# jizongFox/Self-paced-Contrastive-Learning

Hardware: AMD Instinct MI355X
Metric: pretrain slices/sec/node (UNet+InfoNCE, 224^2, bs=32/GPU) (higher is better)
Workload: dtype bf16; 1 GPU; BASELINE.json configs[1]: self-paced pretrain step, UNet base (max_channel=256) encoder to Conv5 + ProjectionHead(256,256,256) + SelfPacedSupConLoss(soft, partition labels, correct_grad) fwd+bwd + RAdam; slices_per_gpu=32, images_per_gpu_step=64, image=1x224x224, global_batch=32, parallelism=dp1, params=1311056, hipgraph=epocher, capture_steps=3

## Files before the change

include/spcl_hip.h:

```cpp
#ifndef SPCL_HIP_H
#define SPCL_HIP_H
#include <stddef.h>
#include <stdint.h>
#ifdef __cplusplus
extern "C" {
#endif

#define SPCL_F32 0
#define SPCL_BF16 1

#define SPCL_OK 0
#define SPCL_EINVAL (-1)
#define SPCL_ELAUNCH (-2)
#define SPCL_EUNSUPPORTED (-3)

#define SPCL_ABI_VERSION 27
int spcl_abi_version(void);
const char* spcl_last_error(void);

size_t spcl_supcon_workspace_bytes(int n, int d);
int spcl_supcon_forward(const float* z1, const float* z2, const float* labels, const float* mask, int n, int d,
                        float temperature, int sp_mode, float gamma, int correct_grad, float* ws, float* out,
                        void* stream);
int spcl_supcon_backward(const float* labels, const float* mask, int n, int d, float temperature, int sp_mode,
                         float gamma, const float* ws_fwd, float* ws_bwd, const float* out_fwd,
                         const float* grad_out, float* dz1, float* dz2, void* stream);
size_t spcl_supcon_bwd_workspace_bytes(int n, int d);
int spcl_supcon_unit_gradient_block(int n, int d, size_t* offset_floats, int* row_pitch);
int spcl_supcon_forward_heads(int K, const float* z1, const float* z2, size_t z_stride, const float* labels, int n,
                              int d, float temperature, int sp_mode, const float* gammas, int correct_grad, float* ws,
                              size_t ws_stride, float* out, void* stream);
int spcl_supcon_rows_supported(int n, int d);
int spcl_supcon_forward_rows(int K, const float* o1, const float* o2, size_t o_stride, const float* labels, int n, int d,
                             float temperature, int sp_mode, const float* gammas, int correct_grad, float* ws,
                             size_t ws_stride, float* out, void* stream);
int spcl_supcon_backward_heads(int K, const float* labels, int n, int d, float temperature, int sp_mode,
                               const float* gammas, const float* ws_fwd, size_t ws_stride, float* ws_bwd,
                               size_t wsb_stride, const float* out_fwd, const float* grad_out, float* dz1, float* dz2,
                               size_t z_stride, void* stream);
int spcl_supcon_materialize(const float* labels, const float* mask, int n, int d, float temperature, int sp_mode,
                            float gamma, const float* ws_fwd, float* sim_logits, float* sim_exp, float* pos_mask,
                            float* neg_mask, float* sp_mask, void* stream);

size_t spcl_supcon_xpos_workspace_bytes(int n, int d);
int spcl_supcon_xpos_forward(const float* z1, const float* z2, const float* labels, const float* mask, int n, int d,
                             float temperature, float* ws, float* out, void* stream);
int spcl_supcon_xpos_backward(const float* z1, const float* z2, int n, int d, float temperature, const float* ws,
                              const float* grad_out, float* dz1, float* dz2, void* stream);

size_t spcl_supcon_weighted_workspace_bytes(int n, int d);
int spcl_supcon_weighted_forward(const float* z1, const float* z2, const float* labels, const float* w11,
                                 const float* w22, const float* w12, int blocks, int mask_semantics, int in_mode, int n,
                                 int d, float temperature, float* ws, float* out, void* stream);
int spcl_supcon_weighted_backward(const float* z1, const float* z2, int n, int d, float temperature, float* ws,
                                  const float* grad_out, float* dz1, float* dz2, void* stream);
int spcl_supcon_weighted_materialize(const float* z1, const float* z2, const float* labels, const float* w11,
                                     const float* w22, const float* w12, int blocks, int mask_semantics, int n, int d,
                                     float temperature, float* ws, float* sim_logits, float* sim_exp, float* pos_weight,
                                     float* enable_mask, void* stream);

int spcl_proj_forward(const void* feat, int dtype, int N, int HW, int C, int Cs, const float* w1, const float* b1,
                      const float* w2, const float* b2, int hid, int out_dim, int normalize, float* pooled,
                      float* pre, float* o, float* z, void* stream);
int spcl_proj_backward(const float* dz, int dtype, int N, int HW, int C, int Cs, const float* w1, const float* w2,
                       int hid, int out_dim, int normalize, const float* pooled, const float* pre, const float* o,
                       float* dw1, float* db1, float* dw2, float* db2, float* scratch ,
                       void* dfeat, void* stream);

int spcl_proj_heads_forward(int K, const void* feat, int dtype, int N, int HW, int C, int Cs, const float* const* w1 ,
                            const float* const* b1 , const float* const* w2 , const float* const* b2 ,
                            int hid, int out_dim, int normalize, float* pooled, float* const* pre ,
                            float* const* o , float* const* z , void* stream);
int spcl_proj_heads_backward(int K, const float* const* dz , int dtype, int N, int HW, int C, int Cs,
                             const float* const* w1 , const float* const* w2 , int hid, int out_dim,
                             int normalize, const float* pooled, const float* const* pre ,
                             const float* const* o , float* const* dw1 , float* const* db1 ,
                             float* const* dw2 , float* const* db2 , float* scratch, void* dfeat, void* stream);
int spcl_proj_heads_backward_pooled(int K, const float* const* dz, int dtype, int N, int HW, int C, int Cs,
                                    const float* const* w1, const float* const* w2, int hid, int out_dim, int normalize,
                                    const float* pooled, const float* const* pre, const float* const* o, float* const* dw1,
                                    float* const* db1, float* const* dw2, float* const* db2, float* scratch, void* dfeat_nc,
                                    void* stream);


size_t spcl_conv_packed_elems(int Cin, int Cout, int kind, int dtype);
int spcl_conv_pack_weights(const float* w_oihw, int Cin, int Cout, int kind, int dtype, void* packed, void* stream);
int spcl_conv_pack_weights_both(const float* w_oihw, int Cin, int Cout, int dtype, void* packed_fwd,
                                void* packed_dgrad, void* stream);

int spcl_conv_pack_weights_block(const float* wa_oihw, int CinA, int CoutA, void* a_fwd, void* a_dgrad,
                                 const float* wb_oihw, int CinB, int CoutB, void* b_fwd, void* b_dgrad, int dtype,
                                 void* stream);
int spcl_conv_pack_weights_block_at(const float* wa_oihw, int CinA, int CoutA, void* a_fwd, void* a_dgrad,
                                    const float* wb_oihw, int CinB, int CoutB, void* b_fwd, void* b_dgrad, int dtype,
                                    int H, int W, void* stream);

#define SPCL_PACK_MULTI_MAX 24
typedef struct spcl_pack_item {
  const float* w_oihw;
// ... 265 lines not shown
int spcl_stage_bytes(void* dst, const void* host_src, size_t nbytes, void* stream);
int spcl_copy_pair(void* dst_a, const void* src_a, size_t bytes_a, void* dst_b, const void* src_b, size_t bytes_b,
                   void* stream);

int spcl_augment_views(const float* src, int S, int HS, int WS, const int* params, int nviews, float* out, int OH,
                       int OW, void* stream);
int spcl_augment_views_pil(const float* src, int S, int HS, int WS, const int* params, int nviews, float* out, int OH,
                           int OW, void* stream);
int spcl_rows_linear_forward(const void* x, int x_dtype, long ldx, int leaky_in, const float* W, const float* bias, int M,
                             int K, int N, float* y, void* stream);
int spcl_rows_linear_forward_act(const void* x, int x_dtype, long ldx, const float* W, const float* bias, int M, int K, int N,
                                 void* h, int h_dtype, void* stream);
int spcl_adaptive_avgpool2d_backward_act(const float* dout, const void* act, int dtype, int N, int H, int W, int C, int OH,
                                         int OW, void* dx, void* stream);
int spcl_rows_linear_backward_input(const void* g, int g_dtype, const float* W, const float* pre, int M, int N, int K, void* dx,
                                    int dx_dtype, long lddx, void* stream);
size_t spcl_rows_linear_backward_weight_workspace_bytes(int M, int N, int K);
int spcl_rows_linear_backward_weight(const void* g, int g_dtype, const void* x, int x_dtype, long ldx, int leaky_in, int M, int N,
                                     int K, float* ws, size_t ws_bytes, float* dW, float* db, void* stream);
int spcl_augment_views_recipe(const float* src, const unsigned char* labels, int S, int HS, int WS, const int* params,
                              int nviews, float* out, long long* label_out, int OH, int OW, int max_pad, void* stream);
size_t spcl_augment_views_recipe_workspace_bytes(int nviews, int OH, int OW);
int spcl_augment_views_recipe_ws(const float* src, const unsigned char* labels, int S, int HS, int WS, const int* params,
                                 int nviews, float* out, long long* label_out, int OH, int OW, int max_pad, void* workspace,
                                 size_t workspace_bytes, void* stream);
int spcl_resize_bilinear_pil(const float* src, int S, int HS, int WS, const int* bounds_x, const int* kk_x, int ksize_x,
                             const int* bounds_y, const int* kk_y, int ksize_y, float* tmp, float* out, int OH, int OW,
                             void* stream);
int spcl_resize_nearest_pil(const unsigned char* src, int S, int HS, int WS, const int* xtab ,
                            const int* ytab , unsigned char* out, int OH, int OW, void* stream);

int spcl_flip_batch(const void* x, void* out, int elem_size, int N, int C, int H, int W, const uint8_t* flags,
                    void* stream);
int spcl_flip_pair(const void* first, const void* second, void* out, int elem_size, int N, int C, int H, int W,
                   const uint8_t* flags, void* stream);
int spcl_flip_pair_stage(const void* first, const void* second, void* out, int elem_size, int N, int C, int H, int W,
                         void* stage_dst, const void* host_src, size_t nbytes, size_t flag_off, void* stream);

int spcl_profile_enable(int on);
int spcl_profile_count(void);
int spcl_profile_get(int i, char* name, int name_cap, float* usec, double* bytes, double* flops);

typedef struct spcl_bn_acc {
  long long* acc;
  const float* gamma;
  const float* beta;
  float* running_mean;
  float* running_var;
  long long* num_batches_tracked;
  float* st;
  float momentum, eps;
  float count;
  int C, CS;
} spcl_bn_acc;
size_t spcl_bn_acc_elems(int CS);
int spcl_conv_bn_acc_supported(int dtype, int N, int H, int W, int CinK, int CoutS, int in_kind, int with_stats_acc);
int spcl_conv3x3_forward_acc(const void* x, int dtype, int N, int H, int W, int CinK, int CoutS, const void* w_packed,
                             const spcl_bn_acc* in_bn, const float* in_scale, const float* in_shift, void* y,
                             long long* stats_acc, float* stats_rows, void* stream);
int spcl_bnrelu_pool_forward_acc(const void* y, int dtype, int N, int H, int W, int CS, const spcl_bn_acc* bn, void* act_out,
                                 void* pool_out, void* stream);
int spcl_bnrelu_gap_supported(int dtype, int H, int W, int C, int CS);
int spcl_bnrelu_gap_forward(const void* y, int dtype, int N, int H, int W, int C, int CS, const float* scale,
                            const float* shift, const spcl_bn_acc* bn, void* act_out, float* gap_out, void* stream);
int spcl_conv_dgrad_bnstats_acc_supported(int dtype, int N, int H, int W, int CinK, int CoutS);
int spcl_conv3x3_dgrad_bnstats_acc(const void* dy, int dtype, int N, int H, int W, int CinK, int CoutS, const void* w_packed,
                                   void* g, const void* y2, const float* scale2, const float* shift2, const float* mean2,
                                   long long* acc, void* stream);
int spcl_conv_dgrad_poolstats_acc_supported(int dtype, int N, int H, int W, int CinK, int CoutS, int H2, int W2);
int spcl_conv3x3_dgrad_poolstats_acc(const void* dy, int dtype, int N, int H, int W, int CinK, int CoutS, const void* w_packed,
                                     void* g, const void* y2, int H2, int W2, const float* scale2, const float* shift2,
                                     const float* mean2, long long* acc, void* stream);
int spcl_bnrelu_pool_forward_ymax(const void* y, int dtype, int N, int H, int W, int CS, const float* scale,
                                  const float* shift, const spcl_bn_acc* bn, void* act_out, void* pool_out, void* ymax_out,
                                  void* stream);
int spcl_conv_dgrad_poolmax_supported(int dtype, int N, int H, int W, int CinK, int CoutS);
int spcl_conv3x3_dgrad_poolmax(const void* dy, int dtype, int N, int H, int W, int CinK, int CoutS, const void* w_packed,
                               void* g, const void* ymax, const float* scale2, const float* shift2, const float* mean2,
                               float* rows2, void* stream);
int spcl_conv_dgrad_poolmax_acc_supported(int dtype, int N, int H, int W, int CinK, int CoutS);
int spcl_conv3x3_dgrad_poolmax_acc(const void* dy, int dtype, int N, int H, int W, int CinK, int CoutS, const void* w_packed,
                                   void* g, const void* ymax, const float* scale2, const float* shift2, const float* mean2,
                                   long long* acc, void* stream);
int spcl_bnrelu_backward_acc(const void* y, const void* dact, const void* dpool, const void* dact_nc, int dtype, int N, int H,
                             int W, int C, int CS, const float* st4, int training, long long* acc, float* dgamma, float* dbeta,
                             void* dy, void* stream);
int spcl_bnrelu_backward_fill_acc(const void* y, void* dact, int dact_stride, const void* dpool, const void* d_up, int dtype,
                                  int N, int H, int W, int C, int CS, const float* st4, int training, long long* acc,
                                  float* dgamma, float* dbeta, void* dy, void* stream);
int spcl_bnrelu_backward_rows_acc(const void* y, const void* dact, const void* dpool, const float* rows, int nrows, int dtype,
                                  int N, int H, int W, int C, int CS, const float* st4, int training, long long* acc,
                                  float* dgamma, float* dbeta, void* dy, void* stream);

size_t spcl_iic_joint_workspace_bytes(int S, int K, int pad);
int spcl_iic_joint_forward(const float* lx, const float* ly, long ld, int N, int H, int W, int S, int K, int pad,
                           const uint8_t* flags_x, long long* jacc, void* stream);
size_t spcl_iic_loss_workspace_bytes(int S, int T);
int spcl_iic_loss(const long long* jacc, const float* jf32, int S, int K, int T, int dense, float scale, float* j_out,
                  float* loss, float* dj, int* nan_flag, void* ws, size_t ws_bytes, void* stream);
int spcl_iic_joint_backward(const float* lx, const float* ly, long ld, int N, int H, int W, int S, int K, int pad,
                            const uint8_t* flags_x, const float* dj, const float* gscale, float* dlx, float* dly, void* stream);
size_t spcl_consistency_workspace_bytes(int N, int H, int W);
int spcl_consistency_softmax_mse(const float* a, const float* b, int N, int C, int H, int W, const uint8_t* flags_a,
                                 float weight, float* loss, float* db, void* ws, size_t ws_bytes, void* stream);

int spcl_iic_patch_plan(int N, int C, int H, int W, int pad, int patch, int* num_patches, size_t* ws_bytes, size_t* dj_elems);
int spcl_iic_patch_forward(const float* lx, const float* ly, int N, int C, int H, int W, int pad, int patch,
                           const uint8_t* flags_y, float scale, float* loss, float* patch_loss, int* nan_flag, float* dj,
                           void* ws, size_t ws_bytes, void* stream);
int spcl_iic_patch_backward(const float* lx, const float* ly, int N, int C, int H, int W, int pad, int patch,
                            const uint8_t* flags_y, const float* dj, const float* gscale, float* dlx, float* dly, void* stream);

int spcl_iic_patch_heads_plan(int N, int S, int K, long ld, int H, int W, int pad, int patch, int* num_patches,
                              size_t* ws_bytes, size_t* dj_elems);
int spcl_iic_patch_heads_forward(const float* lx, const float* ly, long ld, int N, int H, int W, int S, int K, int pad,
                                 int patch, const uint8_t* flags_y, float scale, float* loss, float* head_patch_loss,
                                 int* nan_flag, float* dj, void* ws, size_t ws_bytes, void* stream);
int spcl_iic_patch_heads_backward(const float* lx, const float* ly, long ld, int N, int H, int W, int S, int K, int pad,
                                  int patch, const uint8_t* flags_y, const float* dj, const float* gscale, float* dlx,
                                  float* dly, void* stream);

int spcl_ema_update(float* teacher, const float* student, size_t n, double alpha, double decay, void* stream);
size_t spcl_mt_softmax_mse_workspace_bytes(int N, int H, int W);
int spcl_mt_softmax_mse(const float* teacher, const float* student_logits, int N, int C, int H, int W,
                        const uint8_t* flags_teacher, int teacher_mode, float weight, float* loss, float* dstudent, void* ws,
                        size_t ws_bytes, void* stream);
size_t spcl_entropy_softmax_workspace_bytes(int N, int H, int W);
int spcl_entropy_softmax(const float* logits, int N, int C, int H, int W, float eps, float weight, float* loss, float* dlogits,
                         void* ws, size_t ws_bytes, void* stream);
size_t spcl_ucmt_workspace_bytes(int N, int H, int W);
int spcl_ucmt_softmax_mse(const float* teacher, const float* const* noisy, int K, const float* student_logits, int N, int C,
                          int H, int W, const uint8_t* flags_teacher, float threshold, float eps, float weight, float* loss,
                          float* dstudent, unsigned long long* kept, uint8_t* mask, void* ws, size_t ws_bytes, void* stream);

int spcl_mixup_images(const float* image, const float* image_tf, const int* index, int N2, size_t per_sample, float lam,
                      float oml, float* out, void* stream);
size_t spcl_mixup_kl_workspace_bytes(int N2, int H, int W);
int spcl_mixup_kl_onehot(const float* logits, const int64_t* target, const int64_t* target_tf, const int* index, int N2, int C,
                         int H, int W, float lam, float oml, float eps, float weight, float* loss, float* dlogits, void* ws,
                         size_t ws_bytes, void* stream);

int spcl_patch4s2_rows_forward(const float* a, int Ca, long a_sn, long a_sc, long a_sh, long a_sw, const float* b, int Cb,
                               long b_sn, long b_sc, long b_sh, long b_sw, int N, int H, int W, int mode, const float* scale,
                               const float* shift, float* rows, void* stream);
int spcl_patch4s2_rows_backward(const float* drows, const float* x, int N, int H, int W, int C, int c_lo, int mode,
                                const float* scale, const float* shift, float* dx, void* stream);
size_t spcl_rows_bn_workspace_bytes(int M, int C);
int spcl_rows_bn_forward(const float* x, int M, int C, const float* gamma, const float* beta, float eps, float momentum,
                         float* running_mean, float* running_var, float* stats, void* ws, size_t ws_bytes, void* stream);
int spcl_rows_bn_eval_affine(const float* gamma, const float* beta, const float* running_mean, const float* running_var,
                             float eps, int C, float* stats, void* stream);
int spcl_rows_bn_backward(const float* du, const float* x, int M, int C, const float* gamma, const float* stats, int training,
                          float* dx, float* dgamma, float* dbeta, void* ws, size_t ws_bytes, void* stream);
size_t spcl_discr_head_workspace_bytes(int N, int H, int W, int C);
int spcl_discr_head_forward(const float* x, int N, int H, int W, int C, const float* scale, const float* shift, const float* w,
                            int y, float* t, float* d, float* loss, float* dt, void* ws, size_t ws_bytes, void* stream);
int spcl_discr_head_backward(const float* x, int N, int H, int W, int C, const float* scale, const float* shift, const float* w,
                             const float* dt, const float* grad, float* du, float* dw, void* ws, size_t ws_bytes, void* stream);

int spcl_mine_pairs_forward(const void* feat, const uint8_t* flags, int dtype, int n, int H, int W, int C, void* joint, void* marg,
                            void* stream);
int spcl_mine_pairs_backward(const void* djoint, const void* dmarg, const uint8_t* flags, int dtype, int n, int H, int W, int C,
                             void* dfeat, void* stream);
size_t spcl_mine_head_workspace_bytes(int n, int H, int W, int C);
int spcl_mine_head_forward(const void* act_joint, const void* act_marg, int dtype, int n, int H, int W, int C, const float* w,
                           const float* b, float* t, float* maxima, int* argmax, float* loss, void* ws, size_t ws_bytes,
// ... 16 lines not shown
```

self-paced-contrastive-learning_amd/csrc/bn_acc.hpp:

```cpp
#pragma once
#include "common.hpp"

namespace spcl {

#ifndef SPCL_ACC_REPLICAS
#define SPCL_ACC_REPLICAS 8
#endif
constexpr int BN_ACC_REPLICAS = SPCL_ACC_REPLICAS;
constexpr int BN_ACC_FLAG_WORDS = 4;
constexpr double BN_ACC_HI = 1024.0, BN_ACC_HI_INV = 1.0 / 1024.0;
constexpr double BN_ACC_LO = 1152921504606846976.0 , BN_ACC_LO_INV = 1.0 / 1152921504606846976.0;
constexpr float BN_ACC_MAX = 1099511627776.0f;
#ifndef SPCL_ACC_FWD_TILES
#define SPCL_ACC_FWD_TILES 4096
#endif
constexpr int BN_ACC_MAX_TILES_FWD = SPCL_ACC_FWD_TILES;
constexpr int BN_ACC_MAX_TILES_BWD = 4096;

__host__ __device__ inline size_t bn_acc_words(int CS) { return (size_t)BN_ACC_REPLICAS * CS * 4 + BN_ACC_FLAG_WORDS; }

struct BnAccFwd {
  const long long* acc;
  const float* gamma;
  const float* beta;
// ... 91 lines not shown
    const int cc = c < f.C ? c : f.C - 1;
    g = f.gamma[cc];
    b = f.beta[cc];
    rm = (f.running_mean != nullptr ? f.running_mean : f.gamma)[cc];
    rv = (f.running_var != nullptr ? f.running_var : f.gamma)[cc];
  }
};
__device__ __forceinline__ void bn_acc_fwd_channel(const BnAccFwd& f, const BnAccSums& sums, const BnAccFwdParams& in, int c,
                                                   float& scale, float& shift, bool write) {
  if (c >= f.C) {
    scale = 0.f;
    shift = 0.f;
    if (write) { f.st[c] = 0.f; f.st[f.CS + c] = 0.f; f.st[2 * f.CS + c] = 0.f; f.st[3 * f.CS + c] = 0.f; }
    return;
  }
  double s1, s2;
  sums.totals(s1, s2);
  const float g = in.g, b = in.b;
  const double n = (double)f.count;
  const double mu = s1 * f.inv_count;
  const double m2 = fmax(s2 - s1 * mu, 0.0);
  const double var = m2 * f.inv_count;
  float is = 1.0f / sqrtf((float)var + f.eps);
  float sc = g * is;
  scale = sc;
  shift = b - (float)mu * sc;
  if (sums.flag != 0) {
    is = sc = scale = shift = __builtin_nanf("");
  }
  if (write) {
    f.st[c] = (float)mu;
    f.st[f.CS + c] = is;
    f.st[2 * f.CS + c] = sc;
    f.st[3 * f.CS + c] = shift;
    if (f.running_mean != nullptr) f.running_mean[c] = (1.f - f.momentum) * in.rm + f.momentum * (float)mu;
    if (f.running_var != nullptr) {
      const double unbiased = n > 1.0 ? m2 / (n - 1.0) : var;
      f.running_var[c] = (1.f - f.momentum) * in.rv + f.momentum * (float)unbiased;
    }
    if (f.nbt != nullptr && c == 0) f.nbt[0] += 1;
  }
}
struct BnAccFwdRaw {
  BnAccRaw raw;
  BnAccFwdParams prm;
  __device__ __forceinline__ void load(const BnAccFwd& f, int c) {
    raw.load(f.acc, f.CS, c < f.C ? c : f.C - 1, 0);
    prm.load(f, c);
  }
};
__device__ __forceinline__ void bn_acc_fwd_channel(const BnAccFwd& f, const BnAccFwdRaw& in, int c, float& scale, float& shift,
                                                   bool write) {
  bn_acc_fwd_channel(f, in.raw.sums(), in.prm, c, scale, shift, write);
}

struct BnAccBwdRaw {
  BnAccRaw raw;
  float mean, invstd, scale;
  __device__ __forceinline__ void load(const BnAccBwd& f, int c) {
    raw.load(f.acc, f.CS, c, 0);
    mean = f.st[c];
    invstd = f.st[f.CS + c];
    scale = f.st[2 * f.CS + c];
  }
};
__device__ __forceinline__ void bn_acc_bwd_channel(const BnAccBwd& f, const BnAccBwdRaw& in, int c, float& A, float& B,
                                                   bool write) {
  double t1, t2;
  in.raw.sums().totals(t1, t2);
  const float mean = in.mean, invstd = in.invstd, scale = in.scale;
  const float s1 = (float)t1;
  const float s2 = (float)t2 * invstd;
  A = 0.f;
  B = 0.f;
  if (f.training) {
    A = -scale * invstd * (s2 / f.count);
    B = -scale * (s1 / f.count) - A * mean;
  }
  if (write && c < f.C) {
    f.dbeta[c] = s1;
    f.dgamma[c] = s2;
  }
}
#endif

}
```

self-paced-contrastive-learning_amd/csrc/conv.hip:

```cpp
#include <stdlib.h>
#include "bn_acc.hpp"
#include "conv_common.hpp"
#include "image_acorr.hpp"

namespace spcl {

#ifndef SPCL_SPLIT_KC_MAX
#define SPCL_SPLIT_KC_MAX 64
#endif
__host__ __device__ inline int split_kc(int CinK, int CoutS) {
  const int cap = CoutS <= 16 ? 16 : (CoutS <= 32 ? 32 : SPCL_SPLIT_KC_MAX);
  return CinK < cap ? CinK : cap;
}
__host__ __device__ inline int split_pstride(int KC) {
  const int b = 3 * KC * 2;
  return (b / 32) % 2 == 1 ? b : b + 32;
}
__device__ __forceinline__ f32x4 mfma_bf16(u32x4 w, u32x4 x, f32x4 acc) {
  return __builtin_amdgcn_mfma_f32_16x16x32_bf16(__builtin_bit_cast(bf16x8, w), __builtin_bit_cast(bf16x8, x), acc, 0, 0, 0);
}

template <typename T, int TH, int TW, int NT, bool SPLIT = false>
__global__ __launch_bounds__(256) void conv3x3_mfma_kernel(ConvArgs a) {
  static_assert(!SPLIT || sizeof(T) == 4, "the split k-loop is the f32 storage path");
// ... 1354 lines not shown
  if (!(CinK <= 64 || CinK % 64 == 0)) return false;
  a.in_scale = a.in_shift = nullptr;
  a.stats = nullptr;
  a.N = N; a.H = H; a.W = W; a.CinS = CinK; a.CinK = CinK; a.CoutS = CoutS; a.in_mode = 0;
  a.tilesX = a.tilesY = 0;
  a.tpw = 1;
  a.dbg = 0;
  return true;
}

extern "C" int spcl_conv_dgrad_bnstats_supported(int dtype, int N, int H, int W, int CinK, int CoutS) {
  static const bool off = lab_flag("SPCL_NO_DGRAD_BNSTATS");
  ConvArgs a;
  if (off || !dgrad_bnstats_args(a, dtype, N, H, W, CinK, CoutS)) return 0;
  if (conv_use_gemm(CinK, CoutS, H, W)) return 1;
  a.x = nullptr; a.y = nullptr; a.wp = nullptr;
  float dummy;
  a.rows2 = &dummy;
  TileCfg t = pick_tile(H, W);
  return (t.tw == 14 && launch_conv_fast(a, t.th, nullptr, true)) ? 1 : 0;
}

static int dgrad_bnstats_impl(const void* dy, int dtype, int N, int H, int W, int CinK, int CoutS, const void* w_packed, void* g,
                              const void* y2, const float* scale2, const float* shift2, const float* mean2, float* rows2,
                              long long* acc, void* stream);

extern "C" int spcl_conv3x3_dgrad_bnstats(const void* dy, int dtype, int N, int H, int W, int CinK, int CoutS,
                                          const void* w_packed, void* g, const void* y2, const float* scale2,
                                          const float* shift2, const float* mean2, float* rows2, void* stream) {
  SPCL_CHECK_ARG(rows2, "conv3x3_dgrad_bnstats: null pointer");
  return dgrad_bnstats_impl(dy, dtype, N, H, W, CinK, CoutS, w_packed, g, y2, scale2, shift2, mean2, rows2, nullptr, stream);
}

extern "C" int spcl_conv_dgrad_bnstats_acc_supported(int dtype, int N, int H, int W, int CinK, int CoutS) {
  ConvArgs a;
  if (!spcl_conv_dgrad_bnstats_supported(dtype, N, H, W, CinK, CoutS) || conv_use_gemm(CinK, CoutS, H, W)) return 0;
  if (!dgrad_bnstats_args(a, dtype, N, H, W, CinK, CoutS)) return 0;
  a.x = nullptr; a.y = nullptr; a.wp = nullptr;
  float dummy;
  long long dummy2;
  a.rows2 = &dummy;
  a.rows2_acc = &dummy2;
  TileCfg t = pick_tile(H, W);
  return (t.tw == 14 && launch_conv_fast(a, t.th, nullptr, true)) ? 1 : 0;
}

extern "C" int spcl_conv3x3_dgrad_bnstats_acc(const void* dy, int dtype, int N, int H, int W, int CinK, int CoutS,
                                              const void* w_packed, void* g, const void* y2, const float* scale2,
                                              const float* shift2, const float* mean2, long long* acc, void* stream) {
  SPCL_CHECK_ARG(acc, "conv3x3_dgrad_bnstats_acc: null pointer");
  return dgrad_bnstats_impl(dy, dtype, N, H, W, CinK, CoutS, w_packed, g, y2, scale2, shift2, mean2, nullptr, acc, stream);
}

static int dgrad_bnstats_impl(const void* dy, int dtype, int N, int H, int W, int CinK, int CoutS, const void* w_packed, void* g,
                              const void* y2, const float* scale2, const float* shift2, const float* mean2, float* rows2,
                              long long* acc, void* stream) {
  SPCL_CHECK_ARG(dy && w_packed && g && y2 && scale2 && shift2 && mean2, "conv3x3_dgrad_bnstats: null pointer");
  ConvArgs a;
  if (!dgrad_bnstats_args(a, dtype, N, H, W, CinK, CoutS) || (acc != nullptr && conv_use_gemm(CinK, CoutS, H, W))) {
    set_error("conv3x3_dgrad_bnstats: unsupported configuration");
    return SPCL_EUNSUPPORTED;
  }
  a.x = dy; a.y = g; a.wp = w_packed;
  a.y2 = y2; a.scale2 = scale2; a.shift2 = shift2; a.mean2 = mean2;
  a.rows2 = acc != nullptr ? (float*)acc : rows2;
  a.rows2_acc = acc;
  hipStream_t st = (hipStream_t)stream;
  const double px = (double)N * H * W;
  prof_cost(px * (CinK + 2.0 * CoutS) * 2.0 + 9.0 * CinK * CoutS * 2.0, 2.0 * px * 9.0 * CinK * CoutS);
  TileCfg t = pick_tile(H, W);
  if (conv_use_gemm(CinK, CoutS, H, W)) {
    if (!launch_conv_gemm(a, st)) {
      set_error("conv3x3_dgrad_bnstats: H=%d W=%d CinK=%d CoutS=%d outside the gemm kernel's range", H, W, CinK, CoutS);
      return SPCL_EUNSUPPORTED;
    }
  } else if (!(t.tw == 14 && launch_conv_fast(a, t.th, st))) {
    set_error("conv3x3_dgrad_bnstats: no specialised kernel for H=%d W=%d CinK=%d CoutS=%d", H, W, CinK, CoutS);
    return SPCL_EUNSUPPORTED;
  }
  SPCL_LAUNCH_CHECK("conv3x3_dgrad_bnstats");
  return SPCL_OK;
}

extern "C" int spcl_conv_dgrad_bnstats_image_supported(int dtype, int N, int H, int W, int CinK, int CoutS) {
  static const bool off = lab_flag("SPCL_NO_IMAGE3");
  ConvArgs a;
  if (off || CinK != 16 || CoutS != 16 || !dgrad_bnstats_args(a, dtype, N, H, W, CinK, CoutS)) return 0;
  if (!spcl_conv_dgrad_bnstats_supported(dtype, N, H, W, CinK, CoutS) || conv_use_gemm(CinK, CoutS, H, W)) return 0;
  a.x = nullptr; a.y = nullptr; a.wp = nullptr;
  float dummy;
  a.rows2 = &dummy;
  a.img2 = &dummy;
  TileCfg t = pick_tile(H, W);
  return (t.tw == 14 && t.th == 14 && launch_conv_fast(a, t.th, nullptr, true)) ? 1 : 0;
}

extern "C" int spcl_conv3x3_dgrad_bnstats_image(const void* dy, int dtype, int N, int H, int W, int CinK, int CoutS,
                                                const void* w_packed, void* g, const void* y2, const float* scale2,
                                                const float* shift2, const float* mean2, const float* image,
                                                float* rows11, void* stream) {
  SPCL_CHECK_ARG(dy && w_packed && y2 && scale2 && shift2 && mean2 && image && rows11,
                 "conv3x3_dgrad_bnstats_image: null pointer");
  ConvArgs a;
  if (!spcl_conv_dgrad_bnstats_image_supported(dtype, N, H, W, CinK, CoutS) ||
      !dgrad_bnstats_args(a, dtype, N, H, W, CinK, CoutS)) {
    set_error("conv3x3_dgrad_bnstats_image: unsupported configuration (bf16, 16 -> 16 channels, 14 x 14 tiles)");
    return SPCL_EUNSUPPORTED;
  }
  a.x = dy; a.y = g; a.wp = w_packed;
  a.y2 = y2; a.scale2 = scale2; a.shift2 = shift2; a.mean2 = mean2; a.rows2 = rows11; a.img2 = image;
  hipStream_t st = (hipStream_t)stream;
  const double px = (double)N * H * W;
  prof_cost(px * (CinK + (g ? 2.0 : 1.0) * CoutS) * 2.0 + px * 4.0 + 9.0 * CinK * CoutS * 2.0,
            2.0 * px * 9.0 * CinK * CoutS + 2.0 * px * 9.0 * CoutS);
  TileCfg t = pick_tile(H, W);
  if (!(t.tw == 14 && launch_conv_fast(a, t.th, st))) {
    set_error("conv3x3_dgrad_bnstats_image: no specialised kernel for H=%d W=%d", H, W);
    return SPCL_EUNSUPPORTED;
  }
  SPCL_LAUNCH_CHECK("conv3x3_dgrad_bnstats_image");
  return SPCL_OK;
}

extern "C" int spcl_conv_dgrad_poolstats_supported(int dtype, int N, int H, int W, int CinK, int CoutS, int H2, int W2) {
  static const bool off = lab_flag("SPCL_NO_DGRAD_POOLSTATS");
  ConvArgs a;
  if (off || H != H2 / 2 || W != W2 / 2 || !dgrad_bnstats_args(a, dtype, N, H, W, CinK, CoutS)) return 0;
  if (conv_use_gemm(CinK, CoutS, H, W)) return 0;
  a.x = nullptr; a.y = nullptr; a.wp = nullptr;
  float dummy;
  a.rows2 = &dummy;
  a.H2 = H2; a.W2 = W2;
  TileCfg t = pick_tile(H, W);
  return (t.tw == 14 && launch_conv_fast(a, t.th, nullptr, true)) ? 1 : 0;
}

static int dgrad_poolstats_impl(const void* dy, int dtype, int N, int H, int W, int CinK, int CoutS, const void* w_packed,
                                void* g, const void* y2, int H2, int W2, const float* scale2, const float* shift2,
                                const float* mean2, float* rows2, long long* acc, void* stream);

extern "C" int spcl_conv3x3_dgrad_poolstats(const void* dy, int dtype, int N, int H, int W, int CinK, int CoutS,
                                            const void* w_packed, void* g, const void* y2, int H2, int W2,
                                            const float* scale2, const float* shift2, const float* mean2, float* rows2,
                                            void* stream) {
  SPCL_CHECK_ARG(rows2, "conv3x3_dgrad_poolstats: null pointer");
  return dgrad_poolstats_impl(dy, dtype, N, H, W, CinK, CoutS, w_packed, g, y2, H2, W2, scale2, shift2, mean2, rows2, nullptr,
                              stream);
}

extern "C" int spcl_conv_dgrad_poolstats_acc_supported(int dtype, int N, int H, int W, int CinK, int CoutS, int H2, int W2) {
  ConvArgs a;
  if (!spcl_conv_dgrad_poolstats_supported(dtype, N, H, W, CinK, CoutS, H2, W2)) return 0;
  if (!dgrad_bnstats_args(a, dtype, N, H, W, CinK, CoutS)) return 0;
  a.x = nullptr; a.y = nullptr; a.wp = nullptr;
  float dummy;
  long long dummy2;
  a.rows2 = &dummy;
  a.rows2_acc = &dummy2;
  a.H2 = H2; a.W2 = W2;
  TileCfg t = pick_tile(H, W);
  return (t.tw == 14 && launch_conv_fast(a, t.th, nullptr, true)) ? 1 : 0;
}

extern "C" int spcl_conv3x3_dgrad_poolstats_acc(const void* dy, int dtype, int N, int H, int W, int CinK, int CoutS,
                                                const void* w_packed, void* g, const void* y2, int H2, int W2,
                                                const float* scale2, const float* shift2, const float* mean2,
// ... 97 lines not shown
```

self-paced-contrastive-learning_amd/csrc/conv_common.hpp:

```cpp
#pragma once
#include "common.hpp"

namespace spcl {

struct BnAccFwd;
template <typename T> struct Chunk;
template <> struct Chunk<float> { static constexpr int EPC = 4; };
template <> struct Chunk<bf16_t> { static constexpr int EPC = 8; };

struct uint4_ { uint32_t x, y, z, w; };
typedef __attribute__((ext_vector_type(4))) uint32_t u32x4;

__host__ __device__ inline int conv_kc(int CinK) { return CinK < 64 ? CinK : 64; }
template <typename T> __host__ __device__ inline int conv_pstride(int KC) {
  int b = KC * (int)sizeof(T);
  return b == 32 ? 32 : b + 32;
}
template <typename T> __host__ __device__ inline int conv_nsteps(int KC) {
  int cp = KC / Chunk<T>::EPC;
  return (9 * cp + 3) / 4;
}

struct ConvArgs {
  const void* x;
  void* y;
  const void* wp;
  float* stats;
  const float* in_scale;
  const float* in_shift;
  int N, H, W;
  int CinS;
  int CinK;
  int CoutS;
  int in_mode;
  int tilesX, tilesY;
  int tpw;
  int dbg;
  const void* y2 = nullptr;
  const float* scale2 = nullptr;
  const float* shift2 = nullptr;
  const float* mean2 = nullptr;
  float* rows2 = nullptr;
  int H2 = 0, W2 = 0;
  bool y2_is_poolmax = false;
  const float* img2 = nullptr;
  const void* x2 = nullptr;
  void* y_hi = nullptr;
  bool x_up2 = false;
  float* acorr_rows = nullptr;
  const float* img1 = nullptr;
  const void* wp1 = nullptr;
  long long* stats_acc = nullptr;
  long long* rows2_acc = nullptr;
  const struct BnAccFwd* in_bn = nullptr;
};

struct split_f32 { float v; };
template <> struct Chunk<split_f32> { static constexpr int EPC = 4; };
bool conv_f32_split();

typedef __attribute__((ext_vector_type(2))) float f32x2_;
typedef __attribute__((ext_vector_type(2))) __bf16 bf16x2v_;
struct Split3 { uint32_t hi, mid, lo; };
__device__ __forceinline__ Split3 split3_pair(float v0, float v1) {
  Split3 o;
  f32x2_ v = {v0, v1};
  o.hi = __builtin_bit_cast(uint32_t, __builtin_convertvector(v, bf16x2v_));
  v[0] -= __uint_as_float(o.hi << 16);
  v[1] -= __uint_as_float(o.hi & 0xffff0000u);
  o.mid = __builtin_bit_cast(uint32_t, __builtin_convertvector(v, bf16x2v_));
  v[0] -= __uint_as_float(o.mid << 16);
  v[1] -= __uint_as_float(o.mid & 0xffff0000u);
  o.lo = __builtin_bit_cast(uint32_t, __builtin_convertvector(v, bf16x2v_));
  return o;
}
__device__ __forceinline__ void split3_chunk(const float* e, u32x4& ph, u32x4& pm, u32x4& pl) {
#pragma unroll
  for (int k = 0; k < 4; ++k) {
    const Split3 o = split3_pair(e[2 * k], e[2 * k + 1]);
    ph[k] = o.hi;
    pm[k] = o.mid;
    pl[k] = o.lo;
  }
}
template <typename T> __device__ __forceinline__ f32x4 mfma_chunk(u32x4 w, u32x4 x, f32x4 acc);
template <> __device__ __forceinline__ f32x4 mfma_chunk<bf16_t>(u32x4 w, u32x4 x, f32x4 acc) {
  return __builtin_amdgcn_mfma_f32_16x16x32_bf16(__builtin_bit_cast(bf16x8, w), __builtin_bit_cast(bf16x8, x), acc, 0,
                                                 0, 0);
}
template <> __device__ __forceinline__ f32x4 mfma_chunk<float>(u32x4 w, u32x4 x, f32x4 acc) {
  f32x4 wf = __builtin_bit_cast(f32x4, w), xf = __builtin_bit_cast(f32x4, x);
  acc = __builtin_amdgcn_mfma_f32_16x16x4f32(wf[0], xf[0], acc, 0, 0, 0);
  acc = __builtin_amdgcn_mfma_f32_16x16x4f32(wf[1], xf[1], acc, 0, 0, 0);
  acc = __builtin_amdgcn_mfma_f32_16x16x4f32(wf[2], xf[2], acc, 0, 0, 0);
  acc = __builtin_amdgcn_mfma_f32_16x16x4f32(wf[3], xf[3], acc, 0, 0, 0);
  return acc;
}

__device__ __forceinline__ float row16_sum(float v) {
  v += __builtin_bit_cast(float, __builtin_amdgcn_update_dpp(0, __builtin_bit_cast(int, v), 0xB1, 0xF, 0xF, true));
  v += __builtin_bit_cast(float, __builtin_amdgcn_update_dpp(0, __builtin_bit_cast(int, v), 0x4E, 0xF, 0xF, true));
  v += __builtin_bit_cast(float, __builtin_amdgcn_update_dpp(0, __builtin_bit_cast(int, v), 0x141, 0xF, 0xF, true));
  v += __builtin_bit_cast(float, __builtin_amdgcn_update_dpp(0, __builtin_bit_cast(int, v), 0x140, 0xF, 0xF, true));
  return v;
}

typedef __attribute__((ext_vector_type(2))) float f32x2;
typedef __attribute__((ext_vector_type(2))) __bf16 bf16x2v;
typedef __attribute__((ext_vector_type(2))) short s16x2v;

__device__ __forceinline__ uint32_t relu_bf16x2(uint32_t packed) {
  const s16x2v z = {0, 0};
  return __builtin_bit_cast(uint32_t, __builtin_elementwise_max(__builtin_bit_cast(s16x2v, packed), z));
}

template <typename T> __device__ __forceinline__ u32x4 bnrelu_regs(u32x4 raw, const float* s, const float* b);
template <> __device__ __forceinline__ u32x4 bnrelu_regs<float>(u32x4 raw, const float* s, const float* b) {
  f32x4 v = __builtin_bit_cast(f32x4, raw);
#pragma unroll
  for (int e = 0; e < 4; ++e) v[e] = fmaxf(fmaf(s[e], v[e], b[e]), 0.f);
  return __builtin_bit_cast(u32x4, v);
}
template <> __device__ __forceinline__ u32x4 bnrelu_regs<bf16_t>(u32x4 raw, const float* s, const float* b) {
  u32x4 out;
#pragma unroll
  for (int e = 0; e < 4; ++e) {
    float lo = __uint_as_float(raw[e] << 16), hi = __uint_as_float(raw[e] & 0xffff0000u);
    lo = fmaf(s[2 * e], lo, b[2 * e]);
    hi = fmaf(s[2 * e + 1], hi, b[2 * e + 1]);
    const f32x2 v = {lo, hi};
    out[e] = relu_bf16x2(__builtin_bit_cast(uint32_t, __builtin_convertvector(v, bf16x2v)));
  }
  return out;
}

template <typename T> __device__ __forceinline__ void store4_fast(unsigned char* p, f32x4 v);
template <> __device__ __forceinline__ void store4_fast<float>(unsigned char* p, f32x4 v) { *(f32x4*)p = v; }
template <> __device__ __forceinline__ void store4_fast<bf16_t>(unsigned char* p, f32x4 v) {
  const f32x2 lo = {v[0], v[1]}, hi = {v[2], v[3]};
  uint2 o;
  o.x = __builtin_bit_cast(uint32_t, __builtin_convertvector(lo, bf16x2v));
  o.y = __builtin_bit_cast(uint32_t, __builtin_convertvector(hi, bf16x2v));
  *(uint2*)p = o;
}

__device__ __forceinline__ void write_tile_stats(float* stats, int tile, int CoutS, int cb, int r16, float cnt,
                                                 f32x4 ssum, f32x4 ssq) {
  const float inv = 1.f / cnt;
  f32x4 o;
#pragma unroll
  for (int r = 0; r < 4; ++r) {
    const float s1 = row16_sum(ssum[r]), s2 = row16_sum(ssq[r]);
    const float mean = s1 * inv;
    float prod = s1 * mean;
    asm volatile("" : "+v"(prod));
    const float m2 = fmaxf(s2 - prod, 0.f);
    o[r] = r16 == 0 ? cnt : (r16 == 1 ? mean : m2);
  }
  if (r16 < 3) *(f32x4*)(stats + ((size_t)tile * 3 + r16) * CoutS + cb) = o;
}

bool launch_conv_fast(const ConvArgs& a, int th, hipStream_t st, bool dry = false);

__host__ __device__ inline bool conv_gemm_channels(int CinK, int CoutS) {
  return CinK % 64 == 0 && CoutS % 64 == 0 && CinK >= 64 && CoutS >= 64 && (CinK >= 128 || CoutS >= 128);
}
bool conv_gemm_fits(int H, int W, int CinK, int CoutS);
bool conv_use_gemm(int CinK, int CoutS, int H, int W);
void conv_set_gemm(int mode);
bool launch_conv_gemm(const ConvArgs& a, hipStream_t st);
int conv_gemm_stat_rows(int N, int H, int W, int CinK, int CoutS);

}
```

self-paced-contrastive-learning_amd/csrc/conv_fast.hip:

```cpp
#include <stdlib.h>
#include <type_traits>
#include <vector>
#include "bn_acc.hpp"
#include "conv_common.hpp"

namespace spcl {

struct FastArgs {
  const unsigned char* x;
  const unsigned char* x2;
  unsigned char* y;
  unsigned char* y_hi;
  int up2;
  const u32x4* wp;
  float* stats;
  const float* in_scale;
  const float* in_shift;
  int N, H, W, CinK, CoutS, tilesX, tilesY, gy;
  unsigned long long* stamps;
  int ipw;
  int lds_flip;
  int xcd_remap;
  const unsigned char* y2;
  const float* scale2;
  const float* shift2;
  const float* mean2;
  float* rows2;
  int H2, W2;
  const float* img2;
  const float* img1;
  const u32x4* wp1;
  float* acorr_rows;
  long long* stats_acc;
  long long* rows2_acc;
  BnAccFwd in_bn;
};

#ifndef SPCL_FAST_WPE_NT1
#define SPCL_FAST_WPE_NT1 2
#endif
#ifndef SPCL_FAST_WPE_NT1_NW4
#define SPCL_FAST_WPE_NT1_NW4 3
#endif
#ifndef SPCL_FAST_WR_NT1
#define SPCL_FAST_WR_NT1 9
#endif
#ifndef SPCL_FAST_WPE_KC32
#define SPCL_FAST_WPE_KC32 2
#endif
#ifndef SPCL_FAST_YPRE_MINKC
#define SPCL_FAST_YPRE_MINKC 16
#endif
#ifndef SPCL_FAST_WIDE_STORES
#define SPCL_FAST_WIDE_STORES 1
#endif
#ifndef SPCL_FAST_DBG
#define SPCL_FAST_DBG 0
#endif
#ifndef SPCL_FAST_ROWMAP
#define SPCL_FAST_ROWMAP 1
#endif
#ifndef SPCL_FAST_RP
#define SPCL_FAST_RP (SPCL_FAST_ROWMAP ? 18 : 22)
#endif
#ifndef SPCL_FAST_RP_NARROW
#define SPCL_FAST_RP_NARROW (SPCL_FAST_ROWMAP ? 18 : 22)
#endif
constexpr int fast_pixel_stride(int KC) { return KC == 16 ? 32 : KC * 2 + 32; }
constexpr int fast_row_pitch(int KC) { return KC == 64 ? SPCL_FAST_RP : SPCL_FAST_RP_NARROW; }
constexpr int fast_lds_bytes(int KC, int TH) { return (TH + 2) * fast_row_pitch(KC) * fast_pixel_stride(KC); }
constexpr bool fast_preload_slab(int KC, int NW, int NT) { return KC == 32 || (KC == 64 && NW >= 2 && NT >= 1); }
constexpr int fast_wpe(int KC, int TH, int NW, int NT, int MODE = 0) {
  const int wgs = 160 * 1024 / fast_lds_bytes(KC, TH);
  int w = (wgs * NW + 3) / 4;
  w = w > 4 ? 4 : (w < 1 ? 1 : w);
  const int acc = (SPCL_FAST_ROWMAP ? TH : (TH * 14 + 15) / 16) * NT * 4;
  if (KC == 16 && MODE >= 2 && MODE <= 4 && SPCL_FAST_YPRE_MINKC <= 16 && w > 3 && acc <= 80) return 3;
  if (acc > 80 && w > 2) return 2;
  if (KC == 64 && NT == 1 && NW == 4 && w > 2) return SPCL_FAST_WPE_NT1_NW4;
  if (KC == 64 && NT == 1 && NW >= 2 && w > 2) return SPCL_FAST_WPE_NT1;
  if (KC == 32 && fast_preload_slab(KC, NW, NT) && w > SPCL_FAST_WPE_KC32) return SPCL_FAST_WPE_KC32;
  if (fast_preload_slab(KC, NW, NT) && w > 2) return 2;
  return w;
}

template <int KC, int TH, int NT, int MODE, int NW>
__global__ __launch_bounds__(64 * NW) __attribute__((amdgpu_waves_per_eu(fast_wpe(KC, TH, NW, NT, MODE)))) void
conv3x3_fast_kernel(FastArgs a) {
  constexpr int TW = 14, HW_ = 16, CP = KC / 8, NHALO = (TH + 2) * HW_, PS = fast_pixel_stride(KC);
  constexpr int RP = fast_row_pitch(KC);
  constexpr int NTHR = 64 * NW, NCH = NHALO * CP, ITER = (NCH + NTHR - 1) / NTHR, QS = NTHR / CP;
  constexpr bool RM = SPCL_FAST_ROWMAP != 0;
  constexpr int NPIX = TH * TW, MT = RM ? TH : (NPIX + 15) / 16, NSTEPS = (9 * CP + 3) / 4;
  constexpr bool PRELOAD_W = KC == 16;
  constexpr bool PRELOAD_SLAB = fast_preload_slab(KC, NW, NT);
  static_assert(QS >= HW_ ? QS % HW_ == 0 : HW_ % QS == 0, "staging walk needs whole/even halo rows per iteration");
  extern __shared__ __attribute__((aligned(16))) unsigned char lds[];

  const int t = threadIdx.x, lane = t & 63, wave = t >> 6, r16 = lane & 15, g = lane >> 4;
#ifndef SPCL_FAST_STAMPS_BUILD
#define SPCL_FAST_STAMPS_BUILD 0
#endif
  const bool stamp = SPCL_FAST_STAMPS_BUILD && a.stamps != nullptr && t == 0;
  unsigned long long t_begin = 0, t_k0 = 0, t_k1 = 0, t_store = 0;
  if (stamp) t_begin = __builtin_amdgcn_s_memtime();
  int tx = blockIdx.x, ty = blockIdx.y;
  {
    const int T = a.tilesX * a.tilesY;
    if (a.xcd_remap && (T & 7) == 0) {
      const int L = ty * a.tilesX + tx;
      const int L2 = (L & 7) * (T >> 3) + (L >> 3);
      ty = L2 / a.tilesX;
      tx = L2 - ty * a.tilesX;
    }
  }
  int n = blockIdx.z, by = 0;
#if SPCL_FAST_DBG & 4
  if (KC == 64 && a.CinK >= 128 && gridDim.z == 2u * a.N * a.gy) n >>= 1;
#endif
  if (a.gy > 1) {
    by = n / a.N;
    n -= by * a.N;
  }
  const int y0 = min(ty * TH, a.H - TH), x0 = min(tx * TW, a.W - TW);
  const int oy = ty * TH - y0, ox = tx * TW - x0;
  const int tile = (n * a.tilesY + ty) * a.tilesX + tx;
  const int ntn = a.CoutS >> 4;
  const int nt0 = (by * NW + wave) * NT;
  const bool interior = y0 > 0 && x0 > 0 && y0 + TH < a.H && x0 + TW < a.W;
#if SPCL_FAST_DBG & 4
  const int nslab = KC < 64 ? 1 : ((a.CinK >= 128 && gridDim.z == 2u * a.N * a.gy) ? a.CinK / KC / 2 : a.CinK / KC);
#else
  const int nslab = KC < 64 ? 1 : a.CinK / KC;
#endif
  const int gps = (KC < 64 ? KC : a.CinK) * 2;

  constexpr bool M2 = MODE == 2 || MODE == 4;
  constexpr bool M1 = MODE == 1 || (MODE >= 5 && MODE <= 7);
  constexpr bool M8 = MODE == 8;
  static_assert(!M8 || (KC == 16 && TH == 14 && NT == 1 && NW == 1), "MODE 8: the 16 -> 16 layer on 14 x 14 tiles, one wave");
  constexpr int ACC_TPC = MODE == 5 ? 4 : (MODE == 6 ? 2 : 1);
  float imgv[MODE == 4 ? 4 : 1];
  if (MODE == 4) {
    const int hr = lane >> 2, hc = (lane & 3) * 4;
    const int gy = y0 - 1 + hr;
    const float* ir = a.img2 + ((size_t)n * a.H + (gy < 0 ? 0 : (gy >= a.H ? a.H - 1 : gy))) * a.W;
#pragma unroll
    for (int e = 0; e < 4; ++e) {
      const int gx = x0 - 1 + hc + e;
      const bool in = gy >= 0 && gy < a.H && gx >= 0 && gx < a.W;
      const float xv = ir[gx < 0 ? 0 : (gx >= a.W ? a.W - 1 : gx)];
      imgv[e] = in ? xv : 0.f;
    }
  }

  u32x4 wall[PRELOAD_W ? NSTEPS : 1][NT];
  if (PRELOAD_W) {
#pragma unroll
    for (int s = 0; s < NSTEPS; ++s)
#pragma unroll
      for (int j = 0; j < NT; ++j) wall[s][j] = a.wp[(size_t)(s * ntn + nt0 + j) * 64 + lane];
  }

  const int ch = t & (CP - 1), q0 = t / CP;
  const int hy0 = q0 / HW_, hx0 = q0 % HW_;
  const bool two = a.x2 != nullptr;
  const bool two_chunks = two && a.CinK == KC;
  const int gps1 = two ? gps / 2 : gps;
  const int ch1 = two_chunks ? (ch & (CP / 2 - 1)) : ch;
  const long xorg = (((long)n * a.H + (y0 - 1)) * a.W + (x0 - 1)) * gps1;
  const unsigned char* xb = ((two_chunks && ch >= CP / 2) ? a.x2 : a.x) + xorg;
  const unsigned char* xb2 = two ? a.x2 + xorg : nullptr;
  const unsigned voff = (unsigned)((hy0 * a.W + hx0) * gps1 + ch1 * 16);
  unsigned char* const lp = lds + (hy0 * RP + hx0) * PS + ch * 16;

  int abase[MT];
#pragma unroll
  for (int i = 0; i < MT; ++i) {
    if (RM) {
      abase[i] = (i * RP + r16) * PS + (CP >= 4 ? g * 16 : 0);
    } else {
      int p = 16 * i + r16;
      if (p >= NPIX) p = 0;
      const int py = p / TW, px = p - py * TW;
      abase[i] = (py * RP + px) * PS + (CP >= 4 ? g * 16 : 0);
    }
  }
  f32x4 acc[MT][NT];
#pragma unroll
  for (int i = 0; i < MT; ++i)
#pragma unroll
    for (int j = 0; j < NT; ++j) acc[i][j] = (f32x4){0.f, 0.f, 0.f, 0.f};

  const int flip = a.lds_flip;
  const unsigned wvo = (unsigned)(nt0 * 64 + lane) * 16u;
  const size_t wstep = (size_t)ntn * 1024;
  u32x4 v[ITER];
  float ssc[8], ssh[8];
  constexpr int IW8 = 18;
  float imv8[M8 ? 6 : 1];
  s16x4 wfrag8 = {0, 0, 0, 0};
  f32x4 sc8 = {0.f, 0.f, 0.f, 0.f}, sh8 = {0.f, 0.f, 0.f, 0.f};
  const int ir8 = lane / IW8, ic8 = lane - ir8 * IW8;
  constexpr bool STREAM_W = PRELOAD_SLAB && KC == 64;
  constexpr int WR = STREAM_W ? (NT == 1 ? SPCL_FAST_WR_NT1 : 9) : (PRELOAD_SLAB ? NSTEPS : 1);
  u32x4 wsl[WR][NT];
  constexpr bool acc_in = MODE >= 5 && MODE <= 7;
  float* const coef_l = (float*)(lds + fast_lds_bytes(KC, TH) * (a.lds_flip != 0 ? 2 : 1));
  auto load_coef_lds = [&](int slab) {
    const int cc = two_chunks ? ch1 : ch;
#pragma unroll
    for (int e = 0; e < 8; e += 4) {
      *(f32x4*)&ssc[e] = *(const f32x4*)(coef_l + slab * KC + cc * 8 + e);
      *(f32x4*)&ssh[e] = *(const f32x4*)(coef_l + a.CinK + slab * KC + cc * 8 + e);
    }
  };
  auto issue_halo = [&](int slab, const bool first = false) {
    if (acc_in) {
      if (!first) load_coef_lds(slab);
    } else if (M1) {
#pragma unroll
      for (int e = 0; e < 8; e += 4) {
        const int cc = two_chunks ? ch1 : ch;
        *(f32x4*)&ssc[e] = *(const f32x4*)(a.in_scale + slab * KC + cc * 8 + e);
        *(f32x4*)&ssh[e] = *(const f32x4*)(a.in_shift + slab * KC + cc * 8 + e);
      }
    }
    const int hslab = (a.CinK / KC) >> 1;
    const unsigned char* xs = (two && !two_chunks) ? (slab >= hslab ? xb2 + (slab - hslab) * (KC * 2) : xb + slab * (KC * 2))
                                                   : xb + slab * (KC * 2);
    auto walk = [&](auto up2_c, auto interior_c) {
      constexpr bool UP2 = decltype(up2_c)::value, INTERIOR = decltype(interior_c)::value;
#pragma unroll
      for (int k = 0; k < ITER; ++k) {
        const int dky = QS >= HW_ ? k * (QS / HW_) : k / (HW_ / QS);
        const int dkx = QS >= HW_ ? 0 : (k % (HW_ / QS)) * QS;
        const long soff = ((long)dky * a.W + dkx) * gps1;
        bool inb = (NCH % NTHR == 0) || (k * NTHR + t < NCH);
        if (!INTERIOR) {
          const int gy = y0 - 1 + hy0 + dky, gx = x0 - 1 + hx0 + dkx;
          inb = inb && gy >= 0 && gy < a.H && gx >= 0 && gx < a.W;
        }
        v[k] = (u32x4){0u, 0u, 0u, 0u};
        if (UP2) {
          const int gy = y0 - 1 + hy0 + dky, gx = x0 - 1 + hx0 + dkx;
          if (inb)
            v[k] = *(const u32x4*)(a.x + (((long)n * (a.H >> 1) + (gy >> 1)) * (a.W >> 1) + (gx >> 1)) * gps + slab * (KC * 2) +
                                   ch * 16);
        } else if (inb) v[k] = *(const u32x4*)(xs + soff + voff);
      }
    };
    if (a.up2) walk(std::true_type{}, std::false_type{});
    else if (interior) walk(std::false_type{}, std::true_type{});
    else walk(std::false_type{}, std::false_type{});
  };
  unsigned char* lpw = lp;
  auto slab_body = [&](const int slab, const bool refill) {
    auto stage = [&](auto interior_c) {
      constexpr bool INTERIOR = decltype(interior_c)::value;
#pragma unroll
      for (int k = 0; k < ITER; ++k) {
        const int dky = QS >= HW_ ? k * (QS / HW_) : k / (HW_ / QS);
        const int dkx = QS >= HW_ ? 0 : (k % (HW_ / QS)) * QS;
        const bool in_range = (NCH % NTHR == 0) || (k * NTHR + t < NCH);
        u32x4 tv = v[k];
        if (M1) {
          bool inb = true;
          if (!INTERIOR) {
            const int gy = y0 - 1 + hy0 + dky, gx = x0 - 1 + hx0 + dkx;
            inb = gy >= 0 && gy < a.H && gx >= 0 && gx < a.W;
          }
          if (inb && (!two_chunks || ch >= CP / 2)) tv = bnrelu_regs<bf16_t>(tv, ssc, ssh);
        }
        if (in_range) *(u32x4*)(lpw + (dky * RP + dkx) * PS) = tv;
      }
    };
    if constexpr (M8) {
      typedef uint32_t __attribute__((may_alias)) pair_t;
      typedef unsigned short __attribute__((may_alias)) half_t;
      const pair_t* const pairs = (const pair_t*)lds;
      half_t* const halves = (half_t*)lds;
      unsigned short pb8[6];
#pragma unroll
      for (int k = 0; k < 6; ++k) {
        const f32x2 pv = {imv8[k], 0.f};
        pb8[k] = (unsigned short)__builtin_bit_cast(uint32_t, __builtin_convertvector(pv, bf16x2v));
      }
      if (lane < 3 * IW8) {
#pragma unroll
        for (int k = 0; k < 6; ++k) halves[2 * ((ir8 + 3 * k) * IW8 + ic8)] = pb8[k];
        if (ic8 > 0) {
#pragma unroll
          for (int k = 0; k < 6; ++k) halves[2 * ((ir8 + 3 * k) * IW8 + ic8) - 1] = pb8[k];
        }
        if (ic8 == IW8 - 1) {
#pragma unroll
          for (int k = 0; k < 6; ++k) halves[2 * ((ir8 + 3 * k) * IW8 + ic8) + 1] = 0;
        }
      }
      __syncthreads();
      const int gx = x0 - 1 + r16;
      const bool colin = gx >= 0 && gx < a.W;
      const int gg = g < 3 ? g : 0;
      uint2 hv[HW_];
#pragma unroll
      for (int hy = 0; hy < TH + 2; ++hy) {
        const pair_t* src = pairs + (hy + gg) * IW8 + r16;
        const uint2 xv = {src[0], src[2]};
        const f32x4 y = __builtin_amdgcn_mfma_f32_16x16x16bf16_1k(wfrag8, __builtin_bit_cast(s16x4, xv),
                                                                  (f32x4){0.f, 0.f, 0.f, 0.f}, 0, 0, 0);
        const f32x2 ylo = {y[0], y[1]}, yhi = {y[2], y[3]};
        const uint32_t p0 = __builtin_bit_cast(uint32_t, __builtin_convertvector(ylo, bf16x2v));
        const uint32_t p1 = __builtin_bit_cast(uint32_t, __builtin_convertvector(yhi, bf16x2v));
        const u32x4 raw = {p0, p1, 0u, 0u};
        const float s4[8] = {sc8[0], sc8[1], sc8[2], sc8[3], 0.f, 0.f, 0.f, 0.f};
        const float b4[8] = {sh8[0], sh8[1], sh8[2], sh8[3], 0.f, 0.f, 0.f, 0.f};
        const u32x4 tv = bnrelu_regs<bf16_t>(raw, s4, b4);
        hv[hy] = (uint2){tv[0], tv[1]};
      }
      if (!interior) {
#pragma unroll
        for (int hy = 0; hy < TH + 2; ++hy) {
          const int gy = y0 - 1 + hy;
          if (!(colin && gy >= 0 && gy < a.H)) hv[hy] = (uint2){0u, 0u};
        }
      }
      __syncthreads();
#pragma unroll
      for (int hy = 0; hy < TH + 2; ++hy) *(uint2*)(lds + (hy * RP + r16) * PS + g * 8) = hv[hy];
    } else if (M1 && !interior) stage(std::false_type{});
    else stage(std::true_type{});
    if (refill) issue_halo(slab + 1);
    if (stamp && slab == 0) t_store = __builtin_amdgcn_s_memtime();
    __syncthreads();
    if (stamp && slab == 0) t_k0 = __builtin_amdgcn_s_memtime();

    const u32x4* wslab = a.wp + ((size_t)slab * NSTEPS * ntn + nt0) * 64 + lane;
    auto frag_off = [&](const int s) {
      if (CP >= 4) {
        const int fc0 = 4 * s, tap = fc0 / CP, c0 = fc0 % CP, ky = tap / 3, kx = tap % 3;
        return (ky * RP + kx) * PS + c0 * 16;
      }
      int fc = 4 * s + g;
      if (fc >= 9 * CP) fc = 0;
      const int tap = fc / CP, c = fc % CP, ky = (tap * 11) >> 5, kx = tap - 3 * ky;
      return (ky * RP + kx) * PS + c * 16;
    };
    if (STREAM_W) {
      const __amdgpu_buffer_rsrc_t wrs = __builtin_amdgcn_make_buffer_rsrc((void*)a.wp, 0, 0x7fffffff, 0x00020000);
      unsigned wrun = (unsigned)(((size_t)slab * NSTEPS + WR) * wstep);
      u32x4 xf[2][MT];
#pragma unroll
      for (int i = 0; i < MT; ++i) xf[0][i] = *(const u32x4*)(lds + abase[i] + frag_off(0));
#pragma unroll
      for (int s = 0; s < NSTEPS; ++s) {
        u32x4 wf[NT];
#pragma unroll
        for (int j = 0; j < NT; ++j) wf[j] = wsl[s % WR][j];
#pragma unroll
        for (int i = 0; i < MT; ++i) {
#pragma unroll
          for (int j = 0; j < NT; ++j) acc[i][j] = mfma_chunk<bf16_t>(wf[j], xf[s & 1][i], acc[i][j]);
          if (s + 1 < NSTEPS && !(SPCL_FAST_DBG & 2)) xf[(s + 1) & 1][i] = *(const u32x4*)(lds + abase[i] + frag_off(s + 1));
          if (i == MT - 1 && (s + WR < NSTEPS || refill) && !(SPCL_FAST_DBG & 1)) {
#pragma unroll
            for (int j = 0; j < NT; ++j)
              wsl[s % WR][j] = __builtin_bit_cast(u32x4, __builtin_amdgcn_raw_buffer_load_b128(wrs, wvo + j * 1024, wrun, 0));
          }
          __builtin_amdgcn_sched_barrier(0);
        }
        wrun += (unsigned)wstep;
      }
    } else {
#pragma unroll
      for (int s = 0; s < NSTEPS; ++s) {
        u32x4 wf[NT];
#pragma unroll
        for (int j = 0; j < NT; ++j)
          wf[j] = PRELOAD_W ? wall[s][j] : (PRELOAD_SLAB ? wsl[s][j] : wslab[(size_t)(s * ntn + j) * 64]);
        const int off = frag_off(s);
#pragma unroll
        for (int i = 0; i < MT; ++i) {
          const u32x4 xf = *(const u32x4*)(lds + abase[i] + off);
#pragma unroll
          for (int j = 0; j < NT; ++j) acc[i][j] = mfma_chunk<bf16_t>(wf[j], xf, acc[i][j]);
          if (RM && !PRELOAD_SLAB && i % 7 == 6) __builtin_amdgcn_sched_barrier(0);
        }
      }
    }
  };
#ifndef SPCL_ACC_DBG
#define SPCL_ACC_DBG 0
#endif
  const int acc_part = acc_in ? t / a.CinK : 0, acc_c = t - acc_part * a.CinK;
  constexpr int ACC_RPT = BN_ACC_REPLICAS / ACC_TPC > 0 ? BN_ACC_REPLICAS / ACC_TPC : 1;
  const bool acc_has = acc_part * ACC_RPT < BN_ACC_REPLICAS;
  BnAccPart<ACC_RPT> accp;
  BnAccFwdParams accprm;
  if (acc_in && SPCL_ACC_DBG < 2) {
    accp.load(a.in_bn.acc, a.CinK, acc_c, acc_has ? ACC_RPT * acc_part : 0);
    accprm.load(a.in_bn, acc_c);
  }
  if constexpr (M8) {
    const float* im = a.img1 + (size_t)n * a.H * a.W;
    const int gx = x0 - 2 + ic8;
    const bool colok = gx >= 0 && gx < a.W;
    const int gxc = gx < 0 ? 0 : (gx >= a.W ? a.W - 1 : gx);
#pragma unroll
    for (int k = 0; k < 6; ++k) {
      const int gy = y0 - 2 + ir8 + 3 * k;
      const int gyc = gy < 0 ? 0 : (gy >= a.H ? a.H - 1 : gy);
      const float raw = im[(size_t)gyc * a.W + gxc];
      imv8[k] = (colok && gy >= 0 && gy < a.H) ? raw : 0.f;
    }
    if (g < 3) {
      const bf16_t* wq = (const bf16_t*)a.wp1;
#pragma unroll
      for (int kx = 0; kx < 3; ++kx) {
        const int tap = 3 * g + kx;
        wfrag8[kx] = (short)wq[(size_t)(((tap >> 1) * 64) + (2 * (tap & 1)) * 16 + r16) * 8];
      }
    }
    sc8 = *(const f32x4*)(a.in_scale + 4 * g);
    sh8 = *(const f32x4*)(a.in_shift + 4 * g);
  } else {
    issue_halo(0, true);
  }
  if (PRELOAD_SLAB) {
#pragma unroll
    for (int s = 0; s < WR; ++s)
#pragma unroll
      for (int j = 0; j < NT; ++j) wsl[s][j] = a.wp[((size_t)s * ntn + nt0 + j) * 64 + lane];
  }
  if (acc_in) {
    const bool writer = (blockIdx.x | blockIdx.y | blockIdx.z) == 0;
    BnAccSums sums{0, 0, 0, 0, 0};
    if (SPCL_ACC_DBG < 2 && acc_has) sums = accp.sums();
    if (SPCL_ACC_DBG < 2) sums.flag = accp.flag;
    if (ACC_TPC > 1) {
      long long* const part_l = (long long*)(coef_l + 2 * a.CinK);
      if (acc_part > 0) {
        long long* q = part_l + ((size_t)(acc_part - 1) * a.CinK + acc_c) * 4;
        *(i64x2*)q = (i64x2){sums.h1, sums.l1};
        *(i64x2*)(q + 2) = (i64x2){sums.h2, sums.l2};
      }
      __syncthreads();
      if (acc_part == 0) {
#pragma unroll
        for (int k = 1; k < ACC_TPC; ++k) {
          const long long* q = part_l + ((size_t)(k - 1) * a.CinK + acc_c) * 4;
          const i64x2 u = *(const i64x2*)q, w = *(const i64x2*)(q + 2);
          sums.h1 += u[0]; sums.l1 += u[1]; sums.h2 += w[0]; sums.l2 += w[1];
        }
      }
    }
    if (t < a.CinK) {
      float sc_, sh_;
      if (SPCL_ACC_DBG == 0) bn_acc_fwd_channel(a.in_bn, sums, accprm, t, sc_, sh_, writer);
      else { sc_ = a.in_bn.gamma[t]; sh_ = a.in_bn.beta[t]; }
      coef_l[t] = sc_;
      coef_l[a.CinK + t] = sh_;
    }
    __syncthreads();
    load_coef_lds(0);
  }
  if (MODE == 4) {
    const int q = lane & 3;
    float n0 = __shfl_down(imgv[0], 1, 64), n1 = __shfl_down(imgv[1], 1, 64);
    if (q == 3) n0 = n1 = 0.f;
    const float h6[6] = {imgv[0], imgv[1], imgv[2], imgv[3], n0, n1};
    unsigned char* imb = lds + fast_lds_bytes(KC, TH) + (lane >> 2) * 32 + q * 8;
#pragma unroll
    for (int kx = 0; kx < 3; ++kx) {
      const f32x2 lo = {h6[kx], h6[kx + 1]}, hi = {h6[kx + 2], h6[kx + 3]};
      uint2 w;
      w.x = __builtin_bit_cast(uint32_t, __builtin_convertvector(lo, bf16x2v));
      w.y = __builtin_bit_cast(uint32_t, __builtin_convertvector(hi, bf16x2v));
      *(uint2*)(imb + kx * 512) = w;
    }
  }
  int img = 0;
#pragma unroll 1
  for (int slab = 0; slab + 1 < nslab; ++slab) {
    if (slab > 0 && flip == 0) __syncthreads();
    slab_body(slab, true);
    const int d = img ? -flip : flip;
    img ^= 1;
    lpw += d;
#pragma unroll
    for (int i = 0; i < MT; ++i) abase[i] += d;
  }
  if (nslab > 1 && flip == 0) __syncthreads();
  slab_body(nslab - 1, false);
  if (stamp) t_k1 = __builtin_amdgcn_s_memtime();

  constexpr int DPY = RM ? 1 : 16 / TW, DPX = RM ? 0 : 16 % TW;
  const int rowb = a.CoutS * 2;
  const bool twoy = (MODE == 0 || MODE == 2) && a.y_hi != nullptr;
  const bool up_only = MODE == 2 && twoy;
  const int rowo = twoy ? rowb / 2 : rowb;
  unsigned char* yj[NT];
#pragma unroll
  for (int j = 0; j < NT; ++j) {
    const int gnt = nt0 + j, half = ntn / 2;
    unsigned char* dst = (twoy && gnt >= half) ? a.y_hi : a.y;
    yj[j] = dst + (((size_t)n * a.H + y0) * a.W + x0) * rowo + ((twoy && gnt >= half ? gnt - half : gnt) * 16 + 4 * g) * 2;
  }
  int py = RM ? 0 : r16 / TW, px = r16 - py * TW;
  int ob = (py * a.W + px) * rowo;
  const int dob = (DPY * a.W + DPX) * rowo, wrapo = (a.W - TW) * rowo;
  f32x4 ssum[NT], ssq[NT];
  f32x4 sc2[NT], sh2[NT], mu2[NT];
  const unsigned char* y2b = nullptr;
#pragma unroll
  for (int j = 0; j < NT; ++j) {
    ssum[j] = (f32x4){0.f, 0.f, 0.f, 0.f};
    ssq[j] = (f32x4){0.f, 0.f, 0.f, 0.f};
    if (M2 || MODE == 3) {
      const int gnt2 = nt0 + j, half2 = ntn / 2;
      const int cb = (up_only ? (gnt2 >= half2 ? gnt2 - half2 : 0) : gnt2) * 16 + 4 * g;
      sc2[j] = *(const f32x4*)(a.scale2 + cb);
      sh2[j] = *(const f32x4*)(a.shift2 + cb);
      mu2[j] = *(const f32x4*)(a.mean2 + cb);
    }
  }
  if (M2) y2b = a.y2 + (((size_t)n * a.H + y0) * a.W + x0) * rowb + (nt0 * 16 + 4 * g) * 2;
  const unsigned char* y2j[NT];
  bool st2[NT];
#pragma unroll
  for (int j = 0; j < NT; ++j) {
    const int gnt2 = nt0 + j, half2 = ntn / 2;
    st2[j] = !up_only || gnt2 >= half2;
    y2j[j] = !M2 ? nullptr
                 : (up_only ? a.y2 + (((size_t)n * a.H + y0) * a.W + x0) * rowo + ((st2[j] ? gnt2 - half2 : 0) * 16 + 4 * g) * 2
                            : y2b + j * 32);
  }
  constexpr int M4_DZ = 0, M4_IM = fast_lds_bytes(KC, TH);
  static_assert(MODE != 4 || fast_lds_bytes(KC, TH) >= 7168, "MODE 4 scratch does not fit the halo image");
  if (MODE == 4) {
#pragma unroll
    for (int k = 0; k < 4; ++k) {
      const int e = k * 64 + lane;
      if (e < 16 * TH) *(uint32_t*)(lds + M4_DZ + e * 32 + 28) = 0u;
    }
    __syncthreads();
  }
  const bool shifted = (oy | ox) != 0;
// ... 60 lines not shown
          const bool second = PAIRED && i % 2 == 1 && (RM || 16 * i + 15 < NPIX);
          if (first || second) {
            const f32x2 lo = {acc[i][j][0], acc[i][j][1]}, hi = {acc[i][j][2], acc[i][j][3]};
            uint2 pkc;
            pkc.x = __builtin_bit_cast(uint32_t, __builtin_convertvector(lo, bf16x2v));
            pkc.y = __builtin_bit_cast(uint32_t, __builtin_convertvector(hi, bf16x2v));
            if (first) {
              pk_prev[j] = pkc;
              ob_prev = ob;
            } else {
              const auto rx = __builtin_amdgcn_permlane16_swap(pk_prev[j].x, pkc.x, false, false);
              const auto ry = __builtin_amdgcn_permlane16_swap(pk_prev[j].y, pkc.y, false, false);
              const u32x4 v = {rx[0], ry[0], rx[1], ry[1]};
              *(u32x4*)(yj[j] + ((g & 1) ? ob - 8 : ob_prev)) = v;
            }
          } else {
            store4_fast<bf16_t>(yj[j] + ob, acc[i][j]);
          }
        }
        if (M2) {
          const uint2 yr = YPRE ? ypre[i][j][0] : *(const uint2*)(y2j[j] + ob);
          const f32x2 glo = {acc[i][j][0], acc[i][j][1]}, ghi = {acc[i][j][2], acc[i][j][3]};
          const uint32_t g0 = __builtin_bit_cast(uint32_t, __builtin_convertvector(glo, bf16x2v));
          const uint32_t g1 = __builtin_bit_cast(uint32_t, __builtin_convertvector(ghi, bf16x2v));
          const float yv[4] = {__uint_as_float(yr.x << 16), __uint_as_float(yr.x & 0xffff0000u),
                               __uint_as_float(yr.y << 16), __uint_as_float(yr.y & 0xffff0000u)};
          const float gv[4] = {__uint_as_float(g0 << 16), __uint_as_float(g0 & 0xffff0000u),
                               __uint_as_float(g1 << 16), __uint_as_float(g1 & 0xffff0000u)};
#pragma unroll
          for (int r = 0; r < 4; ++r) {
            const float dz = (st2[j] && fmaf(sc2[j][r], yv[r], sh2[j][r]) > 0.f) ? gv[r] * keep : 0.f;
            ssum[j][r] += dz;
            ssq[j][r] = fmaf(dz, yv[r] - mu2[j][r], ssq[j][r]);
            if (MODE == 4) *(bf16_t*)(lds + M4_DZ + (4 * g + r) * 448 + pyc * 32 + px * 2) = f32_to_bf16(dz);
          }
        } else if (MODE == 3) {
          const f32x2 glo = {acc[i][j][0], acc[i][j][1]}, ghi = {acc[i][j][2], acc[i][j][3]};
          const uint32_t g0 = __builtin_bit_cast(uint32_t, __builtin_convertvector(glo, bf16x2v));
          const uint32_t g1 = __builtin_bit_cast(uint32_t, __builtin_convertvector(ghi, bf16x2v));
          const float gv[4] = {__uint_as_float(g0 << 16), __uint_as_float(g0 & 0xffff0000u),
                               __uint_as_float(g1 << 16), __uint_as_float(g1 & 0xffff0000u)};
          uint2 yr[4];
          if (YPRE) {
#pragma unroll
            for (int k = 0; k < 4; ++k) yr[k] = ypre[i][j][k];
          } else {
            const unsigned char* wb = a.y2 + ((((size_t)n * a.H2 + 2 * (y0 + pyc)) * a.W2 + 2 * (x0 + px)) * rowb) +
                                      ((nt0 + j) * 16 + 4 * g) * 2;
#pragma unroll
            for (int k = 0; k < 4; ++k) yr[k] = *(const uint2*)(wb + ((size_t)(k >> 1) * a.W2 + (k & 1)) * rowb);
          }
#pragma unroll
          for (int r = 0; r < 4; ++r) {
            float zb = -1.f, yb = 0.f;
#pragma unroll
            for (int k = 0; k < 4; ++k) {
              const uint32_t wd = r < 2 ? yr[k].x : yr[k].y;
              const float yv = (r & 1) ? __uint_as_float(wd & 0xffff0000u) : __uint_as_float(wd << 16);
              pool_first_max(k, fmaf(sc2[j][r], yv, sh2[j][r]), yv, zb, yb);
            }
            const float dz = zb > 0.f ? gv[r] * keep : 0.f;
            ssum[j][r] += dz;
            ssq[j][r] = fmaf(dz, yb - mu2[j][r], ssq[j][r]);
          }
        } else {
          const f32x4 av = acc[i][j] * keep;
          ssum[j] += av;
          ssq[j] += av * acc[i][j];
        }
      }
    }
    px += DPX;
    pyc += DPY;
    ob += dob;
    if (!RM && px >= TW) {
      px -= TW;
      pyc += 1;
      ob += wrapo;
    }
  }
  }
  constexpr int RS = MODE == 4 ? 11 : 2;
  const int replica = (int)((blockIdx.x + gridDim.x * (blockIdx.y + gridDim.y * blockIdx.z)) & (BN_ACC_REPLICAS - 1));
  if ((MODE == 2 || MODE == 3) && a.rows2_acc != nullptr) {
#pragma unroll
    for (int j = 0; j < NT; ++j) {
      f32x4 s1, s2;
#pragma unroll
      for (int r = 0; r < 4; ++r) {
        s1[r] = row16_sum(ssum[j][r]);
        s2[r] = row16_sum(ssq[j][r]);
      }
      bn_acc_add_row16(a.rows2_acc, a.CoutS, replica, (nt0 + j) * 16 + 4 * g, r16, s1, s2);
    }
  } else if (M2 || MODE == 3) {
#pragma unroll
    for (int j = 0; j < NT; ++j) {
      f32x4 o;
#pragma unroll
      for (int r = 0; r < 4; ++r) {
        const float s1 = row16_sum(ssum[j][r]), s2 = row16_sum(ssq[j][r]);
        o[r] = r16 == 0 ? s1 : s2;
      }
      if (up_only) {
        if (r16 < 2 && st2[j])
          *(f32x4*)(a.rows2 + ((size_t)tile * RS + r16) * (a.CoutS / 2) + (nt0 + j - ntn / 2) * 16 + 4 * g) = o;
      } else if (r16 < 2) *(f32x4*)(a.rows2 + ((size_t)tile * RS + r16) * a.CoutS + (nt0 + j) * 16 + 4 * g) = o;
    }
    if (MODE == 4) {
      static_assert(MODE != 4 || NT == 1, "image tap sums: one n-tile");
      __syncthreads();
      const int tap = r16 < 9 ? r16 : 0, tky = tap / 3, tkx = tap - 3 * tky;
      const unsigned char* pa = lds + M4_DZ + r16 * 448 + (g >> 1) * 32 + (g & 1) * 16;
      const unsigned char* pb = lds + M4_IM + tkx * 512 + ((g >> 1) + tky) * 32 + (g & 1) * 16;
      f32x4 D = {0.f, 0.f, 0.f, 0.f};
#pragma unroll
      for (int ks = 0; ks < TH / 2; ++ks)
        D = mfma_chunk<bf16_t>(*(const u32x4*)(pa + ks * 64), *(const u32x4*)(pb + ks * 64), D);
      if (r16 < 9) *(f32x4*)(a.rows2 + ((size_t)tile * RS + 2 + r16) * a.CoutS + nt0 * 16 + 4 * g) = D;
    }
  } else if ((MODE == 0 || M1) && a.stats_acc != nullptr) {
#pragma unroll
    for (int j = 0; j < NT; ++j) {
      f32x4 s1, s2;
#pragma unroll
      for (int r = 0; r < 4; ++r) {
        s1[r] = row16_sum(ssum[j][r]);
        s2[r] = row16_sum(ssq[j][r]);
      }
      bn_acc_add_row16(a.stats_acc, a.CoutS, replica, (nt0 + j) * 16 + 4 * g, r16, s1, s2);
    }
  } else if (a.stats != nullptr) {
#pragma unroll
    for (int j = 0; j < NT; ++j)
      write_tile_stats(a.stats, tile, a.CoutS, (nt0 + j) * 16 + 4 * g, r16, (float)((TH - oy) * (TW - ox)), ssum[j],
                       ssq[j]);
  }
  if (stamp) {
    __builtin_amdgcn_s_waitcnt(0);
    const unsigned long long t_end = __builtin_amdgcn_s_memtime();
    unsigned long long* o = a.stamps + ((size_t)(blockIdx.z * gridDim.y + blockIdx.y) * gridDim.x + blockIdx.x) * 4;
    o[0] = t_store - t_begin; o[1] = t_k0 - t_store; o[2] = t_k1 - t_k0; o[3] = t_end - t_k1;
  }
}

template <int TH, bool EVEN, bool ACORR = false, bool STORE = true>
__global__ __launch_bounds__(64) __attribute__((amdgpu_waves_per_eu(4))) void conv3x3_image_kernel(FastArgs a) {
  constexpr int TW = 14, HW_ = 16, LW = HW_ + 2;
  constexpr bool RM = SPCL_FAST_ROWMAP != 0;
  constexpr int NPIX = TH * TW, MT = RM ? TH : (NPIX + 15) / 16, NHALO = (TH + 2) * HW_;
  __shared__ uint32_t pairs[(TH + 2) * LW];
  const int lane = threadIdx.x, r16 = lane & 15, g = lane >> 4;
  int tx = blockIdx.x, ty = blockIdx.y;
  const int n_first = STORE ? (int)blockIdx.z : (int)blockIdx.z * a.ipw;
  const int n_end = STORE ? n_first + 1 : min(n_first + a.ipw, a.N);
  {
    const int T = a.tilesX * a.tilesY;
    if (a.xcd_remap && (T & 7) == 0) {
      const int L = ty * a.tilesX + tx;
      const int L2 = (L & 7) * (T >> 3) + (L >> 3);
      ty = L2 / a.tilesX;
      tx = L2 - ty * a.tilesX;
    }
  }
  const int y0 = min(ty * TH, a.H - TH), x0 = min(tx * TW, a.W - TW);
  const int oy = ty * TH - y0, ox = tx * TW - x0;

// ... 75 lines not shown
      if (STORE) {
        obs[i] = ob;
        const f32x2 lo = {acc[i][0], acc[i][1]}, hi = {acc[i][2], acc[i][3]};
        pk[i].x = __builtin_bit_cast(uint32_t, __builtin_convertvector(lo, bf16x2v));
        pk[i].y = __builtin_bit_cast(uint32_t, __builtin_convertvector(hi, bf16x2v));
      }
      if (ok) {
        if (EVEN) {
          ssum += acc[i];
          ssq += acc[i] * acc[i];
        } else {
          const float keep = (!shifted || (pyc >= oy && px >= ox)) ? 1.f : 0.f;
          const f32x4 av = acc[i] * keep;
          ssum += av;
          ssq += av * acc[i];
        }
      }
      px += DPX;
      pyc += DPY;
      ob += dob;
      if (!RM && px >= TW) {
        px -= TW;
        pyc += 1;
        ob += wrapo;
      }
    }
    constexpr int NPAIR = !STORE ? 0 : (SPCL_FAST_WIDE_STORES ? (RM ? MT / 2 : (NPIX / 16) / 2) : 0);
#pragma unroll
    for (int p = 0; p < NPAIR; ++p) {
      const int i = 2 * p;
      const auto rx = __builtin_amdgcn_permlane16_swap(pk[i].x, pk[i + 1].x, false, false);
      const auto ry = __builtin_amdgcn_permlane16_swap(pk[i].y, pk[i + 1].y, false, false);
      const u32x4 v = {rx[0], ry[0], rx[1], ry[1]};
      *(u32x4*)(yb + ((g & 1) ? obs[i + 1] - 8 : obs[i])) = v;
    }
#pragma unroll
    for (int i = 2 * NPAIR; i < MT; ++i) {
      const bool ok = RM || (16 * i + 15 < NPIX) || (16 * i + r16 < NPIX);
      if (STORE && ok) *(uint2*)(yb + obs[i]) = pk[i];
    }
    }
    if (a.stats != nullptr)
      write_tile_stats(a.stats, tile, a.CoutS, 4 * g, r16, (float)((TH - oy) * (TW - ox)), ssum, ssq);
    if (ACORR) {
      static_assert(!ACORR || (EVEN && TH % 2 == 0), "autocorrelation rows: whole 14 x 14 tiles");
      __shared__ float dsum[2][16][16];
      const int tap = r16 < 9 ? r16 : 0, ky = tap / 3, kx = tap - 3 * ky;
      const uint32_t* src = pairs + ((g >> 1) + ky) * LW + 8 * (g & 1) + kx;
      const bool upper = (g & 1) != 0;
      const u32x4 ones = {0x3f803f80u, 0x3f803f80u, 0x3f803f80u, 0x3f803f80u};
      f32x4 D = {0.f, 0.f, 0.f, 0.f}, S = {0.f, 0.f, 0.f, 0.f};
#pragma unroll
      for (int ks = 0; ks < TH / 2; ++ks) {
        const uint32_t* q = src + ks * 2 * LW;
        const u32x4 fb = {q[0], q[2], q[4], q[6]};
        u32x4 fa = fb;
        fa[3] = upper ? 0u : fb[3];
        D = __builtin_amdgcn_mfma_f32_16x16x32_bf16(__builtin_bit_cast(bf16x8, fa), __builtin_bit_cast(bf16x8, fb), D, 0, 0, 0);
        S = __builtin_amdgcn_mfma_f32_16x16x32_bf16(__builtin_bit_cast(bf16x8, fa), __builtin_bit_cast(bf16x8, ones), S, 0, 0, 0);
      }
#pragma unroll
      for (int r = 0; r < 4; ++r) {
        dsum[0][4 * g + r][r16] = D[r];
        dsum[1][4 * g + r][r16] = S[r];
      }
      __syncthreads();
      const int k = lane;
      float v = 0.f;
      if (k < 45) {
        int ra = 0;
#pragma unroll
        for (int i = 1; i < 9; ++i) ra += k >= i * 9 - i * (i - 1) / 2 ? 1 : 0;
        const int cb = ra + (k - (ra * 9 - ra * (ra - 1) / 2));
        v = dsum[0][ra][cb];
      } else if (k < 54) {
        v = dsum[1][k - 45][0];
      }
      a.acorr_rows[(size_t)tile * 64 + k] = v;
    }
  }
}

template <int KC, int TH, int NT, int NW>
static void launch_fast(const FastArgs& a, int mode, hipStream_t st) {
  static const int env_pipe = lab_env("SPCL_CONV_FAST_PIPE", 1);
  const bool pipe = env_pipe && KC == 64 && a.CinK > KC;
  FastArgs b = a;
  b.lds_flip = pipe ? fast_lds_bytes(KC, TH) : 0;
  const size_t lds = fast_lds_bytes(KC, TH) * (pipe ? 2 : 1) + (a.img2 != nullptr ? 1536 : 0) +
                     (a.in_bn.acc != nullptr ? (size_t)a.CinK * 8 + (size_t)64 * NW * 32 : 0);
  dim3 grid(a.tilesX, a.tilesY, a.N * a.gy), block(64 * NW);
#if SPCL_FAST_DBG & 4
  if (KC == 64 && a.CinK >= 128 && (long)a.tilesX * a.tilesY * a.N * a.gy <= 256) grid.z *= 2;
#endif
  static const bool env_stamps = SPCL_FAST_STAMPS_BUILD && lab_flag("SPCL_FAST_STAMPS");
  const size_t nwg = (size_t)grid.x * grid.y * grid.z;
  b.stamps = nullptr;
  if (env_stamps) {
    (void)hipMalloc(&b.stamps, nwg * 4 * sizeof(unsigned long long));
    (void)hipMemset(b.stamps, 0, nwg * 4 * sizeof(unsigned long long));
  }
  if (a.img2 != nullptr) {
    if constexpr (KC == 16 && TH == 14 && NT == 1 && NW == 1)
      SPCL_LAUNCH((conv3x3_fast_kernel<KC, TH, NT, 4, NW>), grid, block, lds, st, b);
  } else if (mode == 8) {
    if constexpr (KC == 16 && TH == 14 && NT == 1 && NW == 1)
      SPCL_LAUNCH((conv3x3_fast_kernel<KC, TH, NT, 8, NW>), grid, block, lds, st, b);
  } else if (mode == 1 && a.in_bn.acc != nullptr) {
    if constexpr (KC == 64) {
      const int tpc = 64 * NW / a.CinK;
      if (tpc == 4) SPCL_LAUNCH((conv3x3_fast_kernel<KC, TH, NT, 5, NW>), grid, block, lds, st, b);
      else if (tpc == 2) SPCL_LAUNCH((conv3x3_fast_kernel<KC, TH, NT, 6, NW>), grid, block, lds, st, b);
      else SPCL_LAUNCH((conv3x3_fast_kernel<KC, TH, NT, 7, NW>), grid, block, lds, st, b);
    }
  } else if (mode == 1) SPCL_LAUNCH((conv3x3_fast_kernel<KC, TH, NT, 1, NW>), grid, block, lds, st, b);
  else if (a.rows2 != nullptr && a.H2 > 0) SPCL_LAUNCH((conv3x3_fast_kernel<KC, TH, NT, 3, NW>), grid, block, lds, st, b);
  else if (a.rows2 != nullptr) SPCL_LAUNCH((conv3x3_fast_kernel<KC, TH, NT, 2, NW>), grid, block, lds, st, b);
  else SPCL_LAUNCH((conv3x3_fast_kernel<KC, TH, NT, 0, NW>), grid, block, lds, st, b);
  if (b.stamps != nullptr) {
    std::vector<unsigned long long> h(nwg * 4);
    (void)hipStreamSynchronize(st);
    (void)hipMemcpy(h.data(), b.stamps, h.size() * 8, hipMemcpyDeviceToHost);
    (void)hipFree(b.stamps);
    double s4[4] = {0, 0, 0, 0};
    for (size_t i = 0; i < nwg; ++i)
      for (int k = 0; k < 4; ++k) s4[k] += (double)h[i * 4 + k];
    fprintf(stderr, "[conv_fast stamps] <%d,%d,%d,m%d,%d> %dx%d CinK %d CoutS %d wgs %zu | s_memtime ticks per wg: setup + first "
            "halo + LDS store %.0f, barrier %.0f, k-loops (all slabs) %.0f, epilogue %.0f\n", KC, TH, NT,
            mode == 1 ? 1 : (a.rows2 ? (a.H2 > 0 ? 3 : 2) : 0), NW, a.H, a.W, a.CinK, a.CoutS, nwg, s4[0] / nwg, s4[1] / nwg,
            s4[2] / nwg, s4[3] / nwg);
  }
}

bool launch_conv_fast(const ConvArgs& c, int th, hipStream_t st, bool dry) {
  if (c.H < th || c.W < 14) return false;
  if (c.in_mode == 2) {
    if (c.CinS != 1 || c.CoutS != 16 || th != 14) return false;
    FastArgs a;
    if (c.x2 != nullptr) return false;
    if (c.y_hi != nullptr) return false;
    if (c.x_up2) return false;
    a.x = (const unsigned char*)c.x; a.x2 = nullptr; a.y = (unsigned char*)c.y; a.y_hi = nullptr; a.wp = (const u32x4*)c.wp; a.stats = c.stats;
    a.up2 = 0;
    a.in_scale = a.in_shift = nullptr;
    a.y2 = nullptr; a.scale2 = a.shift2 = a.mean2 = nullptr; a.rows2 = nullptr; a.H2 = a.W2 = 0; a.img2 = nullptr;
    a.N = c.N; a.H = c.H; a.W = c.W; a.CinK = 16; a.CoutS = 16;
    static const int env_img_remap = lab_env("SPCL_IMAGE_XCD_REMAP", 1);
    a.tilesX = cdiv(c.W, 14); a.tilesY = cdiv(c.H, 14); a.gy = 1; a.xcd_remap = env_img_remap; a.lds_flip = 0; a.stamps = nullptr;
    a.acorr_rows = c.acorr_rows;
    a.img1 = nullptr; a.wp1 = nullptr; a.ipw = 1;
    a.stats_acc = a.rows2_acc = nullptr;
    a.in_bn = BnAccFwd{};
    if (c.stats_acc != nullptr || c.rows2_acc != nullptr || c.in_bn != nullptr) return false;
    if (c.acorr_rows != nullptr && !(c.H % 14 == 0 && c.W % 14 == 0)) return false;
    if (c.y == nullptr && !dry && c.acorr_rows == nullptr) return false;
    if (!dry) {
      if (c.acorr_rows != nullptr && c.y == nullptr) {
        a.ipw = (int)(((long)a.tilesX * a.tilesY * a.N + 4095) / 4096);
        a.ipw = a.ipw < 1 ? 1 : (a.ipw > a.N ? a.N : a.ipw);
        SPCL_LAUNCH((conv3x3_image_kernel<14, true, true, false>), dim3(a.tilesX, a.tilesY, cdiv(a.N, a.ipw)), dim3(64), 0, st, a);
      }
      else if (c.acorr_rows != nullptr) SPCL_LAUNCH((conv3x3_image_kernel<14, true, true>), dim3(a.tilesX, a.tilesY, a.N), dim3(64), 0, st, a);
      else if (c.H % 14 == 0 && c.W % 14 == 0) SPCL_LAUNCH((conv3x3_image_kernel<14, true>), dim3(a.tilesX, a.tilesY, a.N), dim3(64), 0, st, a);
      else SPCL_LAUNCH((conv3x3_image_kernel<14, false>), dim3(a.tilesX, a.tilesY, a.N), dim3(64), 0, st, a);
    }
    return true;
  }
  if (c.CinS != c.CinK) return false;
  const bool wants_acc = c.stats_acc != nullptr || c.rows2_acc != nullptr || c.in_bn != nullptr;
  const int ntn = c.CoutS / 16, KC = conv_kc(c.CinK);
  static const int env_nt1 = lab_env("SPCL_CONV_FAST_NT1", 0);
  int NT = ntn >= 2 ? 2 : 1;
  if (env_nt1 == 1 && KC == 64 && ntn == 2) NT = 1;
  if (env_nt1 != 2 && KC == 64 && ntn == 2 && c.rows2 != nullptr && c.H2 > 0) NT = 1;
  if (env_nt1 != 2 && KC == 64 && ntn == 2) NT = 1;
  if (KC == 64 && ntn == 4 && env_nt1 != 3 && (c.in_mode == 1 || c.H <= 28)) NT = 1;
  static const int env_wide = lab_env("SPCL_CONV_FAST_NT1_WIDE", 1);
  if (env_wide && KC == 64 && ntn == 4 && c.CinK > 64) NT = 1;
  static const int env_all4 = lab_env("SPCL_CONV_FAST_NT1_64", 1);
  if (env_all4 && KC == 64 && ntn == 4) NT = 1;
  static const int env_fill = lab_env("SPCL_CONV_FAST_FILL", 1);
  static const int env_fill_max = lab_env("SPCL_CONV_FAST_FILL_MAX", 512);
  if (env_fill && KC == 64 && NT == 2 && ntn >= 8 && ntn % 4 == 0 &&
      (long)c.N * cdiv(c.W, 14) * cdiv(c.H, th) * cdiv(ntn, 8) < env_fill_max)
    NT = 1;
  static const int env_narrow = lab_env("SPCL_CONV_FAST_NARROW_NT1", 2);
  if (env_narrow == 1 && KC < 64 && ntn == 2 && th == 7) NT = 1;
  if (env_narrow == 2 && KC == 32 && ntn == 2 && th == 7 && c.rows2 != nullptr && c.H2 == 0 && !c.y2_is_poolmax && c.img2 == nullptr)
    NT = 1;
  int nw = ntn / NT;
  if (nw > 4) nw = 4;
  if (ntn % (NT * nw) != 0) return false;
  FastArgs a;
  a.x = (const unsigned char*)c.x; a.y = (unsigned char*)c.y; a.wp = (const u32x4*)c.wp; a.stats = c.stats;
  a.x2 = (const unsigned char*)c.x2;
  a.y_hi = (unsigned char*)c.y_hi;
  a.up2 = c.x_up2 ? 1 : 0;
  if (c.x_up2 && !(c.in_mode == 0 && c.x2 == nullptr && c.rows2 == nullptr && c.img2 == nullptr && c.H % 2 == 0 &&
                   c.W % 2 == 0 && (double)c.N * c.H * c.W / 4.0 * c.CinK * 2.0 < 2147483648.0))
    return false;
  if (c.y_hi != nullptr && !(c.in_mode == 0 && (c.rows2 == nullptr || c.H2 == 0) && c.img2 == nullptr && c.stats == nullptr &&
                             ntn % 2 == 0))
    return false;
  if (c.x2 != nullptr && !(((c.CinK == KC && KC >= 32) || (KC == 64 && (c.CinK / 64) % 2 == 0)) && c.rows2 == nullptr &&
                           c.img2 == nullptr))
    return false;
  if (c.x2 != nullptr && c.in_mode == 1 && c.CinK != KC) return false;
  a.in_scale = c.in_scale; a.in_shift = c.in_shift;
  a.y2 = (const unsigned char*)c.y2; a.scale2 = c.scale2; a.shift2 = c.shift2; a.mean2 = c.mean2; a.rows2 = c.rows2;
  a.H2 = c.H2; a.W2 = c.W2;
  a.img2 = c.img2;
  a.acorr_rows = nullptr;
  a.img1 = c.img1; a.wp1 = (const u32x4*)c.wp1; a.ipw = 1;
  if (c.img1 != nullptr && !(c.in_mode == 1 && KC == 16 && th == 14 && ntn == 1 && c.x2 == nullptr && c.y_hi == nullptr &&
                             !c.x_up2 && c.rows2 == nullptr && c.img2 == nullptr && !wants_acc && c.H % 14 == 0 && c.W % 14 == 0 &&
                             (dry || (c.wp1 != nullptr && c.in_scale != nullptr && c.in_shift != nullptr))))
    return false;
  a.stats_acc = c.stats_acc;
  a.rows2_acc = c.rows2_acc;
  a.in_bn = c.in_bn != nullptr ? *c.in_bn : BnAccFwd{};
  if (wants_acc) {
    const long tiles = (long)c.N * cdiv(c.W, 14) * cdiv(c.H, th);
    if (c.y_hi != nullptr || c.img2 != nullptr) return false;
    if (c.stats_acc != nullptr && (c.rows2 != nullptr || tiles > BN_ACC_MAX_TILES_FWD)) return false;
    if (c.rows2_acc != nullptr && (c.rows2 == nullptr || tiles > BN_ACC_MAX_TILES_BWD)) return false;
    if (c.in_bn != nullptr && !(c.in_mode == 1 && KC == 64 && c.x2 == nullptr && c.in_bn->CS == c.CinK &&
                                (c.CinK * 4 == 64 * nw || c.CinK * 2 == 64 * nw || c.CinK == 64 * nw)))
      return false;
  }
  if (c.rows2 != nullptr && c.in_mode != 0) return false;
  if (c.img2 != nullptr && !(c.rows2 != nullptr && c.H2 == 0 && KC == 16 && th == 14 && ntn == 1)) return false;
  a.N = c.N; a.H = c.H; a.W = c.W; a.CinK = c.CinK; a.CoutS = c.CoutS;
  a.tilesX = cdiv(c.W, 14); a.tilesY = cdiv(c.H, th); a.gy = ntn / (NT * nw);
  static const int env_remap = lab_env("SPCL_CONV_XCD_REMAP", 1);
  a.xcd_remap = (env_remap && a.gy == 1) ? 1 : 0;
  if (c.rows2 != nullptr && c.H2 > 0 && KC == 64 && nw == 1) return false;
#define SPCL_FAST_CASE(KC_, TH_, NT_, NW_)                               \
  if (KC == KC_ && th == TH_ && NT == NT_ && nw == NW_) {                \
    if (!dry) launch_fast<KC_, TH_, NT_, NW_>(a, c.img1 != nullptr ? 8 : c.in_mode, st); \
    return true;                                                         \
  }
  SPCL_FAST_CASE(16, 14, 1, 1)
  SPCL_FAST_CASE(16, 14, 2, 1)
  SPCL_FAST_CASE(32, 14, 1, 1)
  SPCL_FAST_CASE(16, 7, 2, 1)
  SPCL_FAST_CASE(16, 7, 1, 2)
  SPCL_FAST_CASE(32, 7, 1, 2)
  SPCL_FAST_CASE(32, 7, 1, 1)
  SPCL_FAST_CASE(32, 7, 2, 1)
  SPCL_FAST_CASE(32, 7, 2, 2)
  SPCL_FAST_CASE(64, 7, 2, 1)
  SPCL_FAST_CASE(64, 7, 1, 2)
  SPCL_FAST_CASE(64, 7, 2, 2)
  SPCL_FAST_CASE(64, 7, 1, 4)
  SPCL_FAST_CASE(64, 7, 2, 4)
#undef SPCL_FAST_CASE
  return false;
}

}
```

self-paced-contrastive-learning_amd/functional.py:

```python
from __future__ import annotations

import ctypes
import math
import os
from ctypes import c_double, c_float, c_int

import torch

from . import native as _n

SP_NONE, SP_HARD, SP_SOFT = 0, 1, 2


def take_grad_sink(param, needed: bool = True):
    if not needed or param is None:
        return None
    sink = getattr(param, "_grad_sink", None)
    if sink is None or not getattr(param, "_grad_sink_armed", False):
        return None
    if sink.shape != param.shape or sink.dtype != torch.float32 or not sink.is_contiguous() or sink.device != param.device:
        return None
    param._grad_sink_armed = False
    return sink

# ... 944 lines not shown
    _EVAL_AFFINE.clear()


def prepare_eval_affines(bns):
    _EVAL_AFFINE.clear()
    bns = [bn for bn in bns if bn.running_mean is not None and bn.running_mean.is_cuda and bn.weight is not None]
    for i in range(0, len(bns), _n.BN_EVAL_MAX):
        part = bns[i:i + _n.BN_EVAL_MAX]
        dev = part[0].running_mean.device
        sizes = [_ru16(bn.num_features) for bn in part]
        buf = torch.empty(4 * sum(sizes), dtype=torch.float32, device=dev)
        items, keep, off = [], [], 0
        for bn, cs in zip(part, sizes):
            g, b = bn.weight.detach().contiguous().float(), bn.bias.detach().contiguous().float()
            st = buf[off:off + 4 * cs].view(4, cs)
            off += 4 * cs
            items.append(_n.BnEvalItem(g.data_ptr(), b.data_ptr(), bn.running_mean.data_ptr(), bn.running_var.data_ptr(),
                                       st.data_ptr(), bn.num_features, cs, float(bn.eps)))
            keep.append((g, b))
            _EVAL_AFFINE[(bn.running_mean.data_ptr(), cs)] = st
        arr = (_n.BnEvalItem * len(items))(*items)
        _n.call("spcl_bn_eval_affine_multi", arr, len(items), _n.stream())


def prepack_weights(layers, dtype, image=None):
    _PREPACKED.clear()
    _PREPACKED_ACORR.clear()
    if not _PREPACK or not layers:
        return
    dtc = _n.dtype_code(dtype)
    dev = layers[0][0].device
    sizes = []
    for w, H, W in layers:
        co, ci = w.shape[0], w.shape[1]
        sizes.append((_n.call("spcl_conv_packed_elems", ci, co, 0, dtc), _n.call("spcl_conv_packed_elems", ci, co, 1, dtc)))
    for i in range(0, len(layers), _n.PACK_MULTI_MAX):
        part, psz = layers[i:i + _n.PACK_MULTI_MAX], sizes[i:i + _n.PACK_MULTI_MAX]
        buf = torch.empty(sum(a + b for a, b in psz), dtype=dtype, device=dev)
        items, keep, off = [], [], 0
        for (w, H, W), (n0, n1) in zip(part, psz):
            wc = w.detach().contiguous().float()
            p0, p1 = buf[off:off + n0], buf[off + n0:off + n0 + n1]
            off += n0 + n1
            items.append(_n.PackItem(wc.data_ptr(), p0.data_ptr(), p1.data_ptr(), w.shape[1], w.shape[0],
                                     int(H) if _PACK_AT else 0, int(W) if _PACK_AT else 0))
            keep.append(wc)
            _PREPACKED[(w.data_ptr(), w._version, dtc, int(H), int(W))] = (p0, p1)
        arr = (_n.PackItem * len(items))(*items)
        if image is not None and i == 0 and _acorr_in_conv_rows(dtc, *[int(v) for v in image.shape[:3]]) > 0:
            image = None
        zero = _acc_arena_take_dirty(dev) if i == 0 else None
        zbytes = ctypes.c_size_t(zero.numel() * 8 if zero is not None else 0)
        if image is not None and i == 0:
            N, H, W = int(image.shape[0]), int(image.shape[1]), int(image.shape[2])
            acorr = torch.empty(_n.call("spcl_image_autocorr_rows", N, H, W), 64, dtype=torch.float32, device=dev)
            _n.call("spcl_conv_pack_weights_multi_zero", arr, len(items), dtc, _n.ptr(image), N, H, W, _n.ptr(acorr),
                    _n.ptr(zero), zbytes, _n.stream())
            _PREPACKED_ACORR[(image.data_ptr(), image._version)] = acorr
        else:
            _n.call("spcl_conv_pack_weights_multi_zero", arr, len(items), dtc, None, 0, 0, 0, None, _n.ptr(zero), zbytes,
                    _n.stream())


def _acorr_in_conv_rows(dt_code, N, H, W, cin=1, cout_s=16):
    return _n.call("spcl_conv3x3_forward_image_acorr_rows", dt_code, N, H, W, cin, cout_s)


def _conv_image_acorr(x_store, dt_code, dtype, N, H, W, cin_s, cout_s, wp, want_stats, rows, store=True):
    dev = x_store.device
    y = torch.empty(N, H, W, cout_s, dtype=dtype, device=dev) if store else None
    stats = None
    if want_stats:
        nt = _n.call("spcl_conv_stat_rows", dt_code, N, H, W, 16, cout_s)
        stats = torch.empty(_n.call("spcl_bn_stats_elems", nt, cout_s), dtype=torch.float32, device=dev)
        stats.ntiles = nt
    acorr = torch.empty(rows, 64, dtype=torch.float32, device=dev)
    _n.call("spcl_conv3x3_forward_image_acorr", _n.ptr(x_store), dt_code, N, H, W, cin_s, cout_s, _n.ptr(wp), _n.ptr(y),
            _n.ptr(stats), _n.ptr(acorr), _n.stream())
    return y, stats, acorr


_BLOCK1_RECOMPUTE = os.environ.get("SPCL_BLOCK1_RECOMPUTE", "1") != "0"
_BLOCK1_POOLED_BWD = os.environ.get("SPCL_BLOCK1_POOLED_BWD", "1") != "0"


def _conv_from_image(image, y_image, dt_code, dtype, N, H, W, cout_s, wp_image, scale, shift, wp, want_stats):
    dev = image.device
    y = torch.empty(N, H, W, cout_s, dtype=dtype, device=dev)
    stats = None
    if want_stats:
        nt = N * (H // 14) * (W // 14)
        stats = torch.empty(_n.call("spcl_bn_stats_elems", nt, cout_s), dtype=torch.float32, device=dev)
        stats.ntiles = nt
    _n.call("spcl_conv3x3_forward_from_image", _n.ptr(image), _n.ptr(y_image), dt_code, N, H, W, cout_s, _n.ptr(wp_image),
            _n.ptr(scale), _n.ptr(shift), _n.ptr(wp), _n.ptr(y), _n.ptr(stats), _n.stream())
    return y, stats


def take_prepacked(w, dtc, H, W):
    return _PREPACKED.pop((w.data_ptr(), w._version, dtc, int(H), int(W)), None)


def _conv(x_store, dt_code, dtype, N, H, W, cin_s, cin_k, cout_s, wp, in_mode, scale, shift, want_stats):
    dev = x_store.device
    y = torch.empty(N, H, W, cout_s, dtype=dtype, device=dev)
    stats = None
    if want_stats:
        nt = _n.call("spcl_conv_stat_rows", dt_code, N, H, W, cin_k, cout_s)
        stats = torch.empty(_n.call("spcl_bn_stats_elems", nt, cout_s), dtype=torch.float32, device=dev)
        stats.ntiles = nt
    _n.call("spcl_conv3x3_forward", _n.ptr(x_store), dt_code, N, H, W, cin_s, cin_k, cout_s, _n.ptr(wp), in_mode,
            _n.ptr(scale), _n.ptr(shift), _n.ptr(y), _n.ptr(stats), _n.stream())
    return y, stats


def _conv_cat(xa, xb, dt_code, dtype, N, H, W, chalf, cout_s, wp, want_stats, xb_scale=None, xb_shift=None):
    dev = xa.device
    y = torch.empty(N, H, W, cout_s, dtype=dtype, device=dev)
    stats = None
    if want_stats:
        nt = _n.call("spcl_conv_stat_rows", dt_code, N, H, W, 2 * chalf, cout_s)
        stats = torch.empty(_n.call("spcl_bn_stats_elems", nt, cout_s), dtype=torch.float32, device=dev)
        stats.ntiles = nt
    _n.call("spcl_conv3x3_forward_cat", _n.ptr(xa), _n.ptr(xb), dt_code, N, H, W, chalf, cout_s, _n.ptr(wp),
            _n.ptr(xb_scale), _n.ptr(xb_shift), _n.ptr(y), _n.ptr(stats), _n.stream())
    return y, stats


_BN_ACC = os.environ.get("SPCL_BN_ACC", "1") != "0"
_ACC_ARENA = {"buf": None, "off": 0, "used": 0, "need": 0, "dirty": False}


def bn_acc_arena_begin(device):
    a = _ACC_ARENA
    a["need"], a["used"], a["off"] = a["used"], 0, 0
    a["buf"] = torch.empty(a["need"], dtype=torch.int64, device=device) if (a["need"] > 0 and _BN_ACC) else None
    a["dirty"] = a["buf"] is not None


def _acc_arena_take_dirty(device):
    a = _ACC_ARENA
    if a["dirty"] and a["buf"] is not None and a["buf"].device == device:
        a["dirty"] = False
        return a["buf"]
    return None


def bn_acc_block(cs, device):
    words = _n.call("spcl_bn_acc_elems", int(cs))
    a = _ACC_ARENA
    buf = a["buf"]
    if buf is not None and a["dirty"]:
        buf.zero_()
        a["dirty"] = False
    if buf is None or buf.device != device or a["off"] + words > buf.numel():
        buf = a["buf"] = torch.zeros(max(words, 1 << 15), dtype=torch.int64, device=device)
        a["off"] = 0
    blk = buf[a["off"]:a["off"] + words]
    a["off"] += words
    a["used"] += words
    return blk


def _bn_acc_desc(acc, cfg: "BlockCfg", C, cs, gamma, beta, which, count, st, keep):
    g, b = gamma.detach().contiguous().float(), beta.detach().contiguous().float()
    rm, rv, nbt = cfg.buffers[which]
# ... 344 lines not shown
                    0 if acorr is None else acorr.shape[0], _n.ptr(rows.acorr16) if rows.wg else None, _n.stream())
            return
        _n.call("spcl_conv16_bwd_fused" if y2 is not None else "spcl_conv16_bwd_fused_image", _n.ptr(dy), dt_code, N, H, W,
                _n.ptr(wp_t), _n.ptr(y2 if y2 is not None else wp_image), _n.ptr(st2[2]),
                _n.ptr(st2[3]), _n.ptr(st2[0]), _n.ptr(image), _n.ptr(rows) if not rows.wg else None, _n.ptr(ws), _n.ptr(dw),
                cin, cout, _n.ptr(rows) if rows.wg else None, _n.ptr(acorr), 0 if acorr is None else acorr.shape[0],
                _n.ptr(rows.acorr16) if rows.wg else None, _n.stream())

    queue = sink_queue(sink)
    if queue is not None and _TAILS:
        if queue.capture_tail(sink, (ws, image, dy, y2, rows, wp_image, pooled), launch):
            return None, rows
        return dw, rows
    launch()
    return dw, rows


def _bnrelu_bwd_rows_image3(rows, acorr, w, N, H, W, C, cs, st, training, sinks):
    dev = rows.device
    ws = torch.empty(_n.call("spcl_bnrelu_image3_workspace_bytes", cs) // 4, dtype=torch.float32, device=dev)
    dw = _grad_buffer(sinks[0], (C, 1, 3, 3), dev)
    dgamma, dbeta = _grad_buffer(sinks[1], (C,), dev), _grad_buffer(sinks[2], (C,), dev)
    wc = w.detach().contiguous().float()
    if getattr(rows, "wg", 0):
        _n.call("spcl_bnrelu_backward_wgrows_image3", _n.ptr(rows), rows.wg, _n.ptr(rows.acorr16), 16, _n.ptr(wc), N, H, W, C,
                cs, _n.ptr(st[0]), _n.ptr(st[1]), _n.ptr(st[2]), int(training), _n.ptr(ws), _n.ptr(dgamma), _n.ptr(dbeta),
                _n.ptr(dw), _n.stream())
        return dw, dgamma, dbeta
    _n.call("spcl_bnrelu_backward_rows_image3", _n.ptr(rows), rows.ntiles, _n.ptr(acorr), acorr.shape[0], _n.ptr(wc), N, H,
            W, C, cs, _n.ptr(st[0]), _n.ptr(st[1]), _n.ptr(st[2]), int(training), _n.ptr(ws), _n.ptr(dgamma), _n.ptr(dbeta),
            _n.ptr(dw), _n.stream())
    return dw, dgamma, dbeta


def _bnrelu_pool_bwd_rows(y, dpool, rows, dt_code, dtype, N, H, W, C, cs, st, training, sinks):
    dev = y.device
    ws = torch.empty(_n.call("spcl_bnrelu_bwd_workspace_bytes", N, H, W, cs) // 4, dtype=torch.float32, device=dev)
    dgamma = _grad_buffer(sinks[0], (C,), dev)
    dbeta = _grad_buffer(sinks[1], (C,), dev)
    dy = torch.empty(N, H, W, cs, dtype=dtype, device=dev)
    _n.call("spcl_bnrelu_pool_backward_rows", _n.ptr(y), _n.ptr(dpool), _n.ptr(rows), rows.ntiles, dt_code, N, H, W, C, cs,
            _n.ptr(st[0]), _n.ptr(st[1]), _n.ptr(st[2]), _n.ptr(st[3]), int(training), _n.ptr(ws), _n.ptr(dgamma),
            _n.ptr(dbeta), _n.ptr(dy), _n.stream())
    return dy, dgamma, dbeta


ACC_ROWS = object()


def _bnrelu_bwd_fill(y, dact, dpool, dt_code, dtype, N, H, W, C, cs, st, training, sinks, acc, dact_stride=0, d_up=None):
    dev = y.device
    dgamma = _grad_buffer(sinks[0], (C,), dev)
    dbeta = _grad_buffer(sinks[1], (C,), dev)
    dy = torch.empty(N, H, W, cs, dtype=dtype, device=dev)
    if d_up is not None:
        assert dact is None and dpool is None
        dact = torch.empty(N, H, W, cs, dtype=dtype, device=dev)
    _n.call("spcl_bnrelu_backward_fill_acc", _n.ptr(y), _n.ptr(dact), int(dact_stride), _n.ptr(dpool), _n.ptr(d_up), dt_code,
            N, H, W, C, cs, _n.ptr(st), int(training), _n.ptr(acc), _n.ptr(dgamma), _n.ptr(dbeta), _n.ptr(dy), _n.stream())
    return dy, dgamma, dbeta


def _bnrelu_bwd_rows_acc(y, dact, dpool, rows, dt_code, dtype, N, H, W, C, cs, st, training, sinks, acc):
    dev = y.device
    dgamma = _grad_buffer(sinks[0], (C,), dev)
    dbeta = _grad_buffer(sinks[1], (C,), dev)
    dy = torch.empty(N, H, W, cs, dtype=dtype, device=dev)
    _n.call("spcl_bnrelu_backward_rows_acc", _n.ptr(y), _n.ptr(dact), _n.ptr(dpool), _n.ptr(rows), rows.ntiles, dt_code, N, H, W,
            C, cs, _n.ptr(st), int(training), _n.ptr(acc), _n.ptr(dgamma), _n.ptr(dbeta), _n.ptr(dy), _n.stream())
    return dy, dgamma, dbeta


def _take_acc(ctx, name):
    acc = getattr(ctx, name, None)
    setattr(ctx, name, None)
    return acc


def _dgrad_bnstats_acc(dy, wp_t, y2, st2, dt_code, dtype, N, H, W, cin_k, cout_s, acc):
    g = torch.empty(N, H, W, cout_s, dtype=dtype, device=dy.device)
    _n.call("spcl_conv3x3_dgrad_bnstats_acc", _n.ptr(dy), dt_code, N, H, W, cin_k, cout_s, _n.ptr(wp_t), _n.ptr(g), _n.ptr(y2),
            _n.ptr(st2[2]), _n.ptr(st2[3]), _n.ptr(st2[0]), _n.ptr(acc), _n.stream())
    return g


def _bnrelu_bwd_acc(y, dact, dpool, dact_nc, dt_code, dtype, N, H, W, C, cs, st, training, sinks, acc):
    dev = y.device
    dgamma = _grad_buffer(sinks[0], (C,), dev)
    dbeta = _grad_buffer(sinks[1], (C,), dev)
    dy = torch.empty(N, H, W, cs, dtype=dtype, device=dev)
    assert st.is_contiguous() and tuple(st.shape) == (4, cs)
    _n.call("spcl_bnrelu_backward_acc", _n.ptr(y), _n.ptr(dact), _n.ptr(dpool), _n.ptr(dact_nc), dt_code, N, H, W, C, cs,
            _n.ptr(st), int(training), _n.ptr(acc), _n.ptr(dgamma), _n.ptr(dbeta), _n.ptr(dy), _n.stream())
    return dy, dgamma, dbeta


class _ConvBlockFn(torch.autograd.Function):

    @staticmethod
    def forward(ctx, x, wa, ga, ba, wb, gb, bb, cfg: BlockCfg, x2=None):
        _n.require_gpu(x, wa, wb)
        dtype, dev = cfg.dtype, x.device
        dtc = _n.dtype_code(dtype)
        N, cin, H, W = x.shape
        cout = wa.shape[0]
        cout_s = _ru16(cout)
        x2s = None
        if x2 is not None:
            xs, x2s = to_nhwc_padded(x.detach(), dtype), to_nhwc_padded(x2.detach(), dtype)
            assert not cfg.image_input and x2.shape == x.shape and xs.shape[3] == cin and x2s.shape[3] == cin \
                and wa.shape[1] == 2 * cin, (tuple(x.shape), tuple(x2.shape), tuple(wa.shape))
            chalf, cin = cin, 2 * cin
            cin_s = cin_k = cin
            mode_a = 0
            xl = getattr(cfg, "x2_link", None)
            if xl is not None:
                assert xl.yb.data_ptr() == x2s.data_ptr() and xl.cs == chalf, "x2 is not the linked producer's output"
            ctx.x2_coef = (xl.stb[2], xl.stb[3]) if xl is not None else (None, None)
        elif cfg.image_input:
            if cin > 16:
                raise NotImplementedError("image-input block supports input_dim <= 16")
            xs = x.detach().float().permute(0, 2, 3, 1).contiguous()
            cin_s, cin_k, mode_a = cin, 16, 2
        else:
            xs = to_nhwc_padded(x.detach(), dtype)
            cin_s = cin_k = xs.shape[3]
            mode_a = 0
        need_bwd = any(ctx.needs_input_grad)
        ctx.acorr = None
        acorr_rows = 0
        if (need_bwd and ctx.needs_input_grad[1] and not ctx.needs_input_grad[0]
                and _image3_supported(cfg, cin, dtc, N, H, W, cout_s)):
            ctx.acorr = take_prepacked_acorr(xs)
            acorr_rows = _acorr_in_conv_rows(dtc, N, H, W, cin, cout_s) if (ctx.acorr is None and x2s is None) else 0
            if ctx.acorr is None and acorr_rows == 0:
                ctx.acorr = _image_autocorr(xs, N, H, W)
        pre_a, pre_b = take_prepacked(wa, dtc, H, W), take_prepacked(wb, dtc, H, W)
        if pre_a is not None and pre_b is not None:
            (wpa, wpa_t), (wpb, wpb_t) = pre_a, pre_b
        elif need_bwd:
            (wpa, wpa_t), (wpb, wpb_t) = _pack_block(wa, wb, dtc, dtype, *((H, W) if _PACK_AT else (0, 0)))
        else:
            wpa, wpb, wpa_t, wpb_t = _pack(wa, 0, dtc, dtype), _pack(wb, 0, dtc, dtype), None, None
        ctx.up2 = bool(getattr(cfg, "up2", False)) and cfg.need_act and not cfg.need_pool
        lazy = (bool(getattr(cfg, "lazy_act", False)) and cfg.need_act and not cfg.need_pool and not ctx.up2
                and getattr(cfg, "act_dst", None) is None)
        count = float(N) * H * W
        acc_ok = _BN_ACC and cfg.training and dtype == torch.bfloat16 and cout_s <= 256 and cout == cout_s
        sup = lambda ci, co, kind, out: bool(_n.call("spcl_conv_bn_acc_supported", dtc, N, H, W, ci, co, kind, out))
        use_a = (acc_ok and x2s is None and acorr_rows == 0 and mode_a == 0 and sup(cin_k, cout_s, 0, 1)
                 and sup(cout_s, cout_s, 1, 0))
        use_b = (acc_ok and not lazy and not ctx.up2 and getattr(cfg, "act_dst", None) is None
                 and sup(cout_s, cout_s, 1 if use_a else 2, 1))
        keep = []
        recompute = False
        ctx.acc_bwd_a = ctx.acc_bwd_b = ctx.acc_rows_a = None
        if use_a:
            acc_a = bn_acc_block(cout_s, dev)
            ya, _ = _conv_acc(xs, dtc, dtype, N, H, W, cin_k, cout_s, wpa, None, None, None, acc_a, False)
            sta = torch.empty(4, cout_s, dtype=torch.float32, device=dev)
            bn_a = _bn_acc_desc(acc_a, cfg, cout, cout_s, ga, ba, 0, count, sta, keep)
        else:
            if x2s is not None:
                ya, sa = _conv_cat(xs, x2s, dtc, dtype, N, H, W, chalf, cout_s, wpa, cfg.training, *ctx.x2_coef)
            elif acorr_rows > 0:
                recompute = (_BLOCK1_RECOMPUTE and _CONV16_FUSED and cfg.training and not use_b and cin == 1
# ... 48 lines not shown
            else:
                _n.call("spcl_bnrelu_pool_forward_acc", _n.ptr(yb), dtc, N, H, W, cout_s, ctypes.byref(bn_b), _n.ptr(act),
                        _n.ptr(pool), _n.stream())
        elif lazy:
            act, pool = yb, None
            cfg.link_act = ActLink(yb, stb, N, H, W, cout, cout_s)
        elif ctx.up2:
            act = torch.empty(N, 2 * H, 2 * W, cout_s, dtype=dtype, device=dev)
            pool = None
            _n.call("spcl_bnrelu_up2_forward", _n.ptr(yb), dtc, N, H, W, cout_s, _n.ptr(stb[2]), _n.ptr(stb[3]), _n.ptr(act),
                    _n.stream())
        else:
            act = _act_buffer(cfg, N, H, W, cout_s, dtype, dev) if cfg.need_act else None
            pool = torch.empty(N, H // 2, W // 2, cout_s, dtype=dtype, device=dev) if cfg.need_pool else None
            if want_ymax:
                ymax = torch.empty_like(pool)
                _n.call("spcl_bnrelu_pool_forward_ymax", _n.ptr(yb), dtc, N, H, W, cout_s, _n.ptr(stb[2]), _n.ptr(stb[3]), None,
                        None, _n.ptr(pool), _n.ptr(ymax), _n.stream())
            else:
                _bnrelu_fwd(yb, dtc, N, H, W, cout_s, stb[2], stb[3], act, pool)
        ctx.save_for_backward(xs, ya, yb, sta, stb, wa, wb)
        ctx.x2s = x2s
        ctx.params = (wa, ga, ba, wb, gb, bb)
        ctx.packed_t = (wpa_t, wpb_t)
        ctx.cfg = cfg
        if need_bwd and pool is not None and act is None and cfg.training and dtype == torch.bfloat16:
            cfg.link_out = PoolLink(yb, stb, N, H, W, cout_s, ctx.acc_bwd_b, ymax)
        ctx.meta = (N, cin, H, W, cout, cout_s, cin_s, cin_k, mode_a, x.dtype)
        outs = []
        outs.append(nhwc_to_logical(act, cout) if act is not None else None)
        outs.append(nhwc_to_logical(pool, cout) if pool is not None else None)
        return tuple(outs)

    @staticmethod
    def backward(ctx, d_act, d_pool):
        xs, ya, yb, sta, stb, wa, wb = ctx.saved_tensors
        cfg = ctx.cfg
        N, cin, H, W, cout, cout_s, cin_s, cin_k, mode_a, xdt = ctx.meta
        dtype = cfg.dtype
        dtc = _n.dtype_code(dtype)
        g_nc = broadcast_rows(d_act, dtype) if (_BCAST and d_pool is None and d_act is not None and not ctx.up2
                                                  and d_act.shape[1] == cout_s) else None
        d_up = None
        ul = getattr(cfg, "up_link", None)
        if ul is not None and ul.d_up is not None:
            du, holder = ul.d_up, ul.holder
            same = (d_act is not None and d_pool is None and d_act.data_ptr() == ul.dx_ptr and d_act.dtype == holder.dtype
                    and holder._version == ul.version and nhwc_channel_slice(d_act, dtype) is None
                    and to_nhwc_padded(d_act, dtype).data_ptr() == ul.dx_ptr)
            dirty = holder._version != ul.version
            ul.d_up, ul.dx_ptr, ul.holder = None, 0, None
            if same:
                d_up, d_act = du, None
            else:
                gs = torch.empty(N, H, W, cout_s, dtype=dtype, device=du.device)
                _n.call("spcl_upsample2x_backward", _n.ptr(du), _n.ptr(gs), dtc, N, H, W, cout_s, _n.stream())
                gl = nhwc_to_logical(gs, cout)
                d_act = gl if d_act is None else d_act.to(gl.dtype) + gl
                if dirty:
                    holder.zero_()
        elif ctx.up2 and d_act is not None:
            du = to_nhwc_padded(d_act, dtype)
            if _UP2_BWD_FUSED and d_pool is None:
                d_up, d_act = du, None
            else:
                dsum = torch.empty(N, H, W, cout_s, dtype=dtype, device=du.device)
                _n.call("spcl_upsample2x_backward", _n.ptr(du), _n.ptr(dsum), dtc, N, H, W, cout_s, _n.stream())
                d_act = nhwc_to_logical(dsum, cout)
        da_stride = 0
        da_sl = nhwc_channel_slice(d_act, dtype) if (d_act is not None and g_nc is None) else None
        if da_sl is not None:
            da_s, da_stride = da_sl
        else:
            da_s = to_nhwc_padded(d_act, dtype) if (d_act is not None and g_nc is None) else None
        dp_s = to_nhwc_padded(d_pool, dtype) if d_pool is not None else None
        if da_s is None and dp_s is None and g_nc is None and d_up is None:
            return (None,) * 9
        x2s = ctx.x2s
        ng = ctx.needs_input_grad
        sk = tuple(take_grad_sink(p, ng[i + 1]) for i, p in enumerate(ctx.params))
        lk = cfg.link_out
        la = getattr(cfg, "link_act", None)
        pooled = None
        if la is not None and da_s is not None and dp_s is None and da_stride == 0 and la.fresh(da_s.data_ptr()):
            dyb, dgb, dbb = _bnrelu_bwd_rows(yb, da_s, None, la.rows, dtc, dtype, N, H, W, cout, cout_s, stb, cfg.training,
                                             sk[4:6])
        elif g_nc is not None:
            acc = _take_acc(ctx, "acc_bwd_b")
            if acc is not None:
                dyb, dgb, dbb = _bnrelu_bwd_acc(yb, None, None, g_nc, dtc, dtype, N, H, W, cout, cout_s, stb, cfg.training,
                                                sk[4:6], acc)
            else:
                dyb, dgb, dbb = _bnrelu_bwd_bcast(yb, g_nc, dtc, dtype, N, H, W, cout, cout_s, stb, cfg.training, sk[4:6])
        elif lk is not None and da_s is None and dp_s is not None and lk.fresh(dp_s.data_ptr()):
            if lk.rows is ACC_ROWS:
                dyb, dgb, dbb = _bnrelu_bwd_acc(yb, None, dp_s, None, dtc, dtype, N, H, W, cout, cout_s, stb, cfg.training,
                                                sk[4:6], _take_acc(ctx, "acc_bwd_b"))
            else:
                acc = _take_acc(ctx, "acc_bwd_b") if (_ACC_FILL and H % 2 == 0 and W % 2 == 0 and cout_s <= 256) else None
                if (acc is not None and _BLOCK1_POOLED_BWD and ya is None and ctx.acorr is not None and ctx.wpa_fwd is not None
                        and ctx.needs_input_grad[4] and cout == cout_s and dtype == torch.bfloat16
                        and _n.call("spcl_conv16_bwd_fused_image_pooled_supported", dtc, N, H, W, cout_s, cout_s,
                                    int(cfg.training))):
                    dyb = None
                    dgb, dbb = _grad_buffer(sk[4], (cout,), yb.device), _grad_buffer(sk[5], (cout,), yb.device)
                    pooled = (yb, dp_s, lk.rows, stb, acc, dgb.view(cout), dbb.view(cout), cfg.training)
                elif acc is not None:
                    dyb, dgb, dbb = _bnrelu_bwd_rows_acc(yb, None, dp_s, lk.rows, dtc, dtype, N, H, W, cout, cout_s, stb,
                                                         cfg.training, sk[4:6], acc)
                else:
                    dyb, dgb, dbb = _bnrelu_pool_bwd_rows(yb, dp_s, lk.rows, dtc, dtype, N, H, W, cout, cout_s, stb,
                                                          cfg.training, sk[4:6])
        else:
            acc = _take_acc(ctx, "acc_bwd_b") if _ACC_FILL else None
            if acc is not None and lk is not None and lk.rows is ACC_ROWS:
                acc = None
            if acc is not None:
                dyb, dgb, dbb = _bnrelu_bwd_fill(yb, da_s, dp_s, dtc, dtype, N, H, W, cout, cout_s, stb, cfg.training, sk[4:6],
                                                 acc, dact_stride=da_stride, d_up=d_up)
            else:
                dyb, dgb, dbb = _bnrelu_bwd(yb, da_s, dp_s, dtc, dtype, N, H, W, cout, cout_s, stb, cfg.training, sk[4:6],
                                            dact_stride=da_stride, d_up=d_up)
        if lk is not None:
            lk.rows, lk.dx_ptr, lk.holder = None, 0, None
        if la is not None:
            la.rows, la.dx_ptr, la.holder = None, 0, None
        wpa_t, wpb_t = ctx.packed_t
        if wpb_t is None:
            wpb_t = _pack(wb, 1, dtc, dtype)
        image3 = ctx.acorr is not None
        one_pass = (image3 and (_CONV16_FUSED or ya is None) and ctx.needs_input_grad[4] and cout == cout_s
                    and _n.call("spcl_conv16_bwd_fused_supported", dtc, N, H, W, cout_s, cout_s))
        if ya is None and not one_pass:
            raise RuntimeError("image block backward: the first convolution's output was not stored and the one-pass kernel "
                               "that forms it again is not available")
        if pooled is not None and not one_pass:
            raise RuntimeError("image block backward: the gradient behind the max-pool was not materialised and the one-pass "
                               "kernel that forms it is not available")
        if one_pass:
            dwb, rows16 = _conv16_bwd_fused(dyb, wpb_t, ya, sta, xs, dtc, N, H, W, cout, cout, cout_s, sk[3],
                                            acorr=ctx.acorr if _CONV16_WGROWS else None, wp_image=ctx.wpa_fwd, pooled=pooled)
        else:
            dwb = _wgrad(ya, dyb, dtc, N, H, W, cout, cout_s, cout_s, cout, cout_s, 1, sta[2], sta[3], sk[3]) \
                if ctx.needs_input_grad[4] else None
        if one_pass:
            fused = (None, rows16)
        elif image3:
            fused = _dgrad_bnstats_image(dyb, wpb_t, ya, sta, xs, dtc, dtype, N, H, W, cout_s)
        else:
            acc = _take_acc(ctx, "acc_bwd_a")
            if acc is not None:
                fused = (_dgrad_bnstats_acc(dyb, wpb_t, ya, sta, dtc, dtype, N, H, W, cout_s, cout_s, acc), (ACC_ROWS, acc))
            else:
                fused = _dgrad_bnstats(dyb, wpb_t, ya, sta, dtc, dtype, N, H, W, cout_s, cout_s) \
                    if dtype == torch.bfloat16 else None
        if fused is not None:
            daa, rows = fused
        else:
            daa, _ = _conv(dyb, dtc, dtype, N, H, W, cout_s, cout_s, cout_s, wpb_t, 0, None, None, False)
        image_fused = ctx.needs_input_grad[1] and not ctx.needs_input_grad[0] and _image_wgrad_fusable(cfg, cin, cout_s)
        if image3:
            dya = None
            dwa, dga, dba = _bnrelu_bwd_rows_image3(rows, ctx.acorr, wa, N, H, W, cout, cout_s, sta, cfg.training, sk[0:3])
        elif image_fused:
            dya = None
            if fused is not None:
                dwa, dga, dba = _bnrelu_bwd_rows(ya, daa, xs, rows, dtc, dtype, N, H, W, cout, cout_s, sta, cfg.training,
                                                 sk[0:3])
            else:
                dwa, dga, dba = _bnrelu_bwd_image_wgrad(ya, daa, xs, dtc, N, H, W, cout, cout_s, sta, cfg.training,
                                                        sk[0:3])
        else:
            if fused is not None and isinstance(rows, tuple) and rows[0] is ACC_ROWS:
                dya, dga, dba = _bnrelu_bwd_acc(ya, daa, None, None, dtc, dtype, N, H, W, cout, cout_s, sta, cfg.training,
                                                sk[1:3], rows[1])
            elif fused is not None:
                acc = _take_acc(ctx, "acc_rows_a")
                if acc is not None:
                    dya, dga, dba = _bnrelu_bwd_rows_acc(ya, daa, None, rows, dtc, dtype, N, H, W, cout, cout_s, sta,
                                                         cfg.training, sk[1:3], acc)
                else:
                    dya, dga, dba = _bnrelu_bwd_rows(ya, daa, None, rows, dtc, dtype, N, H, W, cout, cout_s, sta,
                                                     cfg.training, sk[1:3])
            else:
                dya, dga, dba = _bnrelu_bwd(ya, daa, None, dtc, dtype, N, H, W, cout, cout_s, sta, cfg.training,
                                            sk[1:3])
            if not ctx.needs_input_grad[1]:
                dwa = None
            elif x2s is not None:
                dwa = _wgrad_cat(xs, x2s, dya, dtc, N, H, W, cin // 2, cout, cout_s, sk[0], *ctx.x2_coef)
            else:
                dwa = _wgrad(xs, dya, dtc, N, H, W, cin, cin_s, cin_k, cout, cout_s, mode_a, None, None, sk[0])
        dx = dx2 = None
        if ctx.needs_input_grad[0] or (x2s is not None and ctx.needs_input_grad[8]):
            if cfg.image_input:
                raise NotImplementedError("gradient w.r.t. the input image is not on the hot path")
            if wpa_t is None:
                wpa_t = _pack(wa, 1, dtc, dtype)
            li = cfg.link_in
            dxs = None
            if (li is not None and dtype == torch.bfloat16 and li.cout_s == cin_s and li.N == N
                    and _n.call("spcl_conv_dgrad_poolstats_supported", dtc, N, H, W, cout_s, cin_s, li.H, li.W)):
                dxs = torch.empty(N, H, W, cin_s, dtype=dtype, device=dya.device)
                ym = li.ymax if (li.ymax is not None and tuple(li.ymax.shape) == (N, H, W, cin_s)) else None
                if (li.acc is not None and _n.call("spcl_conv_dgrad_poolstats_acc_supported", dtc, N, H, W, cout_s, cin_s,
                                                   li.H, li.W)):
                    acc_in, li.acc = li.acc, None
                    if ym is not None and _n.call("spcl_conv_dgrad_poolmax_acc_supported", dtc, N, H, W, cout_s, cin_s):
                        _n.call("spcl_conv3x3_dgrad_poolmax_acc", _n.ptr(dya), dtc, N, H, W, cout_s, cin_s, _n.ptr(wpa_t),
                                _n.ptr(dxs), _n.ptr(ym), _n.ptr(li.stb[2]), _n.ptr(li.stb[3]), _n.ptr(li.stb[0]),
                                _n.ptr(acc_in), _n.stream())
                    else:
                        _n.call("spcl_conv3x3_dgrad_poolstats_acc", _n.ptr(dya), dtc, N, H, W, cout_s, cin_s, _n.ptr(wpa_t),
                                _n.ptr(dxs), _n.ptr(li.yb), li.H, li.W, _n.ptr(li.stb[2]), _n.ptr(li.stb[3]),
                                _n.ptr(li.stb[0]), _n.ptr(acc_in), _n.stream())
                    rows = ACC_ROWS
                else:
                    nt = _n.call("spcl_conv_stat_rows", dtc, N, H, W, cout_s, cin_s)
                    rows = torch.empty(nt * 2 * cin_s, dtype=torch.float32, device=dya.device)
                    if ym is not None and _n.call("spcl_conv_dgrad_poolmax_supported", dtc, N, H, W, cout_s, cin_s):
                        _n.call("spcl_conv3x3_dgrad_poolmax", _n.ptr(dya), dtc, N, H, W, cout_s, cin_s, _n.ptr(wpa_t),
                                _n.ptr(dxs), _n.ptr(ym), _n.ptr(li.stb[2]), _n.ptr(li.stb[3]), _n.ptr(li.stb[0]),
                                _n.ptr(rows), _n.stream())
                    else:
                        _n.call("spcl_conv3x3_dgrad_poolstats", _n.ptr(dya), dtc, N, H, W, cout_s, cin_s, _n.ptr(wpa_t),
                                _n.ptr(dxs), _n.ptr(li.yb), li.H, li.W, _n.ptr(li.stb[2]), _n.ptr(li.stb[3]),
                                _n.ptr(li.stb[0]), _n.ptr(rows), _n.stream())
                    rows.ntiles = nt
                li.rows, li.dx_ptr, li.holder, li.version = rows, dxs.data_ptr(), dxs, dxs._version
                li.ymax = None
            split = None
# ... 1527 lines not shown
```

self-paced-contrastive-learning_amd/native.py:

```python
from __future__ import annotations

import ctypes
import os
from ctypes import c_char_p, c_double, c_float, c_int, c_long, c_size_t, c_void_p

import torch

HERE = os.path.dirname(os.path.abspath(__file__))
LIB_PATH = os.path.join(HERE, "lib", "libspcl_hip.so")
SPCL_F32, SPCL_BF16 = 0, 1

_lib = None

_P = c_void_p
_SIGNATURES = {
    "spcl_abi_version": (c_int, []),
    "spcl_last_error": (c_char_p, []),
    "spcl_supcon_workspace_bytes": (c_size_t, [c_int, c_int]),
    "spcl_supcon_forward": (c_int, [_P, _P, _P, _P, c_int, c_int, c_float, c_int, c_float, c_int, _P, _P, _P]),
    "spcl_supcon_backward": (c_int, [_P, _P, c_int, c_int, c_float, c_int, c_float, _P, _P, _P, _P, _P, _P, _P]),
    "spcl_supcon_bwd_workspace_bytes": (c_size_t, [c_int, c_int]),
    "spcl_supcon_unit_gradient_block": (c_int, [c_int, c_int, _P, _P]),
    "spcl_supcon_materialize": (c_int, [_P, _P, c_int, c_int, c_float, c_int, c_float, _P, _P, _P, _P, _P, _P, _P]),
    "spcl_supcon_xpos_workspace_bytes": (c_size_t, [c_int, c_int]),
# ... 119 lines not shown
                                                 c_int, _P, _P, _P, _P, _P]),
    "spcl_conv1x1_forward": (c_int, [_P, c_int, c_size_t, c_int, c_int, c_int, _P, _P, _P, _P]),
    "spcl_conv1x1_bwd_workspace_bytes": (c_size_t, [c_int, c_int]),
    "spcl_conv1x1_backward": (c_int, [_P, _P, c_int, c_size_t, c_int, c_int, c_int, _P, _P, _P, _P, _P, _P]),
    "spcl_conv1x1_forward_bn": (c_int, [_P, c_int, c_size_t, c_int, c_int, c_int, _P, _P, _P, _P, _P, _P]),
    "spcl_conv1x1_bwd_rows": (c_int, [c_size_t]),
    "spcl_conv1x1_backward_bn": (c_int, [_P, _P, c_int, c_size_t, c_int, c_int, c_int, _P, _P, _P, _P, _P, _P, _P, _P, _P, _P]),
    "spcl_softmax_forward": (c_int, [_P, c_size_t, c_int, _P, _P]),
    "spcl_softmax_backward": (c_int, [_P, _P, c_size_t, c_int, _P, _P]),
    "spcl_kl_workspace_bytes": (c_size_t, []),
    "spcl_kl_div_forward": (c_int, [_P, _P, c_size_t, c_int, c_float, _P, _P, _P]),
    "spcl_kl_div_backward": (c_int, [_P, _P, c_size_t, c_int, c_float, _P, _P, _P]),
    "spcl_sup_loss_forward": (c_int, [_P, _P, c_int, c_int, c_int, c_float, _P, _P, _P, _P, _P, _P]),
    "spcl_one_hot": (c_int, [_P, c_size_t, c_int, _P, _P]),
    "spcl_argmax_classes": (c_int, [_P, c_size_t, c_int, _P, _P]),
    "spcl_dice_counts": (c_int, [_P, _P, c_int, c_int, c_int, _P, _P, _P]),
    "spcl_surface_workspace_bytes": (c_size_t, [c_int, c_int, c_int, c_int]),
    "spcl_surface_distances": (c_int, [_P, _P, c_int, c_int, c_int, c_int, _P, c_int, c_double, c_double, c_double, _P, _P, _P,
                                       _P, _P, c_size_t, _P]),
    "spcl_surface_3d_workspace_bytes": (c_size_t, [c_int, c_int, c_int, c_int, c_int]),
    "spcl_surface_distances_3d": (c_int, [_P, _P, c_int, c_int, c_int, c_int, c_int, _P, c_int, c_double, c_double, c_double,
                                          c_double, _P, _P, _P, _P, _P, c_size_t, _P]),
    "spcl_largest_component_workspace_bytes": (c_size_t, [c_int, c_int, c_int, c_int, c_int]),
    "spcl_largest_component": (c_int, [_P, c_int, c_int, c_int, c_int, c_int, _P, c_int, _P, _P, _P, _P, c_size_t, _P]),
    "spcl_upsample2x_forward": (c_int, [_P, _P, c_int, c_int, c_int, c_int, c_int, _P]),
    "spcl_upsample2x_backward": (c_int, [_P, _P, c_int, c_int, c_int, c_int, c_int, _P]),
    "spcl_concat2_channels": (c_int, [_P, _P, _P, c_int, c_size_t, c_int, c_int, _P]),
    "spcl_split2_channels": (c_int, [_P, _P, _P, c_int, c_size_t, c_int, c_int, _P]),
    "spcl_augment_views": (c_int, [_P, c_int, c_int, c_int, _P, c_int, _P, c_int, c_int, _P]),
    "spcl_augment_views_recipe": (c_int, [_P, _P, c_int, c_int, c_int, _P, c_int, _P, _P, c_int, c_int, c_int, _P]),
    "spcl_augment_views_recipe_workspace_bytes": (c_size_t, [c_int, c_int, c_int]),
    "spcl_rows_linear_forward": (c_int, [_P, c_int, c_long, c_int, _P, _P, c_int, c_int, c_int, _P, _P]),
    "spcl_rows_linear_forward_act": (c_int, [_P, c_int, c_long, _P, _P, c_int, c_int, c_int, _P, c_int, _P]),
    "spcl_adaptive_avgpool2d_backward_act": (c_int, [_P, _P, c_int, c_int, c_int, c_int, c_int, c_int, c_int, _P, _P]),
    "spcl_rows_linear_backward_input": (c_int, [_P, c_int, _P, _P, c_int, c_int, c_int, _P, c_int, c_long, _P]),
    "spcl_rows_linear_backward_weight_workspace_bytes": (c_size_t, [c_int, c_int, c_int]),
    "spcl_rows_linear_backward_weight": (c_int, [_P, c_int, _P, c_int, c_long, c_int, c_int, c_int, c_int, _P, c_size_t, _P, _P, _P]),
    "spcl_augment_views_recipe_ws": (c_int, [_P, _P, c_int, c_int, c_int, _P, c_int, _P, _P, c_int, c_int, c_int, _P, c_size_t,
                                             _P]),
    "spcl_resize_bilinear_pil": (c_int, [_P, c_int, c_int, c_int, _P, _P, c_int, _P, _P, c_int, _P, _P, c_int, c_int, _P]),
    "spcl_resize_nearest_pil": (c_int, [_P, c_int, c_int, c_int, _P, _P, _P, c_int, c_int, _P]),
    "spcl_augment_views_pil": (c_int, [_P, c_int, c_int, c_int, _P, c_int, _P, c_int, c_int, _P]),
    "spcl_flip_batch": (c_int, [_P, _P, c_int, c_int, c_int, c_int, c_int, _P, _P]),
    "spcl_flip_pair": (c_int, [_P, _P, _P, c_int, c_int, c_int, c_int, c_int, _P, _P]),
    "spcl_flip_pair_stage": (c_int, [_P, _P, _P, c_int, c_int, c_int, c_int, c_int, _P, _P, c_size_t, c_size_t, _P]),
    "spcl_profile_enable": (c_int, [c_int]),
    "spcl_profile_count": (c_int, []),
    "spcl_profile_get": (c_int, [c_int, c_char_p, c_int, _P, _P, _P]),
    "spcl_radam_step": (c_int, [_P, _P, _P, _P, c_size_t, _P, _P, c_double, c_double, c_double, c_double, _P, _P]),
    "spcl_radam_step_scalars": (c_int, [_P, _P, _P, _P, c_size_t, _P, _P, c_double, c_double, c_double, c_double, _P,
                                        c_int, _P, _P, _P, _P]),
    "spcl_radam_step_scaled": (c_int, [_P, _P, c_double, _P, _P, c_size_t, _P, _P, c_double, c_double, c_double, c_double,
                                       _P, c_int, _P, _P, _P, _P]),
    "spcl_bnrelu_gap_supported": (c_int, [c_int, c_int, c_int, c_int, c_int]),
    "spcl_bnrelu_gap_forward": (c_int, [_P, c_int, c_int, c_int, c_int, c_int, c_int, _P, _P, _P, _P, _P, _P]),
    "spcl_bnrelu_backward_fill_acc": (c_int, [_P, _P, c_int, _P, _P, c_int, c_int, c_int, c_int, c_int, c_int, _P, c_int, _P, _P,
                                              _P, _P, _P]),
    "spcl_copy_pair": (c_int, [_P, _P, c_size_t, _P, _P, c_size_t, _P]),
    "spcl_bnrelu_backward_rows_acc": (c_int, [_P, _P, _P, _P, c_int, c_int, c_int, c_int, c_int, c_int, c_int, _P, c_int, _P, _P,
                                              _P, _P, _P]),
    "spcl_radam_apply_staged": (c_int, [_P, _P, c_double, _P, _P, c_size_t, _P, _P, c_double, c_double, c_double, c_double,
                                        c_int, _P, _P, _P, _P]),
    "spcl_adam_step_scaled": (c_int, [_P, _P, c_double, _P, _P, c_size_t, _P, _P, c_double, c_double, c_double, c_double,
                                      c_int, _P, c_int, _P, _P, _P, _P]),
    "spcl_adam_apply_staged": (c_int, [_P, _P, c_double, _P, _P, c_size_t, _P, _P, c_double, c_double, c_double, c_double,
                                       c_int, c_int, _P, _P, _P, _P]),
    "spcl_sgd_step_scaled": (c_int, [_P, _P, c_double, _P, c_size_t, _P, _P, c_double, c_double, c_double, c_int, _P, c_int,
                                     _P, _P, _P, _P]),
    "spcl_sgd_apply_staged": (c_int, [_P, _P, c_double, _P, c_size_t, _P, _P, c_double, c_double, c_double, c_int, c_int, _P,
                                      _P, _P, _P]),
    "spcl_bn_acc_elems": (c_size_t, [c_int]),
    "spcl_conv_bn_acc_supported": (c_int, [c_int, c_int, c_int, c_int, c_int, c_int, c_int, c_int]),
    "spcl_conv3x3_forward_acc": (c_int, [_P, c_int, c_int, c_int, c_int, c_int, c_int, _P, _P, _P, _P, _P, _P, _P, _P]),
    "spcl_bnrelu_pool_forward_acc": (c_int, [_P, c_int, c_int, c_int, c_int, c_int, _P, _P, _P, _P]),
    "spcl_conv_dgrad_bnstats_acc_supported": (c_int, [c_int, c_int, c_int, c_int, c_int, c_int]),
    "spcl_conv3x3_dgrad_bnstats_acc": (c_int, [_P, c_int, c_int, c_int, c_int, c_int, c_int, _P, _P, _P, _P, _P, _P, _P, _P]),
    "spcl_conv_dgrad_poolstats_acc_supported": (c_int, [c_int, c_int, c_int, c_int, c_int, c_int, c_int, c_int]),
    "spcl_conv3x3_dgrad_poolstats_acc": (c_int, [_P, c_int, c_int, c_int, c_int, c_int, c_int, _P, _P, _P, c_int, c_int, _P,
                                                 _P, _P, _P, _P]),
    "spcl_bnrelu_pool_forward_ymax": (c_int, [_P, c_int, c_int, c_int, c_int, c_int, _P, _P, _P, _P, _P, _P, _P]),
    "spcl_conv_dgrad_poolmax_supported": (c_int, [c_int, c_int, c_int, c_int, c_int, c_int]),
    "spcl_conv3x3_dgrad_poolmax": (c_int, [_P, c_int, c_int, c_int, c_int, c_int, c_int, _P, _P, _P, _P, _P, _P, _P, _P]),
    "spcl_conv_dgrad_poolmax_acc_supported": (c_int, [c_int, c_int, c_int, c_int, c_int, c_int]),
    "spcl_conv3x3_dgrad_poolmax_acc": (c_int, [_P, c_int, c_int, c_int, c_int, c_int, c_int, _P, _P, _P, _P, _P, _P, _P, _P]),
    "spcl_bnrelu_backward_acc": (c_int, [_P, _P, _P, _P, c_int, c_int, c_int, c_int, c_int, c_int, _P, c_int, _P, _P, _P, _P,
                                         _P]),
    "spcl_iic_joint_workspace_bytes": (c_size_t, [c_int, c_int, c_int]),
    "spcl_iic_joint_forward": (c_int, [_P, _P, c_long, c_int, c_int, c_int, c_int, c_int, c_int, _P, _P, _P]),
    "spcl_iic_loss_workspace_bytes": (c_size_t, [c_int, c_int]),
    "spcl_iic_loss": (c_int, [_P, _P, c_int, c_int, c_int, c_int, c_float, _P, _P, _P, _P, _P, c_size_t, _P]),
    "spcl_iic_joint_backward": (c_int, [_P, _P, c_long, c_int, c_int, c_int, c_int, c_int, c_int, _P, _P, _P, _P, _P, _P]),
    "spcl_consistency_workspace_bytes": (c_size_t, [c_int, c_int, c_int]),
    "spcl_consistency_softmax_mse": (c_int, [_P, _P, c_int, c_int, c_int, c_int, _P, c_float, _P, _P, _P, c_size_t, _P]),
    "spcl_iic_patch_plan": (c_int, [c_int, c_int, c_int, c_int, c_int, c_int, _P, _P, _P]),
    "spcl_iic_patch_forward": (c_int, [_P, _P, c_int, c_int, c_int, c_int, c_int, c_int, _P, c_float, _P, _P, _P, _P, _P,
                                       c_size_t, _P]),
    "spcl_iic_patch_backward": (c_int, [_P, _P, c_int, c_int, c_int, c_int, c_int, c_int, _P, _P, _P, _P, _P, _P]),
    "spcl_iic_patch_heads_plan": (c_int, [c_int, c_int, c_int, c_long, c_int, c_int, c_int, c_int, _P, _P, _P]),
    "spcl_iic_patch_heads_forward": (c_int, [_P, _P, c_long, c_int, c_int, c_int, c_int, c_int, c_int, c_int, _P, c_float, _P,
                                             _P, _P, _P, _P, c_size_t, _P]),
    "spcl_iic_patch_heads_backward": (c_int, [_P, _P, c_long, c_int, c_int, c_int, c_int, c_int, c_int, c_int, _P, _P, _P, _P,
                                              _P, _P]),
    "spcl_ema_update": (c_int, [_P, _P, c_size_t, c_double, c_double, _P]),
    "spcl_mt_softmax_mse_workspace_bytes": (c_size_t, [c_int, c_int, c_int]),
    "spcl_mt_softmax_mse": (c_int, [_P, _P, c_int, c_int, c_int, c_int, _P, c_int, c_float, _P, _P, _P, c_size_t, _P]),
    "spcl_entropy_softmax_workspace_bytes": (c_size_t, [c_int, c_int, c_int]),
    "spcl_entropy_softmax": (c_int, [_P, c_int, c_int, c_int, c_int, c_float, c_float, _P, _P, _P, c_size_t, _P]),
    "spcl_ucmt_workspace_bytes": (c_size_t, [c_int, c_int, c_int]),
    "spcl_ucmt_softmax_mse": (c_int, [_P, _P, c_int, _P, c_int, c_int, c_int, c_int, _P, c_float, c_float, c_float, _P, _P, _P,
                                      _P, _P, c_size_t, _P]),
    "spcl_mixup_images": (c_int, [_P, _P, _P, c_int, c_size_t, c_float, c_float, _P, _P]),
    "spcl_mixup_kl_workspace_bytes": (c_size_t, [c_int, c_int, c_int]),
    "spcl_mixup_kl_onehot": (c_int, [_P, _P, _P, _P, c_int, c_int, c_int, c_int, c_float, c_float, c_float, c_float, _P, _P, _P,
                                     c_size_t, _P]),
    "spcl_patch4s2_rows_forward": (c_int, [_P, c_int, c_long, c_long, c_long, c_long, _P, c_int, c_long, c_long, c_long, c_long,
                                           c_int, c_int, c_int, c_int, _P, _P, _P, _P]),
    "spcl_patch4s2_rows_backward": (c_int, [_P, _P, c_int, c_int, c_int, c_int, c_int, c_int, _P, _P, _P, _P]),
    "spcl_rows_bn_workspace_bytes": (c_size_t, [c_int, c_int]),
    "spcl_rows_bn_forward": (c_int, [_P, c_int, c_int, _P, _P, c_float, c_float, _P, _P, _P, _P, c_size_t, _P]),
    "spcl_rows_bn_eval_affine": (c_int, [_P, _P, _P, _P, c_float, c_int, _P, _P]),
    "spcl_rows_bn_backward": (c_int, [_P, _P, c_int, c_int, _P, _P, c_int, _P, _P, _P, _P, c_size_t, _P]),
    "spcl_discr_head_workspace_bytes": (c_size_t, [c_int, c_int, c_int, c_int]),
    "spcl_discr_head_forward": (c_int, [_P, c_int, c_int, c_int, c_int, _P, _P, _P, c_int, _P, _P, _P, _P, _P, c_size_t, _P]),
    "spcl_discr_head_backward": (c_int, [_P, c_int, c_int, c_int, c_int, _P, _P, _P, _P, _P, _P, _P, _P, c_size_t, _P]),
    "spcl_mine_pairs_forward": (c_int, [_P, _P, c_int, c_int, c_int, c_int, c_int, _P, _P, _P]),
    "spcl_mine_pairs_backward": (c_int, [_P, _P, _P, c_int, c_int, c_int, c_int, c_int, _P, _P]),
    "spcl_mine_head_workspace_bytes": (c_size_t, [c_int, c_int, c_int, c_int]),
    "spcl_mine_head_forward": (c_int, [_P, _P, c_int, c_int, c_int, c_int, c_int, _P, _P, _P, _P, _P, _P, _P, c_size_t, _P]),
    "spcl_mine_head_backward": (c_int, [_P, _P, _P, _P, _P, c_int, c_int, c_int, c_int, c_int, _P, _P, _P, _P, _P]),
    "spcl_pica_workspace_bytes": (c_size_t, [c_int]),
    "spcl_pica_seg_loss": (c_int, [_P, _P, c_int, c_int, c_int, c_double, c_float, _P, _P, _P, _P, _P, c_size_t, _P]),
    "spcl_pica_global_loss": (c_int, [_P, _P, c_long, c_int, c_int, c_int, c_float, c_float, _P, _P, _P, _P, _P, _P, c_size_t,
                                      _P]),
}


class WgradItem(ctypes.Structure):
    _fields_ = [("x", c_void_p), ("dy", c_void_p), ("in_scale", c_void_p), ("in_shift", c_void_p),
                ("dw_oihw", c_void_p), ("N", c_int), ("H", c_int), ("W", c_int), ("Cin", c_int), ("CinS", c_int),
                ("Cout", c_int), ("CoutS", c_int), ("in_mode", c_int), ("x2", c_void_p), ("x_up2", c_int)]


class PackItem(ctypes.Structure):
    _fields_ = [("w_oihw", c_void_p), ("fwd", c_void_p), ("dgrad", c_void_p), ("Cin", c_int), ("Cout", c_int),
                ("H", c_int), ("W", c_int)]


BN_EVAL_MAX = 32


class BnEvalItem(ctypes.Structure):
    _fields_ = [("gamma", c_void_p), ("beta", c_void_p), ("running_mean", c_void_p), ("running_var", c_void_p),
                ("st", c_void_p), ("C", c_int), ("CS", c_int), ("eps", c_float)]


class BnAcc(ctypes.Structure):
    _fields_ = [("acc", c_void_p), ("gamma", c_void_p), ("beta", c_void_p), ("running_mean", c_void_p),
                ("running_var", c_void_p), ("num_batches_tracked", c_void_p), ("st", c_void_p), ("momentum", c_float),
                ("eps", c_float), ("count", c_float), ("C", c_int), ("CS", c_int)]


PACK_MULTI_MAX = 24


class WgradTail(ctypes.Structure):
    _fields_ = [("partial", c_void_p), ("dw", c_void_p), ("kind", c_int), ("nsplit", c_int), ("nblk_ci", c_int),
                ("nblk_co", c_int), ("CIB", c_int), ("COB", c_int), ("Cin", c_int), ("Cout", c_int)]


ABI_VERSION = 27
WGRAD_BATCH_MAX = 16
WGRAD_TAILS_MAX = 16
_NO_STATUS = ("spcl_abi_version", "spcl_block1_recompute_supported", "spcl_block1_kernels_take", "spcl_conv16_bwd_fused_image_supported", "spcl_conv3x3_forward_image_acorr_rows", "spcl_image_autocorr_rows", "spcl_conv_dgrad_bnstats_image_supported", "spcl_conv16_bwd_fused_supported", "spcl_conv16_bwd_fused_splits", "spcl_conv_num_tiles", "spcl_conv_stat_rows", "spcl_conv_set_gemm", "spcl_conv_set_f32_split", "spcl_conv_get_f32_split", "spcl_supcon_unit_gradient_block", "spcl_conv_cat_supported", "spcl_conv_up2_supported", "spcl_conv_split_supported", "spcl_conv_split_bnstats_supported", "spcl_conv1x1_bwd_rows", "spcl_profile_count", "spcl_conv_dgrad_bnstats_supported", "spcl_conv_dgrad_poolstats_supported",
              "spcl_conv_wgrad_batched_supported", "spcl_conv_bn_acc_supported", "spcl_conv_dgrad_bnstats_acc_supported",
              "spcl_conv_dgrad_poolstats_acc_supported", "spcl_supcon_rows_supported", "spcl_bnrelu_gap_supported",
              "spcl_conv_dgrad_poolmax_supported", "spcl_conv_dgrad_poolmax_acc_supported",
              "spcl_conv16_bwd_fused_image_pooled_supported")


class NativeLibraryError(RuntimeError):
    pass


def lib():
    global _lib
    if _lib is None:
        if not os.path.exists(LIB_PATH):
            raise NativeLibraryError(
                f"{LIB_PATH} is missing: build it with `python self-paced-contrastive-learning_amd/build.py` "
                "(there is no CPU / eager fallback for the hot path)")
        L = ctypes.CDLL(LIB_PATH)
        L.spcl_abi_version.restype, L.spcl_abi_version.argtypes = c_int, []
        have = L.spcl_abi_version()
        if have != ABI_VERSION:
            raise NativeLibraryError(
                f"{LIB_PATH} has C-ABI version {have}, this binding was written for {ABI_VERSION} (include/spcl_hip.h "
                "SPCL_ABI_VERSION): a stale build -- rebuild with `python self-paced-contrastive-learning_amd/build.py`")
        for name, (res, args) in _SIGNATURES.items():
            fn = getattr(L, name, None)
            if fn is None:
                continue
            fn.restype, fn.argtypes = res, args
        _lib = L
    return _lib


def call(name: str, *args):
    L = lib()
    fn = getattr(L, name, None)
    if fn is None:
        raise NativeLibraryError(f"libspcl_hip.so does not export {name}")
    rc = fn(*args)
    if fn.restype is c_int and name not in _NO_STATUS and rc != 0:
        raise RuntimeError(f"{name} failed ({rc}): {L.spcl_last_error().decode()}")
    return rc


def require_gpu(*tensors):
    for t in tensors:
        if t is None:
            continue
        if not t.is_cuda:
            raise RuntimeError("self-paced-contrastive-learning_amd runs on MI355X only: got a CPU tensor "
                               "(the HIP path has no CPU fallback)")


def ptr(t):
    return None if t is None else c_void_p(t.data_ptr())


def stream():
    return c_void_p(torch.cuda.current_stream().cuda_stream)


def ptr_array(tensors):
    return (c_void_p * len(tensors))(*[None if t is None else t.data_ptr() for t in tensors])


def dtype_code(dt: torch.dtype) -> int:
    if dt == torch.float32:
        return SPCL_F32
    if dt == torch.bfloat16:
        return SPCL_BF16
    raise TypeError(f"unsupported activation dtype {dt}")
```

Baseline: 32980 slices/s.

## Fuse pooled BN-ReLU backward into the following conv dgrad halo loader

Adds new conv dgrad modes that compute the BN+ReLU+maxpool backward (dy) on the fly inside the halo staging. They read y and dpool, reduce the BN backward sums in the block prologue, and write dy to global memory from the by==0 blocks so wgrad can use it later. This replaces a separate bnrelu_backward_acc launch and its round trip of dy through memory for channel counts of 128 and up. In exchange the halo loads lose their prefetch pipelining, every tile redoes the per-channel reduction of BN statistics, and register and LDS pressure go up.

After: 33370 slices/s, median of 3. No clear change (+1.2%).

```diff
diff --git a/include/spcl_hip.h b/include/spcl_hip.h
--- a/include/spcl_hip.h
+++ b/include/spcl_hip.h
@@ -14,7 +14,7 @@
 #define SPCL_ELAUNCH (-2)
 #define SPCL_EUNSUPPORTED (-3)
 
-#define SPCL_ABI_VERSION 27
+#define SPCL_ABI_VERSION 28
 int spcl_abi_version(void);
 const char* spcl_last_error(void);
 
@@ -446,6 +446,11 @@
 int spcl_conv3x3_dgrad_poolmax_acc(const void* dy, int dtype, int N, int H, int W, int CinK, int CoutS, const void* w_packed,
                                    void* g, const void* ymax, const float* scale2, const float* shift2, const float* mean2,
                                    long long* acc, void* stream);
+int spcl_conv_dgrad_pooldy_supported(int dtype, int N, int H, int W, int CinK, int CoutS, int training);
+int spcl_conv3x3_dgrad_pooldy_acc(const void* y_b, const void* dpool, int dtype, int N, int H, int W, int CinK, int CoutS,
+                                  const void* w_packed, void* g, const void* y2, const float* scale2, const float* shift2,
+                                  const float* mean2, float* rows2, long long* acc2, int C, const float* st_b, int training,
+                                  const long long* acc_b, float* dgamma, float* dbeta, void* dy, void* stream);
 int spcl_bnrelu_backward_acc(const void* y, const void* dact, const void* dpool, const void* dact_nc, int dtype, int N, int H,
                              int W, int C, int CS, const float* st4, int training, long long* acc, float* dgamma, float* dbeta,
                              void* dy, void* stream);
diff --git a/self-paced-contrastive-learning_amd/csrc/bn_acc.hpp b/self-paced-contrastive-learning_amd/csrc/bn_acc.hpp
--- a/self-paced-contrastive-learning_amd/csrc/bn_acc.hpp
+++ b/self-paced-contrastive-learning_amd/csrc/bn_acc.hpp
@@ -197,6 +197,23 @@
     f.dgamma[c] = s2;
   }
 }
+__device__ __forceinline__ void bn_acc_bwd_channel_sums(const BnAccBwd& f, const BnAccSums& sums, float mean, float invstd,
+                                                        float scale, int c, float& A, float& B, bool write) {
+  double t1, t2;
+  sums.totals(t1, t2);
+  const float s1 = (float)t1;
+  const float s2 = (float)t2 * invstd;
+  A = 0.f;
+  B = 0.f;
+  if (f.training) {
+    A = -scale * invstd * (s2 / f.count);
+    B = -scale * (s1 / f.count) - A * mean;
+  }
+  if (write && c < f.C) {
+    f.dbeta[c] = s1;
+    f.dgamma[c] = s2;
+  }
+}
 #endif
 
 }
diff --git a/self-paced-contrastive-learning_amd/csrc/conv.hip b/self-paced-contrastive-learning_amd/csrc/conv.hip
--- a/self-paced-contrastive-learning_amd/csrc/conv.hip
+++ b/self-paced-contrastive-learning_amd/csrc/conv.hip
@@ -1460,6 +1460,65 @@
   return SPCL_OK;
 }
 
+static bool dgrad_pooldy_dry(int dtype, int N, int H, int W, int CinK, int CoutS, bool acc2) {
+  ConvArgs a;
+  if (!dgrad_bnstats_args(a, dtype, N, H, W, CinK, CoutS) || conv_use_gemm(CinK, CoutS, H, W)) return false;
+  a.x = nullptr; a.y = nullptr; a.wp = nullptr;
+  float dummy;
+  long long dummy2;
+  a.rows2 = &dummy;
+  a.rows2_acc = acc2 ? &dummy2 : nullptr;
+  BnAccBwd bw{};
+  bw.CS = CinK;
+  const ConvPoolDy pool{nullptr, nullptr, &bw};
+  TileCfg t = pick_tile(H, W);
+  return t.tw == 14 && launch_conv_fast(a, t.th, nullptr, true, &pool);
+}
+
+extern "C" int spcl_conv_dgrad_pooldy_supported(int dtype, int N, int H, int W, int CinK, int CoutS, int training) {
+  (void)training;
+  if (dtype != SPCL_BF16 || H <= 0 || W <= 0 || H % 2 != 0 || W % 2 != 0) return 0;
+  if (!spcl_conv_dgrad_bnstats_supported(dtype, N, H, W, CinK, CoutS)) return 0;
+  return dgrad_pooldy_dry(dtype, N, H, W, CinK, CoutS, false) ? 1 : 0;
+}
+
+extern "C" int spcl_conv3x3_dgrad_pooldy_acc(const void* y_b, const void* dpool, int dtype, int N, int H, int W, int CinK,
+                                             int CoutS, const void* w_packed, void* g, const void* y2, const float* scale2,
+                                             const float* shift2, const float* mean2, float* rows2, long long* acc2, int C,
+                                             const float* st_b, int training, const long long* acc_b, float* dgamma,
+                                             float* dbeta, void* dy, void* stream) {
+  SPCL_CHECK_ARG(y_b && dpool && w_packed && g && y2 && scale2 && shift2 && mean2 && st_b && acc_b && dgamma && dbeta && dy,
+                 "conv3x3_dgrad_pooldy_acc: null pointer");
+  SPCL_CHECK_ARG((rows2 != nullptr) != (acc2 != nullptr), "conv3x3_dgrad_pooldy_acc: exactly one of rows2 / acc2");
+  SPCL_CHECK_ARG((uintptr_t)y_b % 16 == 0 && (uintptr_t)dpool % 16 == 0 && (uintptr_t)dy % 16 == 0 && (uintptr_t)acc_b % 16 == 0,
+                 "conv3x3_dgrad_pooldy_acc: tensors must be 16-byte aligned");
+  SPCL_CHECK_ARG(C > 0 && C <= CinK, "conv3x3_dgrad_pooldy_acc: 0 < C <= CinK");
+  SPCL_CHECK_ARG(dy != y_b && dy != g, "conv3x3_dgrad_pooldy_acc: dy must be a tensor of its own");
+  ConvArgs a;
+  if (!spcl_conv_dgrad_pooldy_supported(dtype, N, H, W, CinK, CoutS, training) ||
+      !dgrad_pooldy_dry(dtype, N, H, W, CinK, CoutS, acc2 != nullptr) || !dgrad_bnstats_args(a, dtype, N, H, W, CinK, CoutS)) {
+    set_error("conv3x3_dgrad_pooldy_acc: unsupported configuration (bf16, even H and W, 32 -> 32 / 64 -> 64 / 128 -> 128 "
+              "channels on 7 x 14 tiles, at most %d tiles)", BN_ACC_MAX_TILES_BWD);
+    return SPCL_EUNSUPPORTED;
+  }
+  const BnAccBwd bw{acc_b, st_b, dgamma, dbeta, (float)((size_t)N * H * W), training, C, CinK};
+  a.x = y_b; a.y = g; a.wp = w_packed;
+  a.y2 = y2; a.scale2 = scale2; a.shift2 = shift2; a.mean2 = mean2;
+  a.rows2 = acc2 != nullptr ? (float*)acc2 : rows2;
+  a.rows2_acc = acc2;
+  const ConvPoolDy pool{dpool, dy, &bw};
+  hipStream_t st = (hipStream_t)stream;
+  const double px = (double)N * H * W;
+  prof_cost(px * (2.25 * CinK + 2.0 * CoutS) * 2.0 + 9.0 * CinK * CoutS * 2.0, 2.0 * px * 9.0 * CinK * CoutS);
+  TileCfg t = pick_tile(H, W);
+  if (!(t.tw == 14 && launch_conv_fast(a, t.th, st, false, &pool))) {
+    set_error("conv3x3_dgrad_pooldy_acc: no specialised kernel for H=%d W=%d CinK=%d CoutS=%d", H, W, CinK, CoutS);
+    return SPCL_EUNSUPPORTED;
+  }
+  SPCL_LAUNCH_CHECK("conv3x3_dgrad_pooldy_acc");
+  return SPCL_OK;
+}
+
 extern "C" int spcl_conv_dgrad_bnstats_image_supported(int dtype, int N, int H, int W, int CinK, int CoutS) {
   static const bool off = lab_flag("SPCL_NO_IMAGE3");
   ConvArgs a;
diff --git a/self-paced-contrastive-learning_amd/csrc/conv_common.hpp b/self-paced-contrastive-learning_amd/csrc/conv_common.hpp
--- a/self-paced-contrastive-learning_amd/csrc/conv_common.hpp
+++ b/self-paced-contrastive-learning_amd/csrc/conv_common.hpp
@@ -4,6 +4,7 @@
 namespace spcl {
 
 struct BnAccFwd;
+struct BnAccBwd;
 template <typename T> struct Chunk;
 template <> struct Chunk<float> { static constexpr int EPC = 4; };
 template <> struct Chunk<bf16_t> { static constexpr int EPC = 8; };
@@ -53,6 +54,12 @@
   long long* stats_acc = nullptr;
   long long* rows2_acc = nullptr;
   const struct BnAccFwd* in_bn = nullptr;
+};
+
+struct ConvPoolDy {
+  const void* dpool;
+  void* dy;
+  const struct BnAccBwd* bw;
 };
 
 struct split_f32 { float v; };
@@ -160,7 +167,7 @@
   if (r16 < 3) *(f32x4*)(stats + ((size_t)tile * 3 + r16) * CoutS + cb) = o;
 }
 
-bool launch_conv_fast(const ConvArgs& a, int th, hipStream_t st, bool dry = false);
+bool launch_conv_fast(const ConvArgs& a, int th, hipStream_t st, bool dry = false, const ConvPoolDy* pool = nullptr);
 
 __host__ __device__ inline bool conv_gemm_channels(int CinK, int CoutS) {
   return CinK % 64 == 0 && CoutS % 64 == 0 && CinK >= 64 && CoutS >= 64 && (CinK >= 128 || CoutS >= 128);
diff --git a/self-paced-contrastive-learning_amd/csrc/conv_fast.hip b/self-paced-contrastive-learning_amd/csrc/conv_fast.hip
--- a/self-paced-contrastive-learning_amd/csrc/conv_fast.hip
+++ b/self-paced-contrastive-learning_amd/csrc/conv_fast.hip
@@ -3,8 +3,15 @@
 #include <vector>
 #include "bn_acc.hpp"
 #include "conv_common.hpp"
+#include "pool_dy.hpp"
 
 namespace spcl {
+
+struct FastPool {
+  const unsigned char* dpool;
+  unsigned char* dy_out;
+  BnAccBwd bw;
+};
 
 struct FastArgs {
   const unsigned char* x;
@@ -33,8 +40,13 @@
   float* acorr_rows;
   long long* stats_acc;
   long long* rows2_acc;
-  BnAccFwd in_bn;
+  union {
+    BnAccFwd in_bn;
+    FastPool p;
+  };
 };
+static_assert(sizeof(FastPool) <= sizeof(BnAccFwd) && alignof(FastPool) <= alignof(BnAccFwd), "FastArgs keeps its layout");
+
 
 #ifndef SPCL_FAST_WPE_NT1
 #define SPCL_FAST_WPE_NT1 2
@@ -135,7 +147,9 @@
 #endif
   const int gps = (KC < 64 ? KC : a.CinK) * 2;
 
-  constexpr bool M2 = MODE == 2 || MODE == 4;
+  constexpr bool PD = MODE == 9 || MODE == 10;
+  static_assert(!PD || (TH == 7 && KC >= 32), "pooled-dy loader: 7-row tiles of the 32 / 64-channel-slab kernels");
+  constexpr bool M2 = MODE == 2 || MODE == 4 || PD;
   constexpr bool M1 = MODE == 1 || (MODE >= 5 && MODE <= 7);
   constexpr bool M8 = MODE == 8;
   static_assert(!M8 || (KC == 16 && TH == 14 && NT == 1 && NW == 1), "MODE 8: the 16 -> 16 layer on 14 x 14 tiles, one wave");
@@ -195,8 +209,11 @@
   const int flip = a.lds_flip;
   const unsigned wvo = (unsigned)(nt0 * 64 + lane) * 16u;
   const size_t wstep = (size_t)ntn * 1024;
-  u32x4 v[ITER];
+  u32x4 v[PD ? 1 : ITER];
   float ssc[8], ssh[8];
+  constexpr int PD_WX = 9, PD_NWIN = ((TH + 3) / 2) * PD_WX, PD_IT = (PD_NWIN + QS - 1) / QS;
+  u32x4 pv[PD ? PD_IT : 1][PD ? 5 : 1];
+  const int pd_wr0 = (y0 - 1) & ~1, pd_wc0 = (x0 - 1) & ~1;
   constexpr int IW8 = 18;
   float imv8[M8 ? 6 : 1];
   s16x4 wfrag8 = {0, 0, 0, 0};
@@ -215,7 +232,80 @@
       *(f32x4*)&ssh[e] = *(const f32x4*)(coef_l + a.CinK + slab * KC + cc * 8 + e);
     }
   };
+  auto pool_item = [&](const int it, int& gy, int& gx) {
+    const int w = q0 + it * QS, wy = w / PD_WX, wx = w - wy * PD_WX;
+    gy = pd_wr0 + 2 * wy;
+    gx = pd_wc0 + 2 * wx;
+    return w < PD_NWIN && (interior || (gy >= 0 && gy < a.H && gx >= 0 && gx < a.W));
+  };
+  auto issue_pool = [&](const int slab) {
+    if constexpr (PD) {
+    const int HP = a.H >> 1, WP = a.W >> 1;
+    const unsigned char* ys = a.x + (size_t)n * a.H * a.W * gps + slab * (KC * 2) + ch * 16;
+    const unsigned char* ps = a.p.dpool + (size_t)n * HP * WP * gps + slab * (KC * 2) + ch * 16;
+    const size_t rowy = (size_t)a.W * gps;
+#pragma unroll
+    for (int it = 0; it < PD_IT; ++it) {
+      int gy, gx;
+      const bool in = pool_item(it, gy, gx);
+#pragma unroll
+      for (int j = 0; j < 5; ++j) pv[it][j] = (u32x4){0u, 0u, 0u, 0u};
+      if (in) {
+        const unsigned char* p = ys + ((size_t)gy * a.W + gx) * gps;
+        pv[it][0] = *(const u32x4*)p;
+        pv[it][1] = *(const u32x4*)(p + gps);
+        pv[it][2] = *(const u32x4*)(p + rowy);
+        pv[it][3] = *(const u32x4*)(p + rowy + gps);
+        pv[it][4] = *(const u32x4*)(ps + ((size_t)(gy >> 1) * WP + (gx >> 1)) * gps);
+      }
+    }
+    }
+  };
+  auto stage_pool = [&](const int sb, const int img_off) {
+    if constexpr (PD) {
+    const float* const cf = coef_l + sb * KC + ch * 8;
+    unsigned char* const ib = lds + img_off + ch * 16;
+    unsigned char* const dyb = a.p.dy_out + (size_t)n * a.H * a.W * gps + sb * (KC * 2) + ch * 16;
+#pragma unroll
+    for (int it = 0; it < PD_IT; ++it) {
+      int gy, gx;
+      const bool in = pool_item(it, gy, gx);
+      const u32x4* r = pv[it];
+      u32x4 out[4];
+#pragma unroll
+      for (int wi = 0; wi < 4; ++wi) {
+        const f32x2 cS = *(const f32x2*)(cf + 2 * wi), cH = *(const f32x2*)(cf + a.CinK + 2 * wi);
+        const f32x2 cA = *(const f32x2*)(cf + 2 * a.CinK + 2 * wi), cB = *(const f32x2*)(cf + 3 * a.CinK + 2 * wi);
+        float o[4][2];
+#pragma unroll
+        for (int h = 0; h < 2; ++h) {
+          SPCL_POOL_WINDOW_DY(bf16_t, r, r[4], wi, h, cS[h], cH[h], cA[h], cB[h], o)
+        }
+#pragma unroll
+        for (int q = 0; q < 4; ++q) out[q][wi] = Word<bf16_t>::make(o[q]);
+      }
+      if (!in) {
+#pragma unroll
+        for (int q = 0; q < 4; ++q) out[q] = (u32x4){0u, 0u, 0u, 0u};
+      }
+      if (q0 + it * QS < PD_NWIN) {
+#pragma unroll
+        for (int q = 0; q < 4; ++q) {
+          const int hy = gy + (q >> 1) - (y0 - 1), hx = gx + (q & 1) - (x0 - 1);
+          if (hy >= 0 && hy < TH + 2 && hx >= 0 && hx < HW_) {
+            *(u32x4*)(ib + (hy * RP + hx) * PS) = out[q];
+            if (by == 0 && hy >= 1 && hy <= TH && hx >= 1 && hx <= TW)
+              *(u32x4*)(dyb + ((size_t)(gy + (q >> 1)) * a.W + gx + (q & 1)) * gps) = out[q];
+          }
+        }
+      }
+    }
+    }
+  };
   auto issue_halo = [&](int slab, const bool first = false) {
+    if constexpr (PD) {
+      issue_pool(slab);
+    } else {
     if (acc_in) {
       if (!first) load_coef_lds(slab);
     } else if (M1) {
@@ -253,6 +343,7 @@
     if (a.up2) walk(std::true_type{}, std::false_type{});
     else if (interior) walk(std::false_type{}, std::true_type{});
     else walk(std::false_type{}, std::false_type{});
+    }
   };
   unsigned char* lpw = lp;
   auto slab_body = [&](const int slab, const bool refill) {
@@ -275,7 +366,8 @@
         if (in_range) *(u32x4*)(lpw + (dky * RP + dkx) * PS) = tv;
       }
     };
-    if constexpr (M8) {
+    if constexpr (PD) {
+    } else if constexpr (M8) {
       typedef uint32_t __attribute__((may_alias)) pair_t;
       typedef unsigned short __attribute__((may_alias)) half_t;
       const pair_t* const pairs = (const pair_t*)lds;
@@ -330,7 +422,7 @@
       for (int hy = 0; hy < TH + 2; ++hy) *(uint2*)(lds + (hy * RP + r16) * PS + g * 8) = hv[hy];
     } else if (M1 && !interior) stage(std::false_type{});
     else stage(std::true_type{});
-    if (refill) issue_halo(slab + 1);
+    if (refill && !PD) issue_halo(slab + 1);
     if (stamp && slab == 0) t_store = __builtin_amdgcn_s_memtime();
     __syncthreads();
     if (stamp && slab == 0) t_k0 = __builtin_amdgcn_s_memtime();
@@ -400,6 +492,18 @@
   if (acc_in && SPCL_ACC_DBG < 2) {
     accp.load(a.in_bn.acc, a.CinK, acc_c, acc_has ? ACC_RPT * acc_part : 0);
     accprm.load(a.in_bn, acc_c);
+  }
+  constexpr int PD_TPC = MODE == 9 ? 4 : 2, PD_RPT = BN_ACC_REPLICAS / PD_TPC;
+  static_assert(!PD || PD_RPT * PD_TPC == BN_ACC_REPLICAS, "pooled-dy prologue: the replicas split evenly");
+  const int pd_part = PD ? t / a.CinK : 0, pd_c = t - pd_part * a.CinK;
+  BnAccPart<PD ? PD_RPT : 1> pdp;
+  float pd_mean = 0.f, pd_invstd = 0.f, pd_scale = 0.f, pd_shift = 0.f;
+  if constexpr (PD) {
+    pdp.load(a.p.bw.acc, a.CinK, pd_c, PD_RPT * pd_part);
+    pd_mean = a.p.bw.st[pd_c];
+    pd_invstd = a.p.bw.st[a.CinK + pd_c];
+    pd_scale = a.p.bw.st[2 * a.CinK + pd_c];
+    pd_shift = a.p.bw.st[3 * a.CinK + pd_c];
   }
   if constexpr (M8) {
     const float* im = a.img1 + (size_t)n * a.H * a.W;
@@ -463,6 +567,37 @@
     }
     __syncthreads();
     load_coef_lds(0);
+  }
+  if constexpr (PD) {
+    const bool writer = (blockIdx.x | blockIdx.y | blockIdx.z) == 0;
+    BnAccSums sums = pdp.sums();
+    long long* const part_l = (long long*)(coef_l + 4 * a.CinK);
+    if (pd_part > 0) {
+      long long* q = part_l + ((size_t)(pd_part - 1) * a.CinK + pd_c) * 4;
+      *(i64x2*)q = (i64x2){sums.h1, sums.l1};
+      *(i64x2*)(q + 2) = (i64x2){sums.h2, sums.l2};
+    }
+    __syncthreads();
+    if (pd_part == 0) {
+#pragma unroll
+      for (int k = 1; k < PD_TPC; ++k) {
+        const long long* q = part_l + ((size_t)(k - 1) * a.CinK + pd_c) * 4;
+        const i64x2 u = *(const i64x2*)q, w = *(const i64x2*)(q + 2);
+        sums.h1 += u[0]; sums.l1 += u[1]; sums.h2 += w[0]; sums.l2 += w[1];
+      }
+      float ca, cb;
+      bn_acc_bwd_channel_sums(a.p.bw, sums, pd_mean, pd_invstd, pd_scale, pd_c, ca, cb, writer);
+      coef_l[pd_c] = pd_scale;
+      coef_l[a.CinK + pd_c] = pd_shift;
+      coef_l[2 * a.CinK + pd_c] = ca;
+      coef_l[3 * a.CinK + pd_c] = cb;
+    }
+    __syncthreads();
+#pragma unroll 1
+    for (int sb = 0; sb < nslab; ++sb) {
+      if (sb > 0) issue_pool(sb);
+      stage_pool(sb, sb * flip);
+    }
   }
   if (MODE == 4) {
     const int q = lane & 3;
@@ -689,7 +824,7 @@
   }
   constexpr int RS = MODE == 4 ? 11 : 2;
   const int replica = (int)((blockIdx.x + gridDim.x * (blockIdx.y + gridDim.y * blockIdx.z)) & (BN_ACC_REPLICAS - 1));
-  if ((MODE == 2 || MODE == 3) && a.rows2_acc != nullptr) {
+  if ((MODE == 2 || MODE == 3 || PD) && a.rows2_acc != nullptr) {
 #pragma unroll
     for (int j = 0; j < NT; ++j) {
       f32x4 s1, s2;
@@ -931,13 +1066,14 @@
 }
 
 template <int KC, int TH, int NT, int NW>
-static void launch_fast(const FastArgs& a, int mode, hipStream_t st) {
+static void launch_fast(const FastArgs& a, int mode, hipStream_t st, const FastPool* pool = nullptr) {
   static const int env_pipe = lab_env("SPCL_CONV_FAST_PIPE", 1);
   const bool pipe = env_pipe && KC == 64 && a.CinK > KC;
   FastArgs b = a;
   b.lds_flip = pipe ? fast_lds_bytes(KC, TH) : 0;
   const size_t lds = fast_lds_bytes(KC, TH) * (pipe ? 2 : 1) + (a.img2 != nullptr ? 1536 : 0) +
-                     (a.in_bn.acc != nullptr ? (size_t)a.CinK * 8 + (size_t)64 * NW * 32 : 0);
+                     (pool != nullptr ? (size_t)a.CinK * 16 + (size_t)64 * NW * 32
+                      : a.in_bn.acc != nullptr ? (size_t)a.CinK * 8 + (size_t)64 * NW * 32 : 0);
   dim3 grid(a.tilesX, a.tilesY, a.N * a.gy), block(64 * NW);
 #if SPCL_FAST_DBG & 4
   if (KC == 64 && a.CinK >= 128 && (long)a.tilesX * a.tilesY * a.N * a.gy <= 256) grid.z *= 2;
@@ -949,7 +1085,16 @@
     (void)hipMalloc(&b.stamps, nwg * 4 * sizeof(unsigned long long));
     (void)hipMemset(b.stamps, 0, nwg * 4 * sizeof(unsigned long long));
   }
-  if (a.img2 != nullptr) {
+  if (pool != nullptr) {
+    const int tpc = 64 * NW / a.CinK;
+    b.p = *pool;
+    if constexpr ((KC == 64 && NW == 4 && NT == 1) || (KC == 32 && NW == 2 && NT == 1)) {
+      if (tpc == 4) SPCL_LAUNCH((conv3x3_fast_kernel<KC, TH, NT, 9, NW>), grid, block, lds, st, b);
+    }
+    if constexpr (KC == 64 && NW == 4 && TH == 7) {
+      if (tpc == 2) SPCL_LAUNCH((conv3x3_fast_kernel<KC, TH, NT, 10, NW>), grid, block, lds, st, b);
+    }
+  } else if (a.img2 != nullptr) {
     if constexpr (KC == 16 && TH == 14 && NT == 1 && NW == 1)
       SPCL_LAUNCH((conv3x3_fast_kernel<KC, TH, NT, 4, NW>), grid, block, lds, st, b);
   } else if (mode == 8) {
@@ -981,7 +1126,7 @@
   }
 }
 
-bool launch_conv_fast(const ConvArgs& c, int th, hipStream_t st, bool dry) {
+bool launch_conv_fast(const ConvArgs& c, int th, hipStream_t st, bool dry, const ConvPoolDy* pool) {
   if (c.H < th || c.W < 14) return false;
   if (c.in_mode == 2) {
     if (c.CinS != 1 || c.CoutS != 16 || th != 14) return false;
@@ -1000,6 +1145,7 @@
     a.img1 = nullptr; a.wp1 = nullptr; a.ipw = 1;
     a.stats_acc = a.rows2_acc = nullptr;
     a.in_bn = BnAccFwd{};
+    if (pool != nullptr) return false;
     if (c.stats_acc != nullptr || c.rows2_acc != nullptr || c.in_bn != nullptr) return false;
     if (c.acorr_rows != nullptr && !(c.H % 14 == 0 && c.W % 14 == 0)) return false;
     if (c.y == nullptr && !dry && c.acorr_rows == nullptr) return false;
@@ -1077,6 +1223,21 @@
                                 (c.CinK * 4 == 64 * nw || c.CinK * 2 == 64 * nw || c.CinK == 64 * nw)))
       return false;
   }
+  FastPool fp{};
+  if (pool != nullptr) {
+    if (pool->bw == nullptr) return false;
+    if (c.CinK > KC && lab_env("SPCL_CONV_FAST_PIPE", 1) == 0) return false;
+    fp = FastPool{(const unsigned char*)pool->dpool, (unsigned char*)pool->dy, *pool->bw};
+    const long tiles = (long)c.N * cdiv(c.W, 14) * cdiv(c.H, th);
+    const bool inst = (64 * nw == 4 * c.CinK && NT == 1 && ((KC == 64 && nw == 4) || (KC == 32 && nw == 2))) ||
+                      (64 * nw == 2 * c.CinK && KC == 64 && nw == 4);
+    if (!(c.in_mode == 0 && c.rows2 != nullptr && c.H2 == 0 && !c.y2_is_poolmax && c.img2 == nullptr && c.x2 == nullptr &&
+          c.y_hi == nullptr && !c.x_up2 && c.img1 == nullptr && c.in_bn == nullptr && c.stats_acc == nullptr && th == 7 &&
+          c.H % 2 == 0 && c.W % 2 == 0 && c.CinK <= 2 * KC &&
+          fp.bw.CS == c.CinK && tiles <= BN_ACC_MAX_TILES_BWD && inst &&
+          (dry || (fp.bw.acc != nullptr && fp.bw.st != nullptr && fp.dpool != nullptr && fp.dy_out != nullptr))))
+      return false;
+  }
   if (c.rows2 != nullptr && c.in_mode != 0) return false;
   if (c.img2 != nullptr && !(c.rows2 != nullptr && c.H2 == 0 && KC == 16 && th == 14 && ntn == 1)) return false;
   a.N = c.N; a.H = c.H; a.W = c.W; a.CinK = c.CinK; a.CoutS = c.CoutS;
@@ -1086,7 +1247,7 @@
   if (c.rows2 != nullptr && c.H2 > 0 && KC == 64 && nw == 1) return false;
 #define SPCL_FAST_CASE(KC_, TH_, NT_, NW_)                               \
   if (KC == KC_ && th == TH_ && NT == NT_ && nw == NW_) {                \
-    if (!dry) launch_fast<KC_, TH_, NT_, NW_>(a, c.img1 != nullptr ? 8 : c.in_mode, st); \
+    if (!dry) launch_fast<KC_, TH_, NT_, NW_>(a, c.img1 != nullptr ? 8 : c.in_mode, st, pool != nullptr ? &fp : nullptr); \
     return true;                                                         \
   }
   SPCL_FAST_CASE(16, 14, 1, 1)
diff --git a/self-paced-contrastive-learning_amd/functional.py b/self-paced-contrastive-learning_amd/functional.py
--- a/self-paced-contrastive-learning_amd/functional.py
+++ b/self-paced-contrastive-learning_amd/functional.py
@@ -1050,6 +1050,8 @@
 
 _BLOCK1_RECOMPUTE = os.environ.get("SPCL_BLOCK1_RECOMPUTE", "1") != "0"
 _BLOCK1_POOLED_BWD = os.environ.get("SPCL_BLOCK1_POOLED_BWD", "1") != "0"
+_POOLED_DGRAD_DY = os.environ.get("SPCL_POOLED_DGRAD_DY", "1") != "0"
+_POOLED_DGRAD_DY_MIN_CS = int(os.environ.get("SPCL_POOLED_DGRAD_DY_MIN_CS", "128"))
 
 
 def _conv_from_image(image, y_image, dt_code, dtype, N, H, W, cout_s, wp_image, scale, shift, wp, want_stats):
@@ -1560,6 +1562,22 @@
     _n.call("spcl_conv3x3_dgrad_bnstats_acc", _n.ptr(dy), dt_code, N, H, W, cin_k, cout_s, _n.ptr(wp_t), _n.ptr(g), _n.ptr(y2),
             _n.ptr(st2[2]), _n.ptr(st2[3]), _n.ptr(st2[0]), _n.ptr(acc), _n.stream())
     return g
+
+
+def _dgrad_pooldy(yb, dpool, wp_t, y2, st2, dt_code, dtype, N, H, W, C, cs, stb, training, acc_b, dgamma, dbeta, acc2):
+    dev = yb.device
+    dy = torch.empty(N, H, W, cs, dtype=dtype, device=dev)
+    g = torch.empty(N, H, W, cs, dtype=dtype, device=dev)
+    rows = None
+    if acc2 is None:
+        nt = _n.call("spcl_conv_stat_rows", dt_code, N, H, W, cs, cs)
+        rows = torch.empty(nt * 2 * cs, dtype=torch.float32, device=dev)
+        rows.ntiles = nt
+    assert stb.is_contiguous() and tuple(stb.shape) == (4, cs)
+    _n.call("spcl_conv3x3_dgrad_pooldy_acc", _n.ptr(yb), _n.ptr(dpool), dt_code, N, H, W, cs, cs, _n.ptr(wp_t), _n.ptr(g),
+            _n.ptr(y2), _n.ptr(st2[2]), _n.ptr(st2[3]), _n.ptr(st2[0]), _n.ptr(rows), _n.ptr(acc2), C, _n.ptr(stb),
+            int(training), _n.ptr(acc_b), _n.ptr(dgamma), _n.ptr(dbeta), _n.ptr(dy), _n.stream())
+    return dy, g, (rows if acc2 is None else (ACC_ROWS, acc2))
 
 
 def _bnrelu_bwd_acc(y, dact, dpool, dact_nc, dt_code, dtype, N, H, W, C, cs, st, training, sinks, acc):
@@ -1774,6 +1792,7 @@
         lk = cfg.link_out
         la = getattr(cfg, "link_act", None)
         pooled = None
+        pooled_dg = None
         if la is not None and da_s is not None and dp_s is None and da_stride == 0 and la.fresh(da_s.data_ptr()):
             dyb, dgb, dbb = _bnrelu_bwd_rows(yb, da_s, None, la.rows, dtc, dtype, N, H, W, cout, cout_s, stb, cfg.training,
                                              sk[4:6])
@@ -1786,8 +1805,16 @@
                 dyb, dgb, dbb = _bnrelu_bwd_bcast(yb, g_nc, dtc, dtype, N, H, W, cout, cout_s, stb, cfg.training, sk[4:6])
         elif lk is not None and da_s is None and dp_s is not None and lk.fresh(dp_s.data_ptr()):
             if lk.rows is ACC_ROWS:
-                dyb, dgb, dbb = _bnrelu_bwd_acc(yb, None, dp_s, None, dtc, dtype, N, H, W, cout, cout_s, stb, cfg.training,
-                                                sk[4:6], _take_acc(ctx, "acc_bwd_b"))
+                acc_b = _take_acc(ctx, "acc_bwd_b")
+                if (_POOLED_DGRAD_DY and cout_s >= _POOLED_DGRAD_DY_MIN_CS and acc_b is not None and ya is not None and ctx.acorr is None and not cfg.image_input
+                        and dtype == torch.bfloat16 and tuple(stb.shape) == (4, cout_s)
+                        and _n.call("spcl_conv_dgrad_pooldy_supported", dtc, N, H, W, cout_s, cout_s, int(cfg.training))):
+                    dyb = None
+                    dgb, dbb = _grad_buffer(sk[4], (cout,), yb.device), _grad_buffer(sk[5], (cout,), yb.device)
+                    pooled_dg = (dp_s, acc_b)
+                else:
+                    dyb, dgb, dbb = _bnrelu_bwd_acc(yb, None, dp_s, None, dtc, dtype, N, H, W, cout, cout_s, stb,
+                                                    cfg.training, sk[4:6], acc_b)
             else:
                 acc = _take_acc(ctx, "acc_bwd_b") if (_ACC_FILL and H % 2 == 0 and W % 2 == 0 and cout_s <= 256) else None
                 if (acc is not None and _BLOCK1_POOLED_BWD and ya is None and ctx.acorr is not None and ctx.wpa_fwd is not None
@@ -1832,6 +1859,8 @@
         if one_pass:
             dwb, rows16 = _conv16_bwd_fused(dyb, wpb_t, ya, sta, xs, dtc, N, H, W, cout, cout, cout_s, sk[3],
                                             acorr=ctx.acorr if _CONV16_WGROWS else None, wp_image=ctx.wpa_fwd, pooled=pooled)
+        elif pooled_dg is not None:
+            dwb = None
         else:
             dwb = _wgrad(ya, dyb, dtc, N, H, W, cout, cout_s, cout_s, cout, cout_s, 1, sta[2], sta[3], sk[3]) \
                 if ctx.needs_input_grad[4] else None
@@ -1839,6 +1868,12 @@
             fused = (None, rows16)
         elif image3:
             fused = _dgrad_bnstats_image(dyb, wpb_t, ya, sta, xs, dtc, dtype, N, H, W, cout_s)
+        elif pooled_dg is not None:
+            dyb, daa_, rows_ = _dgrad_pooldy(yb, pooled_dg[0], wpb_t, ya, sta, dtc, dtype, N, H, W, cout, cout_s, stb,
+                                             cfg.training, pooled_dg[1], dgb, dbb, _take_acc(ctx, "acc_bwd_a"))
+            fused = (daa_, rows_)
+            if ctx.needs_input_grad[4]:
+                dwb = _wgrad(ya, dyb, dtc, N, H, W, cout, cout_s, cout_s, cout, cout_s, 1, sta[2], sta[3], sk[3])
         else:
             acc = _take_acc(ctx, "acc_bwd_a")
             if acc is not None:
diff --git a/self-paced-contrastive-learning_amd/native.py b/self-paced-contrastive-learning_amd/native.py
--- a/self-paced-contrastive-learning_amd/native.py
+++ b/self-paced-contrastive-learning_amd/native.py
@@ -225,6 +225,9 @@
     "spcl_conv_dgrad_poolmax_supported": (c_int, [c_int, c_int, c_int, c_int, c_int, c_int]),
     "spcl_conv3x3_dgrad_poolmax": (c_int, [_P, c_int, c_int, c_int, c_int, c_int, c_int, _P, _P, _P, _P, _P, _P, _P, _P]),
     "spcl_conv_dgrad_poolmax_acc_supported": (c_int, [c_int, c_int, c_int, c_int, c_int, c_int]),
+    "spcl_conv_dgrad_pooldy_supported": (c_int, [c_int, c_int, c_int, c_int, c_int, c_int, c_int]),
+    "spcl_conv3x3_dgrad_pooldy_acc": (c_int, [_P, _P, c_int, c_int, c_int, c_int, c_int, c_int, _P, _P, _P, _P, _P, _P, _P, _P,
+                                              c_int, _P, c_int, _P, _P, _P, _P, _P]),
     "spcl_conv3x3_dgrad_poolmax_acc": (c_int, [_P, c_int, c_int, c_int, c_int, c_int, c_int, _P, _P, _P, _P, _P, _P, _P, _P]),
     "spcl_bnrelu_backward_acc": (c_int, [_P, _P, _P, _P, c_int, c_int, c_int, c_int, c_int, c_int, _P, c_int, _P, _P, _P, _P,
                                          _P]),
@@ -311,14 +314,14 @@
                 ("nblk_co", c_int), ("CIB", c_int), ("COB", c_int), ("Cin", c_int), ("Cout", c_int)]
 
 
-ABI_VERSION = 27
+ABI_VERSION = 28
 WGRAD_BATCH_MAX = 16
 WGRAD_TAILS_MAX = 16
 _NO_STATUS = ("spcl_abi_version", "spcl_block1_recompute_supported", "spcl_block1_kernels_take", "spcl_conv16_bwd_fused_image_supported", "spcl_conv3x3_forward_image_acorr_rows", "spcl_image_autocorr_rows", "spcl_conv_dgrad_bnstats_image_supported", "spcl_conv16_bwd_fused_supported", "spcl_conv16_bwd_fused_splits", "spcl_conv_num_tiles", "spcl_conv_stat_rows", "spcl_conv_set_gemm", "spcl_conv_set_f32_split", "spcl_conv_get_f32_split", "spcl_supcon_unit_gradient_block", "spcl_conv_cat_supported", "spcl_conv_up2_supported", "spcl_conv_split_supported", "spcl_conv_split_bnstats_supported", "spcl_conv1x1_bwd_rows", "spcl_profile_count", "spcl_conv_dgrad_bnstats_supported", "spcl_conv_dgrad_poolstats_supported",
               "spcl_conv_wgrad_batched_supported", "spcl_conv_bn_acc_supported", "spcl_conv_dgrad_bnstats_acc_supported",
               "spcl_conv_dgrad_poolstats_acc_supported", "spcl_supcon_rows_supported", "spcl_bnrelu_gap_supported",
               "spcl_conv_dgrad_poolmax_supported", "spcl_conv_dgrad_poolmax_acc_supported",
-              "spcl_conv16_bwd_fused_image_pooled_supported")
+              "spcl_conv16_bwd_fused_image_pooled_supported", "spcl_conv_dgrad_pooldy_supported")
 
 
 class NativeLibraryError(RuntimeError):
```
